# vseib/point-cloud-donkey

Hardware: AMD Instinct MI355X
Metric: objects/sec classified (ModelNet10-like, SHOT-352) (higher is better)
Workload: dtype f32; 1 GPU; configs[1]: ModelNet10-like test split, 16384 pts, 1024 uniform keypoints/object, SHOT-352 (Radius 0.4, LRF 0.3), exact kNN K=1 squared-L2, mean-shift bandwidth 0.6; points_per_object=16384, keypoints_per_object=1024, classes=10, codebook_words=102400, descriptor_dim=352, collective_world_size=1

## Files before the change

### include/ismhip.h

```cpp
#ifndef ISMHIP_H_
#define ISMHIP_H_

#include <stdint.h>

#ifdef __cplusplus
extern "C" {
#endif

#define ISMHIP_ABI_VERSION 4

#define ISMHIP_OK               0
#define ISMHIP_ERR_INVALID     -1
#define ISMHIP_ERR_HIP         -2
#define ISMHIP_ERR_NOMEM       -3
#define ISMHIP_ERR_UNSUPPORTED -4
#define ISMHIP_ERR_NODEVICE    -5

#define ISMHIP_METRIC_L2SQ 0
#define ISMHIP_METRIC_CHI2 1

#define ISMHIP_W_CLASS    1u
#define ISMHIP_W_VOTE     2u
#define ISMHIP_W_MATCHING 4u
#define ISMHIP_W_CODEWORD 8u

#define ISMHIP_KERNEL_GAUSSIAN 0
#define ISMHIP_KERNEL_UNIFORM  1
#define ISMHIP_SUPPRESS_AVERAGE  0
#define ISMHIP_SUPPRESS_SUPPRESS 1
#define ISMHIP_SUPPRESS_NONE     2
#define ISMHIP_MAXFILTER_NONE   0
#define ISMHIP_MAXFILTER_SIMPLE 1
#define ISMHIP_MAXFILTER_MERGE  2
#define ISMHIP_SOM_MEANSHIFT              0
#define ISMHIP_SOM_BANDWIDTH              1
#define ISMHIP_SOM_MODEL_RADIUS           2
#define ISMHIP_SOM_COMPLETE_VOTING_SPACE  3

#define ISMHIP_SHOT_DIM   352
#define ISMHIP_BSHOT_DIM  352
#define ISMHIP_CSHOT_DIM 1344
#define ISMHIP_FPFH_DIM    33
#define ISMHIP_SHORT_SHOT_MAX_DIM 256
#define ISMHIP_COSPAIR_LEVELS 7
#define ISMHIP_COSPAIR_BINS   9
#define ISMHIP_COSPAIR_DIM  378
#define ISMHIP_SPIN_IMAGE_WIDTH 8
#define ISMHIP_SPIN_IMAGE_DIM 153
#define ISMHIP_SHORT_CSHOT_MAX_DIM 1344

typedef struct ismhip_ctx      ismhip_ctx;
typedef struct ismhip_cloud    ismhip_cloud;
typedef struct ismhip_codebook ismhip_codebook;

int  ismhip_abi_version(void);
int  ismhip_ctx_create(int device, void* stream, ismhip_ctx** out);
int  ismhip_ctx_create_on_stream(int device, void* stream, ismhip_ctx** out);
int  ismhip_ctx_destroy(ismhip_ctx* ctx);
int  ismhip_sync(ismhip_ctx* ctx);
const char* ismhip_last_error(const ismhip_ctx* ctx);
int  ismhip_timers_enable(ismhip_ctx* ctx, int on);
int  ismhip_timers_reset(ismhip_ctx* ctx);
int  ismhip_timer_get(ismhip_ctx* ctx, const char* name, double* ms_out, int64_t* launches_out);

int  ismhip_cloud_create(ismhip_ctx* ctx, int n_obj, const uint32_t* pt_offsets_h,
                         const float* x, const float* y, const float* z,
                         const float* nx, const float* ny, const float* nz,
                         const uint32_t* rgba, float cell_size, ismhip_cloud** out);
int  ismhip_cloud_destroy(ismhip_ctx* ctx, ismhip_cloud* cloud);
int  ismhip_estimate_normals(ismhip_ctx* ctx, ismhip_cloud* cloud, float radius, float* nx_out, float* ny_out, float* nz_out);
int  ismhip_estimate_normals_pca(ismhip_ctx* ctx, ismhip_cloud* cloud, float radius, int orientation, float* nx_out, float* ny_out, float* nz_out);
typedef struct ismhip_point_arrays { float *x, *y, *z, *nx, *ny, *nz; uint32_t* rgba; } ismhip_point_arrays;
int  ismhip_filter_normals(ismhip_ctx* ctx, int n_obj, const uint32_t* pt_offsets_h, const ismhip_point_arrays* in,
                           const ismhip_point_arrays* out, uint32_t* pt_offsets_h_out);
#define ISMHIP_SOR_MAX_MEAN_K 64
int  ismhip_filter_statistical(ismhip_ctx* ctx, const ismhip_cloud* cloud, int mean_k, float stddev_mul, uint8_t* keep_out,
                               float* mean_dist_out, double* threshold_h_out);
int  ismhip_filter_radius(ismhip_ctx* ctx, const ismhip_cloud* cloud, float radius, int min_neighbors, uint8_t* keep_out, uint32_t* count_out);
int  ismhip_filter_passthrough_z(ismhip_ctx* ctx, uint32_t n_pts, const float* x, const float* y, const float* z, float z_min, float z_max,
                                 uint8_t* keep_out);
int  ismhip_compact_points(ismhip_ctx* ctx, int n_obj, const uint32_t* pt_offsets_h, const ismhip_point_arrays* in, const uint8_t* keep,
                           const ismhip_point_arrays* out, uint32_t* pt_offsets_h_out);
int  ismhip_cloud_centroids(ismhip_ctx* ctx, const ismhip_cloud* cloud, float* centroid_out);
int  ismhip_cloud_radii(ismhip_ctx* ctx, const ismhip_cloud* cloud, const float* centroid, float* radius_out);

int  ismhip_shot_lrf(ismhip_ctx* ctx, const ismhip_cloud* cloud, const uint32_t* kp_offsets_h,
                     const float* kpx, const float* kpy, const float* kpz,
                     float radius, float* lrf9_out);
int  ismhip_shotna_lrf(ismhip_ctx* ctx, const ismhip_cloud* cloud, const uint32_t* kp_offsets_h,
                       const float* kpx, const float* kpy, const float* kpz,
                       float radius, float* lrf9_out);

int  ismhip_shot352(ismhip_ctx* ctx, const ismhip_cloud* cloud, const uint32_t* kp_offsets_h,
                    const float* kpx, const float* kpy, const float* kpz,
                    const float* lrf9, float radius, float* desc_out, uint32_t* neighbour_count_out);
int  ismhip_bshot_binarize(ismhip_ctx* ctx, int n_rows, const float* src, float* dst);
int  ismhip_bshot352(ismhip_ctx* ctx, const ismhip_cloud* cloud, const uint32_t* kp_offsets_h,
                     const float* kpx, const float* kpy, const float* kpz,
                     const float* lrf9, float radius, float* desc_out, uint32_t* neighbour_count_out);
int  ismhip_cshot1344(ismhip_ctx* ctx, const ismhip_cloud* cloud, const uint32_t* kp_offsets_h,
                      const float* kpx, const float* kpy, const float* kpz, const uint32_t* kp_rgba,
                      const float* lrf9, float radius, float* desc_out, uint32_t* neighbour_count_out);
int  ismhip_fpfh33(ismhip_ctx* ctx, const ismhip_cloud* cloud, const uint32_t* kp_offsets_h,
                   const float* kpx, const float* kpy, const float* kpz,
                   float radius, float* desc_out, uint32_t* neighbour_count_out);
int  ismhip_short_shot(ismhip_ctx* ctx, const ismhip_cloud* cloud, const uint32_t* kp_offsets_h,
                       const float* kpx, const float* kpy, const float* kpz, const float* lrf9,
                       float radius, float min_radius, int log_radius, int r_bins, int e_bins, int a_bins,
                       float* desc_out, uint32_t* neighbour_count_out);
int  ismhip_short_cshot(ismhip_ctx* ctx, const ismhip_cloud* cloud, const uint32_t* kp_offsets_h,
                        const float* kpx, const float* kpy, const float* kpz, const uint32_t* kp_rgba, const float* lrf9,
                        float radius, float min_radius, int log_radius, int r_bins, int e_bins, int a_bins,
                        int rc_bins, int ec_bins, int ac_bins, int hist_size, float* desc_out, uint32_t* neighbour_count_out);
int  ismhip_cospair(ismhip_ctx* ctx, const ismhip_cloud* cloud, const uint32_t* kp_offsets_h,
                    const float* kpx, const float* kpy, const float* kpz, float radius, float* desc_out,
                    uint32_t* neighbour_count_out, uint32_t* level_count_out, uint32_t* snap_index_out);
int  ismhip_keypoint_normals(ismhip_ctx* ctx, const ismhip_cloud* cloud, const uint32_t* kp_offsets_h,
                             const float* kpx, const float* kpy, const float* kpz,
                             float* knx_out, float* kny_out, float* knz_out, int32_t* src_index_out);
int  ismhip_spin_image(ismhip_ctx* ctx, const ismhip_cloud* cloud, const uint32_t* kp_offsets_h,
                       const float* kpx, const float* kpy, const float* kpz, const float* ax, const float* ay, const float* az,
                       float radius, int image_width, float* desc_out, uint32_t* neighbour_count_out);
int  ismhip_center_dist(ismhip_ctx* ctx, const ismhip_cloud* cloud, const uint32_t* kp_offsets_h,
                        const float* kpx, const float* kpy, const float* kpz, float* out);

int  ismhip_global_short_shot(ismhip_ctx* ctx, const ismhip_cloud* cloud, int n_regions, const int32_t* region_obj, const float* region_center,
                              const float* region_radius, double min_radius, int log_radius, int r_bins, int e_bins, int a_bins,
                              uint32_t* n_sel_out, float* centroid_out, float* radius_out, float* lrf9_out, float* desc_out, uint32_t* count_out);
int  ismhip_global_shot352(ismhip_ctx* ctx, const ismhip_cloud* cloud, int n_regions, const int32_t* region_obj, const float* region_center,
                           const float* region_radius, uint32_t* n_sel_out, float* centroid_out, float* radius_out, float* lrf9_out, float* desc_out);

int  ismhip_voxel_keypoints(ismhip_ctx* ctx, int n_obj, const uint32_t* pt_offsets_h,
                            const float* x, const float* y, const float* z, const uint32_t* rgba, float leaf,
                            uint32_t capacity, float* kx, float* ky, float* kz, uint32_t* krgba,
                            uint32_t* kp_offsets_h_out);

int  ismhip_iss3d_saliency(ismhip_ctx* ctx, const ismhip_cloud* cloud, float salient_radius, double gamma21, double gamma32, int min_neighbors,
                           double* saliency_out, double* eig_out, uint32_t* count_out);
int  ismhip_iss3d_keypoints(ismhip_ctx* ctx, const ismhip_cloud* cloud, float salient_radius, float non_max_radius, double gamma21, double gamma32,
                            int min_neighbors, uint32_t capacity, float* kx, float* ky, float* kz, uint32_t* krgba, uint32_t* src_index_out,
                            uint32_t* kp_offsets_h_out);

int  ismhip_compact_features(ismhip_ctx* ctx, int n_obj, const uint32_t* kp_offsets_h, int dim,
                             const float* desc, const float* lrf9,
                             const float* kpx, const float* kpy, const float* kpz,
                             float* desc_out, float* lrf9_out,
                             float* kpx_out, float* kpy_out, float* kpz_out,
                             uint32_t* src_index_out, uint32_t* keep_offsets_h_out);

int  ismhip_compact_descriptor_rows(ismhip_ctx* ctx, int n_obj, const uint32_t* kp_offsets_h, int dim,
                                    const float* desc, const float* lrf9,
                                    const float* kpx, const float* kpy, const float* kpz,
                                    float* desc_out, float* lrf9_out,
                                    float* kpx_out, float* kpy_out, float* kpz_out,
                                    uint32_t* src_index_out, uint32_t* keep_offsets_h_out, int* all_kept_out);

int  ismhip_gather_columns(ismhip_ctx* ctx, int n_rows, int dim_in, const float* src, int n_cols, const int32_t* cols_h, float* dst);

int  ismhip_codebook_create(ismhip_ctx* ctx, int n_words, int dim, const float* words_h,
                            const float* word_weight_h,
                            const uint32_t* vote_offsets_h,
                            const float* vote_xyz_h,
                            const float* vote_weight_h,
                            const float* vote_class_weight_h,
                            const uint32_t* vote_class_h,
                            const uint32_t* vote_instance_h,
                            const float* vote_bbox_quat_h,
                            const float* vote_bbox_size_h,
                            int n_classes, const float* class_sigma_h,
                            ismhip_codebook** out);
int  ismhip_codebook_set_word_class(ismhip_ctx* ctx, ismhip_codebook* cb, const uint32_t* word_class_h);
int  ismhip_codebook_set_word_keypoint(ismhip_ctx* ctx, ismhip_codebook* cb, const float* word_keypoint_h);
int  ismhip_codebook_destroy(ismhip_ctx* ctx, ismhip_codebook* cb);
int  ismhip_codebook_max_votes_per_word(const ismhip_codebook* cb);
int  ismhip_codebook_stage1_dims(const ismhip_codebook* cb, float* energy_out);
int  ismhip_codebook_stage2_dims(const ismhip_codebook* cb, float* energy_out);

int  ismhip_codebook_make_binary(ismhip_ctx* ctx, ismhip_codebook* cb);
int  ismhip_codebook_has_binary(const ismhip_codebook* cb);

int  ismhip_knn(ismhip_ctx* ctx, const ismhip_codebook* cb, int metric, int nq, const float* q,
                int k, int32_t* idx_out, float* dist_out);
int  ismhip_knn_binary(ismhip_ctx* ctx, const ismhip_codebook* cb, int nq, const float* q, int k, int32_t* idx_out, float* dist_out);
#define ISMHIP_KNN_LARGE_K_MAX 1024
int  ismhip_knn_large_k(ismhip_ctx* ctx, const ismhip_codebook* cb, int metric, int nq, const float* q,
                        int k, int32_t* idx_out, float* dist_out);
int  ismhip_knn_ratio(ismhip_ctx* ctx, const ismhip_codebook* cb, int metric, int nq, const float* q,
                      float ratio_threshold, int32_t* idx_out, float* dist_out);

int  ismhip_knn_rule(ismhip_ctx* ctx, const ismhip_codebook* cb, int metric, int nq, const float* q,
                     float ratio_threshold, int32_t* idx_out, float* dist_out);

int  ismhip_knn_threshold(ismhip_ctx* ctx, const ismhip_codebook* cb, int metric, int nq, const float* q, float threshold,
                          int64_t capacity, uint32_t* act_offsets_out, int32_t* idx_out, float* dist_out, int64_t* n_act_h_out);

int  ismhip_cast_votes(ismhip_ctx* ctx, const ismhip_codebook* cb, uint32_t weight_flags,
                       int nq, const float* lrf9, const float* kpx, const float* kpy, const float* kpz,
                       int k, const int32_t* idx, const float* dist,
                       float* vote_pos_out,
                       float* vote_weight_out,
                       int32_t* vote_class_out,
                       int32_t* vote_instance_out,
                       int32_t* vote_codeword_out,
                       float* vote_bbox_quat_out,
                       float* vote_bbox_size_out );

int  ismhip_cast_votes_csr(ismhip_ctx* ctx, const ismhip_codebook* cb, uint32_t weight_flags,
                           int nq, const float* lrf9, const float* kpx, const float* kpy, const float* kpz,
                           const uint32_t* act_offsets, int64_t n_act, const int32_t* idx, const float* dist,
                           float* vote_pos_out, float* vote_weight_out, int32_t* vote_class_out, int32_t* vote_instance_out,
                           int32_t* vote_codeword_out, float* vote_bbox_quat_out, float* vote_bbox_size_out);

int  ismhip_vote_keypoints(ismhip_ctx* ctx, const ismhip_codebook* cb, int nq, const float* kpx, const float* kpy, const float* kpz,
                           int k, const int32_t* idx, float* vote_kp_out, float* vote_kp_train_out);
int  ismhip_vote_keypoints_csr(ismhip_ctx* ctx, const ismhip_codebook* cb, int nq, const float* kpx, const float* kpy, const float* kpz,
                               const uint32_t* act_offsets, int64_t n_act, const int32_t* idx, float* vote_kp_out, float* vote_kp_train_out);

int  ismhip_ransac_filter(ismhip_ctx* ctx, int n_clusters, const uint32_t* cluster_offsets_h, const float* src_xyz, const float* tgt_xyz,
                          const float* threshold_h, int max_iterations, unsigned long long seed,
                          uint8_t* inlier_out, int32_t* kept_out, int32_t* n_inliers_out, int32_t* best_hypothesis_out, int32_t* iterations_out,
                          float* transform_out);
int  ismhip_ransac_hypothesis(ismhip_ctx* ctx, int n_clusters, const uint32_t* cluster_offsets_h, const float* src_xyz, const float* tgt_xyz,
                              const float* threshold_h, unsigned long long seed, const int32_t* hypothesis_h,
                              uint8_t* inlier_out, int32_t* valid_out, int32_t* n_inliers_out, double* d2_out, double* transform_out);

typedef struct ismhip_maxima_params {
    int   n_classes;
    const float* class_bandwidth_h;
    float bandwidth;
    float threshold;
    int   max_iter;
    int   kernel;
    int   suppression;
    int   min_votes_threshold;
    float min_threshold;
    int   best_k;
    int   max_maxima;
    int   max_filter;
    const float* vote_bbox_quat;
    float* max_bbox_quat_out;
    int   single_object_max_type;
    const float* object_centroid;
    const float* object_radius;
} ismhip_maxima_params;

int  ismhip_find_maxima(ismhip_ctx* ctx, int n_obj, const uint32_t* slot_offsets_h,
                        const float* vote_pos, const float* vote_weight, const int32_t* vote_class,
                        const int32_t* vote_instance, const float* vote_bbox_size ,
                        const ismhip_maxima_params* params,
                        int32_t* n_maxima_out, float* max_pos_out, float* max_weight_out,
                        int32_t* max_class_out, int32_t* max_instance_out, float* max_instance_weight_out,
                        float* max_bbox_size_out , int32_t* max_n_votes_out,
                        float* class_score_out);

typedef struct ismhip_ransac_params {
    const float* vote_keypoint;
    const float* vote_keypoint_training;
    float inlier_threshold;
    const float* class_inlier_threshold_h;
    int   max_iterations;
    unsigned long long seed;
} ismhip_ransac_params;
int  ismhip_find_maxima_ransac(ismhip_ctx* ctx, int n_obj, const uint32_t* slot_offsets_h,
                               const float* vote_pos, const float* vote_weight, const int32_t* vote_class,
                               const int32_t* vote_instance, const float* vote_bbox_size ,
                               const ismhip_maxima_params* params,
                               int32_t* n_maxima_out, float* max_pos_out, float* max_weight_out,
                               int32_t* max_class_out, int32_t* max_instance_out, float* max_instance_weight_out,
                               float* max_bbox_size_out , int32_t* max_n_votes_out,
                               float* class_score_out, const ismhip_ransac_params* ransac, float* max_transform_out);

int  ismhip_train_activate(ismhip_ctx* ctx, int metric, int n, int dim, const float* desc, const float* lrf9,
                           const float* kpx, const float* kpy, const float* kpz,
                           const uint32_t* feat_class_h, const uint32_t* feat_model_h, const float* feat_center_h,
                           int n_codewords, const float* codewords ,
                           int k, int clean_up_single_vote, int n_classes,
                           int32_t* n_words_out, uint32_t* word_src_out, uint32_t* vote_offsets_out, uint32_t* vote_feature_out,
                           float* vote_xyz_out, float* vote_weight_out, float* vote_class_weight_out, float* class_sigma_out);

int  ismhip_train_activate_lists(ismhip_ctx* ctx, int metric, int n, int dim, const float* desc, const float* lrf9,
                                 const float* kpx, const float* kpy, const float* kpz,
                                 const uint32_t* feat_class_h, const uint32_t* feat_model_h, const float* feat_center_h,
                                 int n_codewords, const float* codewords ,
                                 const uint32_t* act_offsets, const int32_t* act_idx, int64_t n_act, int n_classes,
                                 int32_t* n_words_out, uint32_t* word_src_out, uint32_t* vote_offsets_out, uint32_t* vote_feature_out,
                                 float* vote_xyz_out, float* vote_weight_out, float* vote_class_weight_out, float* class_sigma_out);

#define ISMHIP_RANK_KNN_ACTIVATION 0
#define ISMHIP_RANK_INCREMENTAL    1
#define ISMHIP_RANK_STRANGENESS    2
#define ISMHIP_RANK_NAIVE_BAYES    3
int  ismhip_rank_scores(ismhip_ctx* ctx, int type, int n, int dim, const float* desc, int n_classes, const uint32_t* class_offsets_h,
                        int k_search, float dist_threshold, int increment_type, float* score_out);
int  ismhip_rank_select(ismhip_ctx* ctx, int n, int n_classes, const uint32_t* class_offsets_h, const float* score,
                        float factor, float extract_offset, uint8_t* keep_out, uint32_t* n_keep_h_out);

#define ISMHIP_CENTERS_RANDOM   0
#define ISMHIP_CENTERS_GONZALES 1
#define ISMHIP_CENTERS_KMEANSPP 2
int  ismhip_kmeans(ismhip_ctx* ctx, int metric, int n, int dim, const float* desc, int n_clusters, int max_iterations,
                   int centers_init, unsigned long long seed, float* centers_out, int32_t* assign_out, float* dist_out,
                   int32_t* n_clusters_out, int32_t* iterations_out );

typedef struct ismhip_hough_params {
    int   n_classes;
    float min_coord[3];
    float max_coord[3];
    float bin_size;
    const float* class_bin_h;
    int   use_interpolation;
    float rel_threshold;
    int   min_votes_threshold;
    float min_threshold;
    int   best_k;
    int   max_maxima;
    int   max_filter;
    const float* vote_bbox_quat;
    float* max_bbox_quat_out;
} ismhip_hough_params;
int  ismhip_hough3d_maxima(ismhip_ctx* ctx, int n_obj, const uint32_t* slot_offsets_h,
                           const float* vote_pos, const float* vote_weight, const int32_t* vote_class,
                           const int32_t* vote_instance, const float* vote_bbox_size ,
                           const ismhip_hough_params* params,
                           int32_t* n_maxima_out, float* max_pos_out, float* max_weight_out,
                           int32_t* max_class_out, int32_t* max_instance_out, float* max_instance_weight_out,
                           float* max_bbox_size_out , int32_t* max_n_votes_out,
                           float* class_score_out);

int  ismhip_hough3d_maxima_ransac(ismhip_ctx* ctx, int n_obj, const uint32_t* slot_offsets_h,
                                  const float* vote_pos, const float* vote_weight, const int32_t* vote_class,
                                  const int32_t* vote_instance, const float* vote_bbox_size ,
                                  const ismhip_hough_params* params,
                                  int32_t* n_maxima_out, float* max_pos_out, float* max_weight_out,
                                  int32_t* max_class_out, int32_t* max_instance_out, float* max_instance_weight_out,
                                  float* max_bbox_size_out , int32_t* max_n_votes_out,
                                  float* class_score_out, const ismhip_ransac_params* ransac, float* max_transform_out);

#ifdef __cplusplus
}
#endif
#endif
```

### point-cloud-donkey_amd/capi.py

```python
import ctypes as C
import os

import numpy as np

_HERE = os.path.dirname(os.path.abspath(__file__))
LIB_PATH = os.path.join(_HERE, "libismhip.so")

METRIC_L2SQ, METRIC_CHI2 = 0, 1
W_CLASS, W_VOTE, W_MATCHING, W_CODEWORD = 1, 2, 4, 8
KERNEL_GAUSSIAN, KERNEL_UNIFORM = 0, 1
SUPPRESS_AVERAGE, SUPPRESS_SUPPRESS, SUPPRESS_NONE = 0, 1, 2
MAXFILTER_NONE, MAXFILTER_SIMPLE, MAXFILTER_MERGE = 0, 1, 2
SOM_MEANSHIFT, SOM_BANDWIDTH, SOM_MODEL_RADIUS, SOM_COMPLETE_VOTING_SPACE = 0, 1, 2, 3
ERR_NODEVICE = -5

EXPORTS = [
    "ismhip_abi_version", "ismhip_ctx_create", "ismhip_ctx_create_on_stream", "ismhip_ctx_destroy", "ismhip_sync", "ismhip_last_error",
    "ismhip_timers_enable", "ismhip_timers_reset", "ismhip_timer_get",
    "ismhip_cloud_create", "ismhip_cloud_destroy", "ismhip_cloud_centroids", "ismhip_cloud_radii", "ismhip_estimate_normals", "ismhip_estimate_normals_pca",
    "ismhip_shot_lrf", "ismhip_shotna_lrf", "ismhip_shot352", "ismhip_cshot1344", "ismhip_fpfh33", "ismhip_center_dist",
    "ismhip_compact_features", "ismhip_compact_descriptor_rows", "ismhip_filter_normals", "ismhip_voxel_keypoints", "ismhip_gather_columns",
    "ismhip_codebook_create", "ismhip_codebook_set_word_class", "ismhip_codebook_destroy", "ismhip_codebook_max_votes_per_word", "ismhip_codebook_stage1_dims", "ismhip_codebook_stage2_dims",
    "ismhip_knn", "ismhip_knn_ratio", "ismhip_knn_rule", "ismhip_cast_votes", "ismhip_find_maxima", "ismhip_hough3d_maxima", "ismhip_train_activate", "ismhip_kmeans",
    "ismhip_knn_threshold", "ismhip_cast_votes_csr", "ismhip_train_activate_lists", "ismhip_knn_large_k",
    "ismhip_filter_statistical", "ismhip_filter_radius", "ismhip_filter_passthrough_z", "ismhip_compact_points",
    "ismhip_codebook_set_word_keypoint", "ismhip_vote_keypoints", "ismhip_vote_keypoints_csr", "ismhip_ransac_filter", "ismhip_ransac_hypothesis",
    "ismhip_find_maxima_ransac", "ismhip_hough3d_maxima_ransac", "ismhip_short_shot", "ismhip_short_cshot", "ismhip_cospair",
    "ismhip_bshot_binarize", "ismhip_bshot352", "ismhip_codebook_make_binary", "ismhip_codebook_has_binary", "ismhip_knn_binary",
    "ismhip_rank_scores", "ismhip_rank_select", "ismhip_global_short_shot", "ismhip_global_shot352",
    "ismhip_iss3d_saliency", "ismhip_iss3d_keypoints", "ismhip_keypoint_normals", "ismhip_spin_image",
]
RANSAC_MAX_ITERATIONS = 10000
RANSAC_SEED = 12345


class MaximaParams(C.Structure):
    _fields_ = [("n_classes", C.c_int), ("class_bandwidth_h", C.c_void_p), ("bandwidth", C.c_float),
                ("threshold", C.c_float), ("max_iter", C.c_int), ("kernel", C.c_int), ("suppression", C.c_int),
                ("min_votes_threshold", C.c_int), ("min_threshold", C.c_float), ("best_k", C.c_int),
                ("max_maxima", C.c_int), ("max_filter", C.c_int),
                ("vote_bbox_quat", C.c_void_p), ("max_bbox_quat_out", C.c_void_p), ("single_object_max_type", C.c_int),
                ("object_centroid", C.c_void_p), ("object_radius", C.c_void_p)]


class HoughParams(C.Structure):
    _fields_ = [("n_classes", C.c_int), ("min_coord", C.c_float * 3), ("max_coord", C.c_float * 3), ("bin_size", C.c_float),
                ("class_bin_h", C.c_void_p), ("use_interpolation", C.c_int), ("rel_threshold", C.c_float),
                ("min_votes_threshold", C.c_int), ("min_threshold", C.c_float), ("best_k", C.c_int), ("max_maxima", C.c_int), ("max_filter", C.c_int),
                ("vote_bbox_quat", C.c_void_p), ("max_bbox_quat_out", C.c_void_p)]


class RansacParams(C.Structure):
    _fields_ = [("vote_keypoint", C.c_void_p), ("vote_keypoint_training", C.c_void_p), ("inlier_threshold", C.c_float),
                ("class_inlier_threshold_h", C.c_void_p), ("max_iterations", C.c_int), ("seed", C.c_ulonglong)]


class IsmHipError(RuntimeError):
    pass


_lib = None


def lib():
    global _lib
    if _lib is None:
        if not os.path.exists(LIB_PATH):
            raise IsmHipError(f"{LIB_PATH} not built: run `python -c 'import __graft_entry__ as g; g.build()'` "
                              "(make -C point-cloud-donkey_amd/csrc)")
        import torch
        L = C.CDLL(LIB_PATH)
        L.ismhip_last_error.restype = C.c_char_p
        L.ismhip_last_error.argtypes = [C.c_void_p]
        for name in EXPORTS:
            fn = getattr(L, name)
            if name != "ismhip_last_error":
                fn.restype = C.c_int
        _lib = L
    return _lib


def _p(t):
    if t is None:
        return C.c_void_p(0)
    if isinstance(t, np.ndarray):
        assert t.flags["C_CONTIGUOUS"]
        return C.c_void_p(t.ctypes.data)
    assert t.is_contiguous()
    return C.c_void_p(t.data_ptr())


def _u32(a):
    return np.ascontiguousarray(np.asarray(a, dtype=np.uint32))


class Ctx:
    def __init__(self, device=0, stream="torch"):
        self._h = C.c_void_p()
        L = lib()
        if stream is None:
            rc = L.ismhip_ctx_create(C.c_int(device), C.c_void_p(0), C.byref(self._h))
        else:
            if stream == "torch":
                import torch
                if not torch.cuda.is_available():
                    raise IsmHipError("no gfx950 device visible: the hot path has no CPU fallback (ISMHIP_ERR_NODEVICE)")
                if not (0 <= device < torch.cuda.device_count()):
                    raise IsmHipError(f"device {device} out of range (ISMHIP_ERR_INVALID)")
                stream = torch.cuda.current_stream(device).cuda_stream
            rc = L.ismhip_ctx_create_on_stream(C.c_int(device), C.c_void_p(stream), C.byref(self._h))
        if rc != 0:
            raise IsmHipError(f"ismhip_ctx_create failed ({rc}); a gfx950 device is required, there is no CPU fallback")
        self.device = device

    def check(self, rc, what):
        if rc != 0:
            raise IsmHipError(f"{what} failed ({rc}): {lib().ismhip_last_error(self._h).decode()}")

    def sync(self):
        self.check(lib().ismhip_sync(self._h), "ismhip_sync")

    def timers_enable(self, on=True):
        self.check(lib().ismhip_timers_enable(self._h, C.c_int(1 if on else 0)), "timers_enable")

    def timers_reset(self):
        self.check(lib().ismhip_timers_reset(self._h), "timers_reset")

    def timer(self, name):
        ms, n = C.c_double(), C.c_int64()
        self.check(lib().ismhip_timer_get(self._h, name.encode(), C.byref(ms), C.byref(n)), "timer_get")
        return ms.value, n.value

    def close(self):
        if self._h:
            lib().ismhip_ctx_destroy(self._h)
            self._h = C.c_void_p()

    def __del__(self):
        try:
            self.close()
        except Exception:
            pass


class Cloud:

    def __init__(self, ctx, pt_offsets, x, y, z, nx, ny, nz, cell_size, rgba=None):
        self.ctx = ctx
        self.pt_offsets = _u32(pt_offsets)
        self.n_obj = len(self.pt_offsets) - 1
        self._keep = (x, y, z, nx, ny, nz, rgba)
        self._h = C.c_void_p()
        rc = lib().ismhip_cloud_create(ctx._h, C.c_int(self.n_obj), _p(self.pt_offsets), _p(x), _p(y), _p(z), _p(nx), _p(ny),
                                       _p(nz), _p(rgba), C.c_float(cell_size), C.byref(self._h))
        ctx.check(rc, "ismhip_cloud_create")

    def close(self):
        if self._h:
            lib().ismhip_cloud_destroy(self.ctx._h, self._h)
            self._h = C.c_void_p()

    def __del__(self):
        try:
            self.close()
        except Exception:
            pass


class Codebook:
    def __init__(self, ctx, words, vote_offsets, vote_xyz, vote_class, vote_instance, n_classes, class_sigma,
                 word_weight=None, vote_weight=None, vote_class_weight=None, vote_bbox_quat=None, vote_bbox_size=None):
        f32 = lambda a: None if a is None else np.ascontiguousarray(np.asarray(a, dtype=np.float32))
        self.ctx = ctx
        words = f32(words)
        self.n_words, self.dim = words.shape
        self.n_classes = int(n_classes)
        self._h = C.c_void_p()
        rc = lib().ismhip_codebook_create(ctx._h, C.c_int(self.n_words), C.c_int(self.dim), _p(words), _p(f32(word_weight)),
                                          _p(_u32(vote_offsets)), _p(f32(vote_xyz)), _p(f32(vote_weight)),
                                          _p(f32(vote_class_weight)), _p(_u32(vote_class)), _p(_u32(vote_instance)),
                                          _p(f32(vote_bbox_quat)), _p(f32(vote_bbox_size)), C.c_int(self.n_classes),
                                          _p(f32(class_sigma)), C.byref(self._h))
        ctx.check(rc, "ismhip_codebook_create")
        self.max_votes = lib().ismhip_codebook_max_votes_per_word(self._h)
        e = C.c_float(1.0)
        self.stage1_dims = int(lib().ismhip_codebook_stage1_dims(self._h, C.byref(e)))
        self.stage1_energy = float(e.value)
        self.stage2_dims = int(lib().ismhip_codebook_stage2_dims(self._h, C.byref(e)))
        self.stage2_energy = float(e.value)

    def set_word_class(self, word_class):
        self.ctx.check(lib().ismhip_codebook_set_word_class(self.ctx._h, self._h, _p(_u32(word_class))), "ismhip_codebook_set_word_class")

    def set_word_keypoint(self, word_keypoint):
        kp = np.ascontiguousarray(np.asarray(word_keypoint, dtype=np.float32))
        assert kp.shape == (self.n_words, 3)
        self.ctx.check(lib().ismhip_codebook_set_word_keypoint(self.ctx._h, self._h, _p(kp)), "ismhip_codebook_set_word_keypoint")

    def make_binary(self):
        self.ctx.check(lib().ismhip_codebook_make_binary(self.ctx._h, self._h), "ismhip_codebook_make_binary")

    @property
    def has_binary(self):
        return lib().ismhip_codebook_has_binary(self._h) == 1

    def close(self):
        if self._h:
            lib().ismhip_codebook_destroy(self.ctx._h, self._h)
            self._h = C.c_void_p()

    def __del__(self):
        try:
            self.close()
        except Exception:
            pass


def _torch():
    import torch
    return torch


def shot_lrf(ctx, cloud, kp_offsets, kpx, kpy, kpz, radius):
    torch = _torch()
    ko = _u32(kp_offsets)
    out = torch.empty((int(ko[-1]), 9), dtype=torch.float32, device=kpx.device)
    ctx.check(lib().ismhip_shot_lrf(ctx._h, cloud._h, _p(ko), _p(kpx), _p(kpy), _p(kpz), C.c_float(radius), _p(out)), "ismhip_shot_lrf")
    return out


def shotna_lrf(ctx, cloud, kp_offsets, kpx, kpy, kpz, radius):
    torch = _torch()
    ko = _u32(kp_offsets)
    out = torch.empty((int(ko[-1]), 9), dtype=torch.float32, device=kpx.device)
    ctx.check(lib().ismhip_shotna_lrf(ctx._h, cloud._h, _p(ko), _p(kpx), _p(kpy), _p(kpz), C.c_float(radius), _p(out)), "ismhip_shotna_lrf")
    return out


LRF_TYPES = {"SHOT": shot_lrf, "SHOTNA": shotna_lrf}


def shot352(ctx, cloud, kp_offsets, kpx, kpy, kpz, lrf, radius, want_counts=False):
    torch = _torch()
    ko = _u32(kp_offsets)
    n = int(ko[-1])
    out = torch.empty((n, 352), dtype=torch.float32, device=kpx.device)
    cnt = torch.empty((n,), dtype=torch.int32, device=kpx.device) if want_counts else None
    ctx.check(lib().ismhip_shot352(ctx._h, cloud._h, _p(ko), _p(kpx), _p(kpy), _p(kpz), _p(lrf), C.c_float(radius), _p(out), _p(cnt)),
              "ismhip_shot352")
    return (out, cnt) if want_counts else out


def bshot_binarize(ctx, src, out=None):
    torch = _torch()
    assert src.dim() == 2 and src.shape[1] == 352 and src.dtype == torch.float32
    if out is None:
        out = torch.empty_like(src)
    ctx.check(lib().ismhip_bshot_binarize(ctx._h, C.c_int(src.shape[0]), _p(src), _p(out)), "ismhip_bshot_binarize")
    return out


def bshot352(ctx, cloud, kp_offsets, kpx, kpy, kpz, lrf, radius, want_counts=False):
    torch = _torch()
    ko = _u32(kp_offsets)
    n = int(ko[-1])
    out = torch.empty((n, 352), dtype=torch.float32, device=kpx.device)
    cnt = torch.empty((n,), dtype=torch.int32, device=kpx.device) if want_counts else None
    ctx.check(lib().ismhip_bshot352(ctx._h, cloud._h, _p(ko), _p(kpx), _p(kpy), _p(kpz), _p(lrf), C.c_float(radius), _p(out), _p(cnt)),
              "ismhip_bshot352")
    return (out, cnt) if want_counts else out


def cshot1344(ctx, cloud, kp_offsets, kpx, kpy, kpz, kp_rgba, lrf, radius, want_counts=False):
    torch = _torch()
    ko = _u32(kp_offsets)
    n = int(ko[-1])
    out = torch.empty((n, 1344), dtype=torch.float32, device=kpx.device)
    cnt = torch.empty((n,), dtype=torch.int32, device=kpx.device) if want_counts else None
    ctx.check(lib().ismhip_cshot1344(ctx._h, cloud._h, _p(ko), _p(kpx), _p(kpy), _p(kpz), _p(kp_rgba), _p(lrf), C.c_float(radius),
                                     _p(out), _p(cnt)), "ismhip_cshot1344")
    return (out, cnt) if want_counts else out


def short_shot(ctx, cloud, kp_offsets, kpx, kpy, kpz, lrf, radius, bins=(2, 2, 8), min_radius=0.0, log_radius=False, want_counts=False):
    torch = _torch()
    ko = _u32(kp_offsets)
    n = int(ko[-1])
    r, e, a = (int(b) for b in bins)
    out = torch.empty((n, max(r * e * a, 0) if min(r, e, a) > 0 else 0), dtype=torch.float32, device=kpx.device)
    cnt = torch.empty((n,), dtype=torch.int32, device=kpx.device) if want_counts else None
    ctx.check(lib().ismhip_short_shot(ctx._h, cloud._h, _p(ko), _p(kpx), _p(kpy), _p(kpz), _p(lrf), C.c_float(radius), C.c_float(min_radius),
                                      C.c_int(1 if log_radius else 0), C.c_int(r), C.c_int(e), C.c_int(a), _p(out), _p(cnt)), "ismhip_short_shot")
    return (out, cnt) if want_counts else out


SHORT_SHOT_AUTO_BINS = {8: (1, 1, 8), 16: (2, 2, 4), 24: (2, 2, 6), 32: (2, 2, 8), 64: (2, 4, 8), 96: (3, 4, 8), 128: (4, 4, 8), 192: (6, 4, 8),
                        256: (8, 4, 8)}


def short_shot_grid(dims=32, bin_type="auto", bins=(2, 2, 8)):
    if bin_type == "manual":
        r, e, a = (int(b) for b in bins)
        return r * e * a, (r, e, a)
    if bin_type == "auto" and int(dims) in SHORT_SHOT_AUTO_BINS:
        return int(dims), SHORT_SHOT_AUTO_BINS[int(dims)]
    return 32, (2, 2, 8)


def short_shot_min_radius(radius, use_min_radius=False, min_radius_relative=0.0, log_radius=False):
    if use_min_radius:
        return float(np.float32(float(np.float32(radius)) * float(min_radius_relative)))
    return float(np.float32(float(np.float32(radius)) * float(np.float32(0.1)))) if log_radius else 0.0


def short_cshot(ctx, cloud, kp_offsets, kpx, kpy, kpz, kp_rgba, lrf, radius, bins=(2, 2, 8), color_bins=(2, 2, 8), hist_size=15, min_radius=0.0,
                log_radius=False, want_counts=False):
    torch = _torch()
    ko = _u32(kp_offsets)
    n = int(ko[-1])
    r, e, a = (int(b) for b in bins)
    rc, ec, ac = (int(b) for b in color_bins)
    h = int(hist_size)
    out = torch.empty((n, r * e * a + rc * ec * ac * h if min(r, e, a, rc, ec, ac, h) > 0 else 0), dtype=torch.float32, device=kpx.device)
    cnt = torch.empty((n,), dtype=torch.int32, device=kpx.device) if want_counts else None
    ctx.check(lib().ismhip_short_cshot(ctx._h, cloud._h, _p(ko), _p(kpx), _p(kpy), _p(kpz), _p(kp_rgba), _p(lrf), C.c_float(radius),
                                       C.c_float(min_radius), C.c_int(1 if log_radius else 0), C.c_int(r), C.c_int(e), C.c_int(a), C.c_int(rc),
                                       C.c_int(ec), C.c_int(ac), C.c_int(h), _p(out), _p(cnt)), "ismhip_short_cshot")
    return (out, cnt) if want_counts else out


SHORT_CSHOT_COLOR_BINS = {d: SHORT_SHOT_AUTO_BINS[d] for d in (8, 16, 24, 32, 64, 96, 128)}


def short_cshot_color_grid(dims=32):
    if int(dims) in SHORT_CSHOT_COLOR_BINS:
        return int(dims), SHORT_CSHOT_COLOR_BINS[int(dims)]
    return 32, (2, 2, 8)


COSPAIR_LEVELS, COSPAIR_BINS, COSPAIR_DIM = 7, 9, 378


def cospair(ctx, cloud, kp_offsets, kpx, kpy, kpz, radius, want_counts=False, want_levels=False, want_snap=False):
    torch = _torch()
    ko = _u32(kp_offsets)
    n = int(ko[-1])
    out = torch.empty((n, COSPAIR_DIM), dtype=torch.float32, device=kpx.device)
    cnt = torch.empty((n,), dtype=torch.int32, device=kpx.device) if want_counts else None
    lev = torch.empty((n, COSPAIR_LEVELS), dtype=torch.int32, device=kpx.device) if want_levels else None
    snap = torch.empty((n,), dtype=torch.int32, device=kpx.device) if want_snap else None
    ctx.check(lib().ismhip_cospair(ctx._h, cloud._h, _p(ko), _p(kpx), _p(kpy), _p(kpz), C.c_float(radius), _p(out), _p(cnt), _p(lev), _p(snap)),
              "ismhip_cospair")
    extra = [t for t in (cnt, lev, snap) if t is not None]
    return (out, *extra) if extra else out


SPIN_IMAGE_WIDTH = 8
SPIN_IMAGE_DIM = (SPIN_IMAGE_WIDTH + 1) * (2 * SPIN_IMAGE_WIDTH + 1)


def keypoint_normals(ctx, cloud, kp_offsets, kpx, kpy, kpz, want_index=False):
    torch = _torch()
    ko = _u32(kp_offsets)
    n = int(ko[-1])
    nx, ny, nz = (torch.empty((n,), dtype=torch.float32, device=kpx.device) for _ in range(3))
    src = torch.empty((n,), dtype=torch.int32, device=kpx.device) if want_index else None
    ctx.check(lib().ismhip_keypoint_normals(ctx._h, cloud._h, _p(ko), _p(kpx), _p(kpy), _p(kpz), _p(nx), _p(ny), _p(nz), _p(src)),
              "ismhip_keypoint_normals")
    return (nx, ny, nz, src) if want_index else (nx, ny, nz)


def spin_image(ctx, cloud, kp_offsets, kpx, kpy, kpz, ax, ay, az, radius, image_width=SPIN_IMAGE_WIDTH, want_counts=False):
    torch = _torch()
    ko = _u32(kp_offsets)
    n = int(ko[-1])
    w = int(image_width)
    out = torch.empty((n, (w + 1) * (2 * w + 1) if w >= 1 else 0), dtype=torch.float32, device=kpx.device)
    cnt = torch.empty((n,), dtype=torch.int32, device=kpx.device) if want_counts else None
    ctx.check(lib().ismhip_spin_image(ctx._h, cloud._h, _p(ko), _p(kpx), _p(kpy), _p(kpz), _p(ax), _p(ay), _p(az), C.c_float(radius), C.c_int(w),
                                      _p(out), _p(cnt)), "ismhip_spin_image")
    return (out, cnt) if want_counts else out


GLOBAL_SHORT_SHOT_AUTO_BINS = dict(SHORT_SHOT_AUTO_BINS)
GLOBAL_SHORT_SHOT_AUTO_BINS[64] = (4, 2, 8)


def global_short_shot_grid(dims=32, bin_type="auto", bins=(1, 1, 8)):
    if bin_type == "manual":
        r, e, a = (int(b) for b in bins)
        return r * e * a, (r, e, a)
    if bin_type == "auto" and int(dims) in GLOBAL_SHORT_SHOT_AUTO_BINS:
        return int(dims), GLOBAL_SHORT_SHOT_AUTO_BINS[int(dims)]
    return 32, (2, 2, 8)


def _regions(cloud, region_obj, region_center, region_radius, dev):
    torch = _torch()
    obj = torch.as_tensor(np.ascontiguousarray(np.asarray(region_obj, dtype=np.int32)), device=dev)
    n = int(obj.shape[0])
    cen = np.zeros((n, 3), np.float32) if region_center is None else np.ascontiguousarray(np.asarray(region_center, dtype=np.float32)).reshape(n, 3)
    rad = np.full((n,), -1.0, np.float32) if region_radius is None else np.ascontiguousarray(np.asarray(region_radius, dtype=np.float32)).reshape(n)
    return n, obj, torch.as_tensor(cen, device=dev), torch.as_tensor(rad, device=dev)


def _global_outputs(n, dim, dev):
    torch = _torch()
    return dict(n_sel=torch.empty((n,), dtype=torch.int32, device=dev), centroid=torch.empty((n, 3), dtype=torch.float32, device=dev),
                radius=torch.empty((n,), dtype=torch.float32, device=dev), lrf=torch.empty((n, 9), dtype=torch.float32, device=dev),
                desc=torch.empty((n, dim), dtype=torch.float32, device=dev))


def global_short_shot(ctx, cloud, dev, region_obj, region_center=None, region_radius=None, bins=(2, 2, 8), min_radius=0.1, log_radius=False,
                      want_counts=False):
    torch = _torch()
    n, obj, cen, rad = _regions(cloud, region_obj, region_center, region_radius, dev)
    r, e, a = (int(b) for b in bins)
    out = _global_outputs(n, r * e * a if min(r, e, a) > 0 else 0, dev)
    if want_counts:
        out["counts"] = torch.empty_like(out["desc"], dtype=torch.int32)
    ctx.check(lib().ismhip_global_short_shot(ctx._h, cloud._h, C.c_int(n), _p(obj), _p(cen), _p(rad), C.c_double(min_radius),
                                             C.c_int(1 if log_radius else 0), C.c_int(r), C.c_int(e), C.c_int(a), _p(out["n_sel"]),
                                             _p(out["centroid"]), _p(out["radius"]), _p(out["lrf"]), _p(out["desc"]), _p(out.get("counts"))),
              "ismhip_global_short_shot")
    return out


def global_shot352(ctx, cloud, dev, region_obj, region_center=None, region_radius=None):
    n, obj, cen, rad = _regions(cloud, region_obj, region_center, region_radius, dev)
    out = _global_outputs(n, 352, dev)
    ctx.check(lib().ismhip_global_shot352(ctx._h, cloud._h, C.c_int(n), _p(obj), _p(cen), _p(rad), _p(out["n_sel"]), _p(out["centroid"]),
                                          _p(out["radius"]), _p(out["lrf"]), _p(out["desc"])), "ismhip_global_shot352")
    return out


def fpfh33(ctx, cloud, kp_offsets, kpx, kpy, kpz, radius, want_counts=False):
    torch = _torch()
    ko = _u32(kp_offsets)
    n = int(ko[-1])
    out = torch.empty((n, 33), dtype=torch.float32, device=kpx.device)
    cnt = torch.empty((n,), dtype=torch.int32, device=kpx.device) if want_counts else None
    ctx.check(lib().ismhip_fpfh33(ctx._h, cloud._h, _p(ko), _p(kpx), _p(kpy), _p(kpz), C.c_float(radius), _p(out), _p(cnt)),
              "ismhip_fpfh33")
    return (out, cnt) if want_counts else out


def cloud_centroids(ctx, cloud, device):
    torch = _torch()
    out = torch.empty((cloud.n_obj, 3), dtype=torch.float32, device=device)
    ctx.check(lib().ismhip_cloud_centroids(ctx._h, cloud._h, _p(out)), "ismhip_cloud_centroids")
    return out


def cloud_radii(ctx, cloud, centroid):
    torch = _torch()
    out = torch.empty((cloud.n_obj,), dtype=torch.float32, device=centroid.device)
    ctx.check(lib().ismhip_cloud_radii(ctx._h, cloud._h, _p(centroid), _p(out)), "ismhip_cloud_radii")
    return out


def center_dist(ctx, cloud, kp_offsets, kpx, kpy, kpz):
    torch = _torch()
    ko = _u32(kp_offsets)
    out = torch.empty((int(ko[-1]),), dtype=torch.float32, device=kpx.device)
    ctx.check(lib().ismhip_center_dist(ctx._h, cloud._h, _p(ko), _p(kpx), _p(kpy), _p(kpz), _p(out)), "ismhip_center_dist")
    return out


def estimate_normals(ctx, cloud, radius, nx, ny, nz):
    ctx.check(lib().ismhip_estimate_normals(ctx._h, cloud._h, C.c_float(radius), _p(nx), _p(ny), _p(nz)), "ismhip_estimate_normals")
    cloud._keep = getattr(cloud, "_keep", ()) + (nx, ny, nz)
    return nx, ny, nz


def estimate_normals_pca(ctx, cloud, radius, orientation, nx, ny, nz):
    ctx.check(lib().ismhip_estimate_normals_pca(ctx._h, cloud._h, C.c_float(radius), C.c_int(orientation), _p(nx), _p(ny), _p(nz)), "ismhip_estimate_normals_pca")
    cloud._keep = getattr(cloud, "_keep", ()) + (nx, ny, nz)
    return nx, ny, nz


class _PointArrays(C.Structure):
    _fields_ = [(n, C.c_void_p) for n in ("x", "y", "z", "nx", "ny", "nz", "rgba")]


def _compact_point_arrays(ctx, symbol, pt_offsets, arrays, rgba, *mask):
    torch = _torch()
    po = _u32(pt_offsets)
    n_obj = len(po) - 1
    ins = list(arrays) + ([rgba] if rgba is not None else [])
    outs = [torch.empty_like(t) for t in ins]
    a_in = _PointArrays(*[t.data_ptr() for t in ins], *([None] if rgba is None else []))
    a_out = _PointArrays(*[t.data_ptr() for t in outs], *([None] if rgba is None else []))
    new = np.zeros(n_obj + 1, dtype=np.uint32)
# ... 431 lines not shown
```

### point-cloud-donkey_amd/csrc/common.h

```cpp
#pragma once
#include <hip/hip_runtime.h>
#include <stdint.h>
#include <map>
#include <set>
#include <string>
#include <vector>
#include "../../include/ismhip.h"

#define ISM_WAVE 64

#define ISM_GRID_MAXDIM 32
#define ISM_GRID_MAXCELLS (ISM_GRID_MAXDIM * ISM_GRID_MAXDIM * ISM_GRID_MAXDIM)
#define ISM_GRID_STRIDE (ISM_GRID_MAXCELLS + 1)

#define ISM_GRID_XFRAC 3
struct GridMeta {
    float minv[3];
    float cell[3];
    float inv_cell[3];
    int   dim[3];
    float centroid[3];
    uint32_t n_finite;
};

struct ismhip_cloud {
    int n_obj = 0;
    uint32_t n_pts = 0;
    uint32_t max_pts = 0;
    std::vector<uint32_t> pt_off_h;
    uint32_t* pt_off = nullptr;
    const float *x = nullptr, *y = nullptr, *z = nullptr, *nx = nullptr, *ny = nullptr, *nz = nullptr;
    const uint32_t* rgba = nullptr;
    float4* sp4 = nullptr;
    float4* sn4 = nullptr;
    float4* slab4 = nullptr;
    uint32_t* cell_of_pt = nullptr;
    uint32_t* rank_of_pt = nullptr;
    uint32_t* members = nullptr;
    GridMeta* meta = nullptr;
    uint32_t* cell_start = nullptr;
    float requested_cell = 0.f;
    uint32_t* kp_perm = nullptr;
    size_t kp_perm_cap = 0;
    const float* kp_perm_key = nullptr;
    std::vector<uint32_t> kp_perm_off;
    uint16_t* cospair_code = nullptr;
    size_t cospair_code_cap = 0;
    bool cospair_code_valid = false;
    size_t cap_pts = 0; int cap_obj = 0; bool cap_color = false;
};

struct PcaImage {
    int m = 0;
    float* R = nullptr;
    unsigned short* f16t = nullptr;
    float* cn_scaled = nullptr;
    float* osc = nullptr;
    float sq = 1.f, sc = 1.f;
    float cmax2 = 0.f;
    float inv_sig2 = 1.f;
    float d_rel = 0.f;
    float dq_abs = 0.f, dc_abs = 0.f;
    float resid2 = 0.f;
    float energy = 0.f;
};

struct ismhip_codebook {
    int n_words = 0, dim = 0, dim_pad = 0, n_votes = 0, max_votes = 0, n_classes = 0;
    float* words = nullptr;
    int n_words_pad = 0;
    float* word_norm = nullptr;
    unsigned short* words_bf16_hi = nullptr;
    unsigned short* words_bf16_lo = nullptr;
    unsigned short* words_f16 = nullptr;
    unsigned short* words_f16t = nullptr;
    int ld16 = 0;
    float f16_scale = 1.f;
    bool words_nonneg = false;
    float max_norm2 = 0.f;
    float* word_weight = nullptr;
    uint32_t* vote_off = nullptr;
    float* vote_xyz = nullptr;
    float* vote_weight = nullptr;
    float* vote_class_weight = nullptr;
    uint32_t* vote_class = nullptr;
    uint32_t* vote_instance = nullptr;
    float* vote_bbox_quat = nullptr;
    float* vote_bbox_size = nullptr;
    float* class_sigma = nullptr;
    uint32_t* word_class = nullptr;
    float* word_keypoint = nullptr;
    ismhip_codebook* chi_shadow = nullptr;
    uint32_t* shadow_perm = nullptr;
    PcaImage pca, pca2;
    int8_t* bin_words = nullptr;
    int32_t* bin_norm = nullptr;
    int bin_ld = 0, bin_shift = 0;
};

struct TimerAcc {
    std::vector<std::pair<hipEvent_t, hipEvent_t>> pending;
    double ms = 0.0;
    int64_t launches = 0;
};

struct ismhip_ctx {
    int device = 0;
    hipStream_t stream = nullptr;
    bool own_stream = false;
    std::string err;
    bool timers_on = false;
    std::map<std::string, TimerAcc> timers;
    std::vector<hipEvent_t> event_pool;
    struct Slot { void* p = nullptr; size_t bytes = 0; };
    std::map<int, Slot> scratch;
    float* lut_srgb = nullptr;
    float* lut_sxyz = nullptr;
    std::vector<ismhip_cloud*> cloud_pool;
    uint32_t* truncated_d = nullptr;
    unsigned long long* ransac_counters_d = nullptr;
    uint32_t knn_stats[2] = {0, 0};
    std::set<const void*> attr_done;
    uint32_t knn_stage2_queries = 0;
    uint32_t knn_stage2_list_entries = 0;
    uint32_t knn_stage2_ranged = 0;
    uint32_t knn_seed_launches = 0;
    bool knn_stage2_splits = true;
    bool knn_stage2_seed = true;
    bool knn_two_stage = true;
    bool knn_join = true;
    bool knn_qpanel2 = true;
    bool knn_half = false;
    int knn_splits = 0;
    int knn_t = 0;
    bool xcd_map = true;
    bool grid_fused = true;
    bool kp_order = true;
    float grid_xfrac = 0.f;
    int shot_var = 0;
    bool knn_hell_emit = true;
    bool knn_hellinger = true;
    int knn_t1 = 2;
    int knn_pre_step = 32;
    float knn_pre_gamma = 1.0f;
    bool knn_prepass = true;
    int knn_pca_m = -1;
    bool knn_stage2_t4 = false;
    bool codebook_light = false;
    int knn_pca_m2 = -1;
    uint32_t knn_pca_launches = 0;
    uint32_t knn_thr_overflow = 0;
    uint32_t knn_thr_mfma_launches = 0;
    bool knn_lk_fast = false;
    bool knn_lk_exact = false;
    float knn_lk_seed_scale = 1.0f;
    uint32_t knn_lk_stats[3] = {0, 0, 0};
    uint32_t knn_binary_launches = 0;
    uint32_t rank_launches = 0;
    bool iss3d_wave = false;
    int knn_mode = 0;
};

enum ScratchSlot {
    SCR_KP_OFF = 1, SCR_TIE_LIST, SCR_TIE_REC, SCR_TIE_KEYS, SCR_COUNTERS, SCR_KNN_CAND_IDX, SCR_KNN_CAND_VAL,
    SCR_QNORM, SCR_FPFH_FLAG, SCR_FPFH_LIST, SCR_FPFH_SPFH, SCR_FPFH_LOOKUP, SCR_SLOT_OFF, SCR_CLASS_BW,
    SCR_COMPACT_KEEP, SCR_COMPACT_POS, SCR_OBJ_COUNT, SCR_QPAD, SCR_LRF_COV, SCR_KNN_FLAGS, SCR_KNN_QSPLIT, SCR_MAX_REC, SCR_QNORM2, SCR_KNN_Q2, SCR_KNN_LIST2, SCR_TRAIN, SCR_TRAIN2, SCR_MAX_WORK, SCR_KMEANS, SCR_KNN_CLOCK, SCR_PCA, SCR_KNN_THR0, SCR_KNN_QSQRT, SCR_KNN_HELL_EMIT, SCR_KNN_THR, SCR_KNN_THR2, SCR_TRAIN_ACT, SCR_KNN_LK, SCR_KNN_LK2, SCR_KNN_LK3, SCR_PREFILTER, SCR_RANSAC, SCR_COSPAIR, SCR_KNNB_FLAG, SCR_KNNB_Q, SCR_KNNB_CAND, SCR_RANK, SCR_RANK_KNN, SCR_KNN_LISTS, SCR_KNN_QUEUE, SCR_ISS3D
};

int  ism_set_err(ismhip_ctx* ctx, int code, const std::string& msg);
void* ism_scratch(ismhip_ctx* ctx, int slot, size_t bytes);
int  ism_lds_cap(ismhip_ctx* ctx, const void* kern, size_t bytes);

uint32_t* ism_upload_offsets(ismhip_ctx* ctx, int slot, const uint32_t* off_h, int n);
struct RaggedOffsets { uint32_t max_run = 0, total = 0; uint32_t* dev = nullptr; };
enum { RAGGED_START0 = 1,
       RAGGED_EMPTY = 2 };
int ism_ragged_offsets(ismhip_ctx* ctx, const std::string& name, const uint32_t* off_h, int n, int slot, int flags, RaggedOffsets* r);
int ism_offsets_from_counts(ismhip_ctx* ctx, int n, const uint32_t* cnt_d, uint32_t* off_h_out, uint32_t* max_run_out);
const uint32_t* ism_kp_order(ismhip_ctx* ctx, const ismhip_cloud* cloud, const uint32_t* kp_offsets_h, const uint32_t* ko,
                             const float* kpx, const float* kpy, const float* kpz, uint32_t maxk);

int ism_compact_keypoints(ismhip_ctx* ctx, const std::string& who, const ismhip_cloud* cloud, const uint8_t* mask, uint32_t capacity,
                          float* kx, float* ky, float* kz, uint32_t* krgba, uint32_t* src_index_out, uint32_t* kp_offsets_h_out);

#define ISM_HIP(ctx, call)                                                                          \
    do {                                                                                            \
        hipError_t e__ = (call);                                                                    \
        if (e__ != hipSuccess)                                                                      \
            return ism_set_err((ctx), ISMHIP_ERR_HIP, std::string(#call) + ": " + hipGetErrorString(e__)); \
    } while (0)

#define ISM_CHECK_LAUNCH(ctx, name)                                                                 \
    do {                                                                                            \
        hipError_t e__ = hipGetLastError();                                                         \
        if (e__ != hipSuccess)                                                                      \
            return ism_set_err((ctx), ISMHIP_ERR_HIP, std::string("launch ") + name + ": " + hipGetErrorString(e__)); \
    } while (0)

struct TimerScope {
    ismhip_ctx* ctx; const char* name; hipEvent_t a = nullptr, b = nullptr;
    TimerScope(ismhip_ctx* c, const char* n);
    ~TimerScope();
};

#ifdef __HIPCC__
__device__ __forceinline__ int lane_id() { return threadIdx.x & 63; }

__device__ __forceinline__ float sqdist3(float ax, float ay, float az, float bx, float by, float bz) {
    float r = 0.f, d;
    d = ax - bx; r += d * d;
    d = ay - by; r += d * d;
    d = az - bz; r += d * d;
    return r;
}

template <int CTRL>
__device__ __forceinline__ int dpp_mov0(int v) { return __builtin_amdgcn_update_dpp(0, v, CTRL, 0xf, 0xf, false); }

__device__ __forceinline__ float wave_sum_f(float v) {
    v += __int_as_float(dpp_mov0<0xb1>(__float_as_int(v)));
    v += __int_as_float(dpp_mov0<0x4e>(__float_as_int(v)));
    v += __int_as_float(dpp_mov0<0x114>(__float_as_int(v)));
    v += __int_as_float(dpp_mov0<0x118>(__float_as_int(v)));
    v += __int_as_float(dpp_mov0<0x142>(__float_as_int(v)));
    v += __int_as_float(dpp_mov0<0x143>(__float_as_int(v)));
    return __int_as_float(__builtin_amdgcn_readlane(__float_as_int(v), 63));
}
__device__ __forceinline__ int wave_sum_i(int v) {
    v += dpp_mov0<0xb1>(v);
    v += dpp_mov0<0x4e>(v);
    v += dpp_mov0<0x114>(v);
    v += dpp_mov0<0x118>(v);
    v += dpp_mov0<0x142>(v);
    v += dpp_mov0<0x143>(v);
    return __builtin_amdgcn_readlane(v, 63);
}
template <int CTRL>
__device__ __forceinline__ int dpp_movi(int ident, int v) { return __builtin_amdgcn_update_dpp(ident, v, CTRL, 0xf, 0xf, false); }
__device__ __forceinline__ float wave_min_f(float v) {
    const int inf = 0x7f800000;
    v = fminf(v, __int_as_float(dpp_movi<0xb1>(inf, __float_as_int(v))));
    v = fminf(v, __int_as_float(dpp_movi<0x4e>(inf, __float_as_int(v))));
    v = fminf(v, __int_as_float(dpp_movi<0x114>(inf, __float_as_int(v))));
    v = fminf(v, __int_as_float(dpp_movi<0x118>(inf, __float_as_int(v))));
    v = fminf(v, __int_as_float(dpp_movi<0x142>(inf, __float_as_int(v))));
    v = fminf(v, __int_as_float(dpp_movi<0x143>(inf, __float_as_int(v))));
    return __int_as_float(__builtin_amdgcn_readlane(__float_as_int(v), 63));
}
template <int CTRL>
__device__ __forceinline__ unsigned long long dpp_min_u64(unsigned long long v) {
    const unsigned lo = (unsigned)dpp_movi<CTRL>(-1, (int)(unsigned)(v & 0xffffffffull)), hi = (unsigned)dpp_movi<CTRL>(-1, (int)(unsigned)(v >> 32));
    const unsigned long long o = ((unsigned long long)hi << 32) | lo;
    return o < v ? o : v;
}
__device__ __forceinline__ unsigned long long wave_min_u64(unsigned long long v) {
    v = dpp_min_u64<0xb1>(v); v = dpp_min_u64<0x4e>(v); v = dpp_min_u64<0x114>(v);
    v = dpp_min_u64<0x118>(v); v = dpp_min_u64<0x142>(v); v = dpp_min_u64<0x143>(v);
    const unsigned lo = (unsigned)__builtin_amdgcn_readlane((int)(unsigned)(v & 0xffffffffull), 63), hi = (unsigned)__builtin_amdgcn_readlane((int)(unsigned)(v >> 32), 63);
    return ((unsigned long long)hi << 32) | lo;
}
__device__ __forceinline__ float wave_max_f(float v) {
    const int ninf = (int)0xff800000;
    v = fmaxf(v, __int_as_float(dpp_movi<0xb1>(ninf, __float_as_int(v))));
    v = fmaxf(v, __int_as_float(dpp_movi<0x4e>(ninf, __float_as_int(v))));
    v = fmaxf(v, __int_as_float(dpp_movi<0x114>(ninf, __float_as_int(v))));
    v = fmaxf(v, __int_as_float(dpp_movi<0x118>(ninf, __float_as_int(v))));
    v = fmaxf(v, __int_as_float(dpp_movi<0x142>(ninf, __float_as_int(v))));
    v = fmaxf(v, __int_as_float(dpp_movi<0x143>(ninf, __float_as_int(v))));
    return __int_as_float(__builtin_amdgcn_readlane(__float_as_int(v), 63));
}
__device__ __forceinline__ uint32_t wave_max_u32(uint32_t v) {
    v = max(v, (uint32_t)dpp_mov0<0xb1>((int)v)); v = max(v, (uint32_t)dpp_mov0<0x4e>((int)v)); v = max(v, (uint32_t)dpp_mov0<0x114>((int)v));
    v = max(v, (uint32_t)dpp_mov0<0x118>((int)v)); v = max(v, (uint32_t)dpp_mov0<0x142>((int)v)); v = max(v, (uint32_t)dpp_mov0<0x143>((int)v));
    return (uint32_t)__builtin_amdgcn_readlane((int)v, 63);
}
template <int CTRL>
__device__ __forceinline__ unsigned long long dpp_mov0_u64(unsigned long long v) {
    const unsigned lo = (unsigned)dpp_mov0<CTRL>((int)(unsigned)(v & 0xffffffffull)), hi = (unsigned)dpp_mov0<CTRL>((int)(unsigned)(v >> 32));
    return ((unsigned long long)hi << 32) | lo;
}
__device__ __forceinline__ unsigned long long readlane63_u64(unsigned long long v) {
    const unsigned lo = (unsigned)__builtin_amdgcn_readlane((int)(unsigned)(v & 0xffffffffull), 63), hi = (unsigned)__builtin_amdgcn_readlane((int)(unsigned)(v >> 32), 63);
    return ((unsigned long long)hi << 32) | lo;
}
template <int CTRL>
__device__ __forceinline__ unsigned long long dpp_max_u64(unsigned long long v) { const unsigned long long o = dpp_mov0_u64<CTRL>(v); return o > v ? o : v; }
__device__ __forceinline__ unsigned long long wave_max_u64(unsigned long long v) {
    v = dpp_max_u64<0xb1>(v); v = dpp_max_u64<0x4e>(v); v = dpp_max_u64<0x114>(v);
    v = dpp_max_u64<0x118>(v); v = dpp_max_u64<0x142>(v); v = dpp_max_u64<0x143>(v);
    return readlane63_u64(v);
}
__device__ __forceinline__ unsigned long long wave_sum_u64(unsigned long long v) {
    v += dpp_mov0_u64<0xb1>(v); v += dpp_mov0_u64<0x4e>(v); v += dpp_mov0_u64<0x114>(v);
    v += dpp_mov0_u64<0x118>(v); v += dpp_mov0_u64<0x142>(v); v += dpp_mov0_u64<0x143>(v);
    return readlane63_u64(v);
}
__device__ __forceinline__ uint32_t wave_incl_scan_u32(uint32_t v) {
    int x = (int)v;
    x += dpp_mov0<0x111>(x); x += dpp_mov0<0x112>(x); x += dpp_mov0<0x114>(x); x += dpp_mov0<0x118>(x);
    x += __builtin_amdgcn_update_dpp(0, x, 0x142, 0xa, 0xf, false);
    x += __builtin_amdgcn_update_dpp(0, x, 0x143, 0xc, 0xf, false);
    return (uint32_t)x;
}
template <int NT>
struct BlockScan {
    uint32_t wave[NT / 64];
    uint32_t carry;
    __device__ __forceinline__ void init() {
        if (threadIdx.x == 0) carry = 0;
        __syncthreads();
    }
    __device__ __forceinline__ uint32_t step(uint32_t v) {
        const uint32_t incl = wave_incl_scan_u32(v);
        const int w = threadIdx.x >> 6;
        if (lane_id() == 63) wave[w] = incl;
        __syncthreads();
        uint32_t before = carry;
        for (int k = 0; k < w; ++k) before += wave[k];
        __syncthreads();
        if (threadIdx.x == NT - 1) carry = before + incl;
        __syncthreads();
        return before + incl - v;
    }
    __device__ __forceinline__ uint32_t total() const { return carry; }
};
template <int NT>
struct BlockRank {
    uint32_t wave[NT / 64];
    __device__ __forceinline__ uint32_t step(bool flag, uint32_t& total) {
        const unsigned long long b = __ballot(flag);
        const int w = threadIdx.x >> 6;
        if (lane_id() == 0) wave[w] = (uint32_t)__popcll(b);
        __syncthreads();
        uint32_t before = total, chunk = 0;
#pragma unroll
        for (int k = 0; k < NT / 64; ++k) { const uint32_t c = wave[k]; chunk += c; if (k < w) before += c; }
        __syncthreads();
        total += chunk;
        return before + (uint32_t)__popcll(b & ((1ull << lane_id()) - 1ull));
    }
};
template <int CTRL>
__device__ __forceinline__ double dpp_mov0_d(double v) {
    const long long b = __double_as_longlong(v);
    const int lo = dpp_mov0<CTRL>((int)(b & 0xffffffffll)), hi = dpp_mov0<CTRL>((int)(b >> 32));
    return __longlong_as_double(((long long)hi << 32) | (unsigned int)lo);
}
__device__ __forceinline__ double wave_sum_d(double v) {
    v += dpp_mov0_d<0xb1>(v);
    v += dpp_mov0_d<0x4e>(v);
    v += dpp_mov0_d<0x114>(v);
    v += dpp_mov0_d<0x118>(v);
    v += dpp_mov0_d<0x142>(v);
    v += dpp_mov0_d<0x143>(v);
    const long long b = __double_as_longlong(v);
    const int lo = __builtin_amdgcn_readlane((int)(b & 0xffffffffll), 63), hi = __builtin_amdgcn_readlane((int)(b >> 32), 63);
    return __longlong_as_double(((long long)hi << 32) | (unsigned int)lo);
}

template <int NW, class T, class F>
__device__ __forceinline__ T block_fold(T wave_total, T* red, F&& combine) {
    if (lane_id() == 0) red[threadIdx.x >> 6] = wave_total;
    __syncthreads();
    T r = red[0];
#pragma unroll
    for (int k = 1; k < NW; ++k) r = combine(r, red[k]);
    __syncthreads();
    return r;
}
template <int NW = 4, class T>
__device__ __forceinline__ T block_sum_i(T v, T* red) { return block_fold<NW>((T)wave_sum_i((int)v), red, [](T a, T b) { return (T)(a + b); }); }
template <int NW = 4>
__device__ __forceinline__ unsigned long long block_sum_u64(unsigned long long v, unsigned long long* red) {
    return block_fold<NW>(wave_sum_u64(v), red, [](unsigned long long a, unsigned long long b) { return a + b; });
}
template <int NW = 4>
__device__ __forceinline__ float block_min_f(float v, float* red) { return block_fold<NW>(wave_min_f(v), red, [](float a, float b) { return fminf(a, b); }); }
template <int NW = 4>
__device__ __forceinline__ float block_max_f(float v, float* red) { return block_fold<NW>(wave_max_f(v), red, [](float a, float b) { return fmaxf(a, b); }); }
template <int NW = 4>
__device__ __forceinline__ uint32_t block_max_u32(uint32_t v, uint32_t* red) { return block_fold<NW>(wave_max_u32(v), red, [](uint32_t a, uint32_t b) { return a > b ? a : b; }); }
template <int NW = 4>
__device__ __forceinline__ unsigned long long block_min_u64(unsigned long long v, unsigned long long* red) {
    return block_fold<NW>(wave_min_u64(v), red, [](unsigned long long a, unsigned long long b) { return b < a ? b : a; });
}
template <int NW = 4>
__device__ __forceinline__ unsigned long long block_max_u64(unsigned long long v, unsigned long long* red) {
    return block_fold<NW>(wave_max_u64(v), red, [](unsigned long long a, unsigned long long b) { return b > a ? b : a; });
}
template <int NW = 4>
__device__ __forceinline__ double block_sum_d_left(double v, double* red) { return block_fold<NW>(wave_sum_d(v), red, [](double a, double b) { return a + b; }); }
template <class T>
__device__ __forceinline__ T block_sum_pairwise(T wave_total, T* red) {
    if (lane_id() == 0) red[threadIdx.x >> 6] = wave_total;
    __syncthreads();
    const T r = (red[0] + red[1]) + (red[2] + red[3]);
    __syncthreads();
    return r;
}
__device__ __forceinline__ float block_sum_f_pairwise(float v, float* red) { return block_sum_pairwise(wave_sum_f(v), red); }
__device__ __forceinline__ double block_sum_d_pairwise(double v, double* red) { return block_sum_pairwise(wave_sum_d(v), red); }

__device__ __forceinline__ float shot_atan2(float y, float x) {
    const float ax = fabsf(x), ay = fabsf(y);
    const float mx = fmaxf(ax, ay), mn = fminf(ax, ay);
    const float a = mn * __builtin_amdgcn_rcpf(mx);
    const float z = a * a;
    float p = 0.0028662257f;
    p = __builtin_fmaf(p, z, -0.0161657367f); p = __builtin_fmaf(p, z, 0.0429096138f); p = __builtin_fmaf(p, z, -0.0752896400f);
    p = __builtin_fmaf(p, z, 0.1065626393f); p = __builtin_fmaf(p, z, -0.1420889944f); p = __builtin_fmaf(p, z, 0.1999355085f);
    p = __builtin_fmaf(p, z, -0.3333314528f); p = __builtin_fmaf(p, z, 1.0f);
    float r = a * p;
    if (ay > ax) r = 1.57079632679489661923f - r;
    if (x < 0.f) r = 3.14159265358979323846f - r;
    return y < 0.f ? -r : r;
}

__device__ __forceinline__ void rgb2lab(const float* lut_srgb, const float* lut_sxyz, uint32_t c4, float& L, float& A, float& B) {
    const float fr = lut_srgb[(c4 >> 16) & 0xff], fg = lut_srgb[(c4 >> 8) & 0xff], fb = lut_srgb[c4 & 0xff];
    const float X = fr * 0.412453f + fg * 0.357580f + fb * 0.180423f;
    const float Y = fr * 0.212671f + fg * 0.715160f + fb * 0.072169f;
    const float Z = fr * 0.019334f + fg * 0.119193f + fb * 0.950227f;
    float vx = X / 0.95047f, vy = Y, vz = Z / 1.08883f;
    int ix = (int)(vx * 4000), iy = (int)(vy * 4000), iz = (int)(vz * 4000);
    ix = ix < 0 ? 0 : (ix > 3999 ? 3999 : ix); iy = iy < 0 ? 0 : (iy > 3999 ? 3999 : iy); iz = iz < 0 ? 0 : (iz > 3999 ? 3999 : iz);
    vx = lut_sxyz[ix]; vy = lut_sxyz[iy]; vz = lut_sxyz[iz];
    L = 116.0f * vy - 16.0f; if (L > 100) L = 100.0f;
    A = 500.0f * (vx - vy); if (A > 120) A = 120.0f; else if (A < -120) A = -120.0f;
    B = 200.0f * (vy - vz); if (B > 120) B = 120.0f; else if (B < -120) B = -120.0f;
}
__device__ __forceinline__ void rgb2lab_norm(const float* lut_srgb, const float* lut_sxyz, uint32_t c4, float& L, float& A, float& B) {
    rgb2lab(lut_srgb, lut_sxyz, c4, L, A, B);
    L /= 100.0f; A /= 120.0f; B /= 120.0f;
}

__device__ __forceinline__ bool xcd_object_block(int nbx, int n_obj, int& o, int& bx) {
    if (n_obj < 8) { o = blockIdx.x / nbx; bx = blockIdx.x % nbx; return true; }
    const int slot = blockIdx.x >> 3;
    o = (slot / nbx) * 8 + (blockIdx.x & 7);
    bx = slot % nbx;
    return o < n_obj;
}
__device__ __forceinline__ uint32_t ordered_keypoint(const uint32_t* __restrict__ perm, uint32_t kp_begin, uint32_t slot) {
    return kp_begin + (perm ? perm[kp_begin + slot] : slot);
}
static inline unsigned xcd_object_grid(unsigned nbx, int n_obj) { return n_obj < 8 ? nbx * (unsigned)n_obj : 8u * nbx * (unsigned)((n_obj + 7) / 8); }

__device__ __forceinline__ int cell_coord(float v, float minv, float inv_cell, int dim) {
    int c = (int)floorf((v - minv) * inv_cell);
    return c < 0 ? 0 : (c >= dim ? dim - 1 : c);
}
// ... 140 lines not shown
```

### point-cloud-donkey_amd/csrc/ctx.hip

```cpp
#include "common.h"
#include <cmath>
#include <cstring>
#include <cstdlib>

extern "C" void ism_cloud_pool_release(ismhip_ctx* ctx);

int ism_set_err(ismhip_ctx* ctx, int code, const std::string& msg) {
    if (ctx) ctx->err = msg;
    return code;
}

int ism_lds_cap(ismhip_ctx* ctx, const void* kern, size_t bytes) {
    if (ctx->attr_done.count(kern)) return ISMHIP_OK;
    ISM_HIP(ctx, hipFuncSetAttribute(kern, hipFuncAttributeMaxDynamicSharedMemorySize, (int)bytes));
    ctx->attr_done.insert(kern);
    return ISMHIP_OK;
}

void* ism_scratch(ismhip_ctx* ctx, int slot, size_t bytes) {
    if (bytes == 0) bytes = 16;
    auto& s = ctx->scratch[slot];
    if (s.bytes >= bytes) return s.p;
    if (s.p) { (void)hipStreamSynchronize(ctx->stream); (void)hipFree(s.p); s.p = nullptr; s.bytes = 0; }
    size_t want = bytes + bytes / 4;
    void* p = nullptr;
    if (hipMalloc(&p, want) != hipSuccess) { ism_set_err(ctx, ISMHIP_ERR_NOMEM, "scratch hipMalloc failed"); return nullptr; }
    s.p = p; s.bytes = want;
    return p;
}

TimerScope::TimerScope(ismhip_ctx* c, const char* n) : ctx(c), name(n) {
    if (!ctx->timers_on) return;
    auto get = [&]() {
        hipEvent_t e = nullptr;
        if (!ctx->event_pool.empty()) { e = ctx->event_pool.back(); ctx->event_pool.pop_back(); }
        else (void)hipEventCreate(&e);
        return e;
    };
    a = get(); b = get();
    (void)hipEventRecord(a, ctx->stream);
}
TimerScope::~TimerScope() {
    if (!a) return;
    (void)hipEventRecord(b, ctx->stream);
    ctx->timers[name].pending.emplace_back(a, b);
}

extern "C" {

int ismhip_abi_version(void) { return ISMHIP_ABI_VERSION; }

static int ctx_create_impl(int device, void* stream, bool own, ismhip_ctx** out);

int ismhip_ctx_create(int device, void* stream, ismhip_ctx** out) { return ctx_create_impl(device, stream, stream == nullptr, out); }
int ismhip_ctx_create_on_stream(int device, void* stream, ismhip_ctx** out) { return ctx_create_impl(device, stream, false, out); }

static int ctx_create_impl(int device, void* stream, bool own, ismhip_ctx** out) {
    if (!out) return ISMHIP_ERR_INVALID;
    *out = nullptr;
    int n = 0;
    if (hipGetDeviceCount(&n) != hipSuccess || n <= 0) return ISMHIP_ERR_NODEVICE;
    if (device < 0 || device >= n) return ISMHIP_ERR_INVALID;
    if (hipSetDevice(device) != hipSuccess) return ISMHIP_ERR_HIP;
    hipDeviceProp_t prop;
    if (hipGetDeviceProperties(&prop, device) != hipSuccess) return ISMHIP_ERR_HIP;
    if (std::strncmp(prop.gcnArchName, "gfx950", 6) != 0) return ISMHIP_ERR_NODEVICE;
    ismhip_ctx* ctx = new ismhip_ctx();
    ctx->device = device;
    { const char* e = getenv("ISMHIP_KNN_MODE"); ctx->knn_mode = !e ? 0 : (!strcmp(e, "bf16x3") ? 1 : (!strcmp(e, "f32") ? 2 : 0)); }
    { const char* e = getenv("ISMHIP_XCD_MAP"); ctx->xcd_map = !(e && e[0] == '0'); }
    { const char* e = getenv("ISMHIP_GRID_FUSED"); ctx->grid_fused = !(e && e[0] == '0'); }
    { const char* e = getenv("ISMHIP_KP_ORDER"); ctx->kp_order = !(e && e[0] == '0'); }
    { const char* e = getenv("ISMHIP_GRID_XFRAC"); ctx->grid_xfrac = e ? (float)atof(e) : 0.f; }
    { const char* e = getenv("ISMHIP_SHOT_VAR"); ctx->shot_var = e ? atoi(e) : 0; }
    { const char* e = getenv("ISMHIP_KNN_TWOSTAGE"); ctx->knn_two_stage = !(e && e[0] == '0'); }
    { const char* e = getenv("ISMHIP_KNN_JOIN"); ctx->knn_join = !(e && e[0] == '0'); }
    { const char* e = getenv("ISMHIP_KNN_QPANEL2"); ctx->knn_qpanel2 = !(e && e[0] == '0'); }
    { const char* e = getenv("ISMHIP_KNN_HALF"); ctx->knn_half = e && e[0] == '1'; }
    { const char* e = getenv("ISMHIP_KNN_SPLITS"); ctx->knn_splits = e ? atoi(e) : 0; }
    { const char* e = getenv("ISMHIP_KNN_T"); ctx->knn_t = e ? atoi(e) : 0; }
    { const char* e = getenv("ISMHIP_KNN_HELL_EMIT"); ctx->knn_hell_emit = !(e && e[0] == '0'); }
    { const char* e = getenv("ISMHIP_KNN_HELLINGER"); ctx->knn_hellinger = !(e && e[0] == '0'); }
    { const char* e = getenv("ISMHIP_KNN_T1"); if (e) ctx->knn_t1 = atoi(e); }
    { const char* e = getenv("ISMHIP_KNN_STAGE2_T4"); if (e) ctx->knn_stage2_t4 = atoi(e) != 0; }
    { const char* e = getenv("ISMHIP_KNN_STAGE2_SPLITS"); ctx->knn_stage2_splits = !(e && e[0] == '0'); }
    { const char* e = getenv("ISMHIP_KNN_STAGE2_SEED"); ctx->knn_stage2_seed = !(e && e[0] == '0'); }
    { const char* e = getenv("ISMHIP_KNN_PRE_STEP"); if (e && atoi(e) > 0) ctx->knn_pre_step = atoi(e); }
    { const char* e = getenv("ISMHIP_KNN_PRE_GAMMA"); if (e) ctx->knn_pre_gamma = (float)atof(e); }
    { const char* e = getenv("ISMHIP_KNN_PREPASS"); ctx->knn_prepass = !(e && e[0] == '0'); }
    { const char* e = getenv("ISMHIP_KNN_PCA_M"); ctx->knn_pca_m = e ? atoi(e) : -1; }
    { const char* e = getenv("ISMHIP_KNN_LARGE_K_FAST"); ctx->knn_lk_fast = e && e[0] == '1'; }
    { const char* e = getenv("ISMHIP_KNN_LARGE_K_EXACT"); ctx->knn_lk_exact = e && e[0] == '1'; }
    { const char* e = getenv("ISMHIP_KNN_LARGE_K_SEED_SCALE"); if (e) ctx->knn_lk_seed_scale = (float)atof(e); }
    { const char* e = getenv("ISMHIP_ISS3D_MAP"); ctx->iss3d_wave = e && !strcmp(e, "wave"); }
    { const char* e = getenv("ISMHIP_KNN_PCA_M2"); ctx->knn_pca_m2 = e ? atoi(e) : -1; }
    if (!own) { ctx->stream = (hipStream_t)stream; ctx->own_stream = false; }
    else {
        if (hipStreamCreateWithFlags(&ctx->stream, hipStreamNonBlocking) != hipSuccess) { delete ctx; return ISMHIP_ERR_HIP; }
        ctx->own_stream = true;
    }
    std::vector<float> srgb(256), sxyz(4000);
    for (int i = 0; i < 256; i++) {
        float f = static_cast<float>(i) / 255.0f;
        srgb[i] = (f > 0.04045) ? powf((f + 0.055f) / 1.055f, 2.4f) : f / 12.92f;
    }
    for (int i = 0; i < 4000; i++) {
        float f = static_cast<float>(i) / 4000.0f;
        sxyz[i] = (f > 0.008856) ? static_cast<float>(powf(f, 0.3333f)) : static_cast<float>((7.787 * f) + (16.0 / 116.0));
    }
    if (hipMalloc((void**)&ctx->lut_srgb, 256 * 4) != hipSuccess || hipMalloc((void**)&ctx->lut_sxyz, 4000 * 4) != hipSuccess) {
        delete ctx; return ISMHIP_ERR_NOMEM;
    }
    (void)hipMemcpy(ctx->lut_srgb, srgb.data(), 256 * 4, hipMemcpyHostToDevice);
    (void)hipMemcpy(ctx->lut_sxyz, sxyz.data(), 4000 * 4, hipMemcpyHostToDevice);
    if (hipMalloc((void**)&ctx->truncated_d, 4) != hipSuccess) { delete ctx; return ISMHIP_ERR_NOMEM; }
    (void)hipMemset(ctx->truncated_d, 0, 4);
    (void)hipDeviceSynchronize();
    *out = ctx;
    return ISMHIP_OK;
}

int ismhip_ctx_destroy(ismhip_ctx* ctx) {
    if (!ctx) return ISMHIP_ERR_INVALID;
    (void)hipSetDevice(ctx->device);
    (void)hipStreamSynchronize(ctx->stream);
    ism_cloud_pool_release(ctx);
    for (auto& kv : ctx->scratch) if (kv.second.p) (void)hipFree(kv.second.p);
    for (auto& kv : ctx->timers) for (auto& pr : kv.second.pending) { (void)hipEventDestroy(pr.first); (void)hipEventDestroy(pr.second); }
    for (auto e : ctx->event_pool) (void)hipEventDestroy(e);
    if (ctx->lut_srgb) (void)hipFree(ctx->lut_srgb);
    if (ctx->lut_sxyz) (void)hipFree(ctx->lut_sxyz);
    if (ctx->truncated_d) (void)hipFree(ctx->truncated_d);
    if (ctx->ransac_counters_d) (void)hipFree(ctx->ransac_counters_d);
    if (ctx->own_stream) (void)hipStreamDestroy(ctx->stream);
    delete ctx;
    return ISMHIP_OK;
}

int ismhip_sync(ismhip_ctx* ctx) {
    if (!ctx) return ISMHIP_ERR_INVALID;
    if (ctx->truncated_d) {
        uint32_t n = 0;
        ISM_HIP(ctx, hipMemcpyAsync(&n, ctx->truncated_d, 4, hipMemcpyDeviceToHost, ctx->stream));
        ISM_HIP(ctx, hipStreamSynchronize(ctx->stream));
        if (n) {
            ISM_HIP(ctx, hipMemsetAsync(ctx->truncated_d, 0, 4, ctx->stream));
            ISM_HIP(ctx, hipStreamSynchronize(ctx->stream));
            return ism_set_err(ctx, ISMHIP_ERR_UNSUPPORTED, "find_maxima / hough3d_maxima: " + std::to_string(n) +
                               " (object, class) lists exceeded 128 maxima per class or 1024 per object since the last sync; the results of those objects are truncated");
        }
        return ISMHIP_OK;
    }
    ISM_HIP(ctx, hipStreamSynchronize(ctx->stream));
    return ISMHIP_OK;
}

const char* ismhip_last_error(const ismhip_ctx* ctx) { return ctx ? ctx->err.c_str() : "null ctx"; }

int ismhip_timers_enable(ismhip_ctx* ctx, int on) {
    if (!ctx) return ISMHIP_ERR_INVALID;
    ctx->timers_on = on != 0;
    return ISMHIP_OK;
}

static void resolve_timers(ismhip_ctx* ctx) {
    (void)hipStreamSynchronize(ctx->stream);
    for (auto& kv : ctx->timers) {
        for (auto& pr : kv.second.pending) {
            float ms = 0.f;
            if (hipEventElapsedTime(&ms, pr.first, pr.second) == hipSuccess) { kv.second.ms += ms; kv.second.launches++; }
            ctx->event_pool.push_back(pr.first); ctx->event_pool.push_back(pr.second);
        }
        kv.second.pending.clear();
    }
}

int ismhip_timers_reset(ismhip_ctx* ctx) {
    if (!ctx) return ISMHIP_ERR_INVALID;
    resolve_timers(ctx);
    for (auto& kv : ctx->timers) { kv.second.ms = 0; kv.second.launches = 0; }
    if (ctx->ransac_counters_d) { ISM_HIP(ctx, hipMemsetAsync(ctx->ransac_counters_d, 0, 4 * sizeof(unsigned long long), ctx->stream)); ISM_HIP(ctx, hipStreamSynchronize(ctx->stream)); }
    return ISMHIP_OK;
}

int ismhip_timer_get(ismhip_ctx* ctx, const char* name, double* ms_out, int64_t* launches_out) {
    if (!ctx || !name) return ISMHIP_ERR_INVALID;
    resolve_timers(ctx);
    if (std::strcmp(name, "knn_seed_launches") == 0) { if (ms_out) *ms_out = (double)ctx->knn_seed_launches; if (launches_out) *launches_out = 1; return ISMHIP_OK; }
    if (std::strcmp(name, "knn_binary_launches") == 0) { if (ms_out) *ms_out = (double)ctx->knn_binary_launches; if (launches_out) *launches_out = 1; return ISMHIP_OK; }
    if (std::strcmp(name, "rank_launches") == 0) { if (ms_out) *ms_out = (double)ctx->rank_launches; if (launches_out) *launches_out = 1; return ISMHIP_OK; }
    if (std::strcmp(name, "knn_pca_launches") == 0) { if (ms_out) *ms_out = (double)ctx->knn_pca_launches; if (launches_out) *launches_out = 1; return ISMHIP_OK; }
    if (std::strcmp(name, "knn_threshold_overflow_queries") == 0) { if (ms_out) *ms_out = (double)ctx->knn_thr_overflow; if (launches_out) *launches_out = 1; return ISMHIP_OK; }
    if (std::strcmp(name, "knn_threshold_mfma_launches") == 0) { if (ms_out) *ms_out = (double)ctx->knn_thr_mfma_launches; if (launches_out) *launches_out = 1; return ISMHIP_OK; }
    {
        static const char* const lk[3] = {"knn_large_k_certified_queries", "knn_large_k_retry_queries", "knn_large_k_exact_queries"};
        for (int i = 0; i < 3; ++i)
            if (std::strcmp(name, lk[i]) == 0) { if (ms_out) *ms_out = (double)ctx->knn_lk_stats[i]; if (launches_out) *launches_out = 1; return ISMHIP_OK; }
    }
    {
        static const char* const rs[4] = {"ransac_clusters", "ransac_clusters_kept", "ransac_hypotheses_needed", "ransac_hypotheses_evaluated"};
        for (int i = 0; i < 4; ++i)
            if (std::strcmp(name, rs[i]) == 0) {
                unsigned long long v[4] = {0, 0, 0, 0};
                if (ctx->ransac_counters_d) {
                    ISM_HIP(ctx, hipMemcpyAsync(v, ctx->ransac_counters_d, sizeof(v), hipMemcpyDeviceToHost, ctx->stream));
                    ISM_HIP(ctx, hipStreamSynchronize(ctx->stream));
                }
                if (ms_out) *ms_out = (double)v[i]; if (launches_out) *launches_out = 1; return ISMHIP_OK;
            }
    }
    if (std::strcmp(name, "knn_stage2_list_entries") == 0) { if (ms_out) *ms_out = (double)ctx->knn_stage2_list_entries; if (launches_out) *launches_out = 1; return ISMHIP_OK; }
    if (std::strcmp(name, "knn_stage2_ranged") == 0) { if (ms_out) *ms_out = (double)ctx->knn_stage2_ranged; if (launches_out) *launches_out = 1; return ISMHIP_OK; }
    if (std::strcmp(name, "knn_stage2_queries") == 0) { if (ms_out) *ms_out = (double)ctx->knn_stage2_queries; if (launches_out) *launches_out = 1; return ISMHIP_OK; }
    if (std::strcmp(name, "knn_flagged_queries") == 0 || std::strcmp(name, "knn_flagged_items") == 0) {
        if (ms_out) *ms_out = (double)ctx->knn_stats[name[12] == 'q' ? 0 : 1];
        if (launches_out) *launches_out = 1;
        return ISMHIP_OK;
    }
    auto it = ctx->timers.find(name);
    if (ms_out) *ms_out = it == ctx->timers.end() ? 0.0 : it->second.ms;
    if (launches_out) *launches_out = it == ctx->timers.end() ? 0 : it->second.launches;
    return ISMHIP_OK;
}

}
```

### point-cloud-donkey_amd/csrc/knn.hip

```cpp
#include "knn_internal.h"

namespace {

__device__ __forceinline__ u16 f32_to_bf16_rn(float x) {
    const unsigned u = __float_as_uint(x);
    return (u16)((u + 0x7FFFu + ((u >> 16) & 1u)) >> 16);
}

__global__ void k_split_bf16(const float* __restrict__ src, int n, int dim, int ld, int n_pad, int dim_pad,
                             u16* __restrict__ hi, u16* __restrict__ lo) {
    const size_t i = (size_t)blockIdx.x * blockDim.x + threadIdx.x;
    if (i >= (size_t)n_pad * dim_pad) return;
    const int row = (int)(i / dim_pad), col = (int)(i % dim_pad);
    float x = 0.f;
    if (row < n && col < dim) x = src[(size_t)row * ld + col];
    const u16 h = f32_to_bf16_rn(x);
    const float hf = __uint_as_float((unsigned)h << 16);
    hi[i] = h; lo[i] = f32_to_bf16_rn(x - hf);
}

__global__ void k_absmax(const float* __restrict__ src, int n, int dim, int ld, uint32_t* __restrict__ out_bits) {
    uint32_t m = 0u;
    const size_t tot = (size_t)n * dim;
    if (ld == dim) {
        const size_t n4 = tot >> 2;
        const uint4* s4 = (const uint4*)src;
        for (size_t i = (size_t)blockIdx.x * blockDim.x + threadIdx.x; i < n4; i += (size_t)gridDim.x * blockDim.x) {
            const uint4 v = s4[i];
            const uint32_t a = max(max(v.x & 0x7fffffffu, v.y & 0x7fffffffu), max(v.z & 0x7fffffffu, v.w & 0x7fffffffu));
            m = a > m ? a : m;
        }
        for (size_t i = 4 * n4 + (size_t)blockIdx.x * blockDim.x + threadIdx.x; i < tot; i += (size_t)gridDim.x * blockDim.x) {
            const uint32_t b = __float_as_uint(src[i]) & 0x7fffffffu; m = b > m ? b : m;
        }
    } else
    for (size_t i = (size_t)blockIdx.x * blockDim.x + threadIdx.x; i < tot; i += (size_t)gridDim.x * blockDim.x) {
        const int row = (int)(i / dim), col = (int)(i % dim);
        const uint32_t b = __float_as_uint(src[(size_t)row * ld + col]) & 0x7fffffffu;
        m = b > m ? b : m;
    }
    __shared__ uint32_t s_m[4];
    m = block_max_u32(m, s_m);
    if (threadIdx.x == 0 && m) atomicMax(out_bits, m);
}
__device__ __forceinline__ float f16_image_scalars(uint32_t* __restrict__ sc, float other_scale, size_t i) {
    const float s = f16_scale_for(sc[0]);
    if (i == 0) {
        ((float*)sc)[1] = -2.0f / (s * other_scale);
        ((float*)sc)[2] = (sc[0] >> 23) == 255u ? __builtin_inff() : F16_FLUSH / s;
    }
    return s;
}
__device__ __forceinline__ u16 f16_image_element(const float* __restrict__ src, int n, int dim, int ld, size_t row, int col, float s) {
    float x = 0.f;
    if (row < (size_t)n && col < dim) x = src[row * ld + col];
    const _Float16 hx = (_Float16)(x * s);
    return __builtin_bit_cast(u16, hx);
}
__global__ void k_to_f16(const float* __restrict__ src, int n, int dim, int ld, int n_pad, int dim_pad,
                         uint32_t* __restrict__ sc, float other_scale, u16* __restrict__ dst) {
    const size_t i = (size_t)blockIdx.x * blockDim.x + threadIdx.x;
    const float s = f16_image_scalars(sc, other_scale, i);
    if (i >= (size_t)n_pad * dim_pad) return;
    dst[i] = f16_image_element(src, n, dim, ld, i / dim_pad, (int)(i % dim_pad), s);
}
__global__ void k_to_f16_tiled(const float* __restrict__ src, int n, int dim, int ld, int n_tiles, int nk,
                               uint32_t* __restrict__ sc, float other_scale, u16* __restrict__ dst) {
    const size_t i = (size_t)blockIdx.x * blockDim.x + threadIdx.x;
    const float s = f16_image_scalars(sc, other_scale, i);
    if (i >= f16t_halves(n_tiles, nk)) return;
    const int e = (int)(i & 7), p = (int)((i >> 3) & 3), r = (int)((i / F16T_KB) % F16T_ROWS);
    const size_t blk = i / F16T_BLOCK;
    const int col = (int)(blk % nk) * F16T_KB + ((p ^ f16t_swizzle(r)) << 3) + e;
    dst[i] = f16_image_element(src, n, dim, ld, blk / nk * F16T_ROWS + r, col, s);
}

__global__ void k_scale_norms(const float* __restrict__ norm, int n, const float* __restrict__ out_scale, float* __restrict__ dst) {
    const int i = blockIdx.x * blockDim.x + threadIdx.x;
    if (i < n) dst[i] = norm[i] * (1.0f / out_scale[0]);
}
__global__ void k_pad_rows(const float* __restrict__ src, int n, int dim, float* __restrict__ dst, int dim_pad) {
    const size_t i = (size_t)blockIdx.x * blockDim.x + threadIdx.x;
    if (i >= (size_t)n * dim_pad) return;
    const int row = (int)(i / dim_pad), col = (int)(i % dim_pad);
    dst[i] = col < dim ? src[(size_t)row * dim + col] : 0.f;
}

__global__ void k_sqrt_rows(const float* __restrict__ src, int n, int dim, int ld, int dim_pad, float* __restrict__ dst, uint32_t* __restrict__ flag) {
    const size_t i = (size_t)blockIdx.x * blockDim.x + threadIdx.x;
    bool bad = false;
    if (i < (size_t)n * dim_pad) {
        const int row = (int)(i / dim_pad), col = (int)(i % dim_pad);
        float v = 0.f;
        if (col < dim) { v = src[(size_t)row * ld + col]; bad = !(v >= 0.f); }
        dst[i] = sqrtf(v);
    }
    if (__any(bad) && (threadIdx.x & 63) == 0) atomicOr(flag, 1u);
}

__global__ void k_ratio(int nq, float thr, const int32_t* __restrict__ idx2, const float* __restrict__ d2,
                        int32_t* __restrict__ idx_out, float* __restrict__ dist_out) {
    const int i = blockIdx.x * blockDim.x + threadIdx.x;
    if (i >= nq) return;
    int id = idx2[i * 2]; const float a = d2[i * 2], b = d2[i * 2 + 1];
    if (idx2[i * 2 + 1] >= 0 && a / b > thr) id = -1;
    idx_out[i] = id; dist_out[i] = a;
}

__global__ void k_rule(int nq, float thr, const int32_t* __restrict__ idx3, const float* __restrict__ d3, const uint32_t* __restrict__ word_class,
                       int32_t* __restrict__ idx_out, float* __restrict__ dist_out) {
    const int i = blockIdx.x * blockDim.x + threadIdx.x;
    if (i >= nq) return;
    const int i0 = idx3[i * 3], i1 = idx3[i * 3 + 1], i2 = idx3[i * 3 + 2];
    const float a = d3[i * 3], b = d3[i * 3 + 1], c = d3[i * 3 + 2];
    int id = -1; float dd = __builtin_nanf("");
    if (i2 < 0) {
        if (i0 >= 0) { id = i0; dd = a; }
    } else {
        const uint32_t c0 = word_class[i0], c1 = word_class[i1], c2 = word_class[i2];
        if (c0 == c1 && c0 == c2) { id = i0; dd = a; }
        else if (c0 == c1 && c0 != c2) { if (a / c < thr) { id = i0; dd = a; } }
        else if (c0 != c1 && c1 == c2) { if (a / b >= thr) { id = i1; dd = b; } }
        else if (c0 != c1 && c1 != c2) { if (a / b < thr) { id = i0; dd = a; } }
    }
    idx_out[i] = id; dist_out[i] = dd;
}

int knn_carve_scratch(KnnRun& r) {
    const KnnPlan& p = r.p; const size_t nq = (size_t)r.nq, q_items = nq * p.n_bound;
    r.n_cand = p.n_cand; r.n_bound = p.n_bound;
    r.cand_val = (float*)ism_scratch(r.ctx, SCR_KNN_CAND_VAL, nq * (p.n_cand + p.n_bound + (p.merged ? KNN_MERGE_KEEP + 1 : 0)) * sizeof(float));
    r.cand_idx = (int*)ism_scratch(r.ctx, SCR_KNN_CAND_IDX, nq * (p.n_cand + (p.merged ? KNN_MERGE_KEEP : 0)) * sizeof(int));
    r.counters = (uint32_t*)ism_scratch(r.ctx, SCR_KNN_FLAGS, knn_queue_bytes(nq, q_items, r.k));
    if (!r.cand_val || !r.cand_idx || !r.counters) return ISMHIP_ERR_NOMEM;
    r.cand_bound = r.cand_val + nq * p.n_cand; r.qsc = r.counters + KNN_CNT_QSC;
    ISM_HIP(r.ctx, hipMemsetAsync(r.counters, 0, KNN_CNT_WORDS * sizeof(uint32_t), r.ctx->stream));
    r.queue = r.rq->ranged ? *r.rq->ranged->queue : knn_queue_carve(r.counters, nq, q_items);
    return ISMHIP_OK;
}

int knn_query_images(KnnRun& r) {
    ismhip_ctx* ctx = r.ctx; const ismhip_codebook* cb = r.cb; const KnnPlan& p = r.p; const int nq = r.nq;
    if (p.mode != 0 && p.mode != 1) return ISMHIP_OK;
    const bool ring = p.cand == KNN_CAND_RING16;
    const int nq_pad = ring ? (nq + F16T_ROWS - 1) / F16T_ROWS * F16T_ROWS : (nq + p.BN - 1) / p.BN * p.BN;
    const size_t tot = ring ? f16t_halves(nq_pad / F16T_ROWS, p.ring_nk) : (size_t)nq_pad * cb->ld16;
    r.q_hi = (u16*)ism_scratch(ctx, SCR_KNN_QSPLIT, tot * 2 * sizeof(u16));
    if (!r.q_hi) return ISMHIP_ERR_NOMEM;
    r.q_lo = r.q_hi + tot;
    if (p.pca) {
        TimerScope tr(ctx, "knn_rotate");
        const int rc = ism_pca_rotate_queries(ctx, cb, r.PI, r.qq, nq, r.ldq, r.q_hi);
        if (rc != ISMHIP_OK) return rc;
        ++ctx->knn_pca_launches;
    } else if (p.mode == 0) {
        const float* cq = p.hell ? r.rq->hell_q : r.qq; const int cldq = p.hell ? cb->dim_pad : r.ldq;
        hipLaunchKernelGGL(k_absmax, dim3(512), dim3(256), 0, ctx->stream, cq, nq, cb->dim, cldq, r.qsc);
        ISM_CHECK_LAUNCH(ctx, "k_absmax");
        if (ring) hipLaunchKernelGGL(k_to_f16_tiled, dim3((unsigned)((tot + 255) / 256)), dim3(256), 0, ctx->stream, cq, nq, cb->dim, cldq, nq_pad / F16T_ROWS, p.ring_nk, r.qsc, r.xb->f16_scale, r.q_hi);
        else hipLaunchKernelGGL(k_to_f16, dim3((unsigned)((tot + 255) / 256)), dim3(256), 0, ctx->stream, cq, nq, cb->dim, cldq, nq_pad, cb->ld16, r.qsc, r.xb->f16_scale, r.q_hi);
        ISM_CHECK_LAUNCH(ctx, "k_to_f16");
    } else {
        hipLaunchKernelGGL(k_split_bf16, dim3((unsigned)((tot + 255) / 256)), dim3(256), 0, ctx->stream, r.qq, nq, cb->dim, r.ldq, nq_pad, cb->ld16, r.q_hi, r.q_lo);
        ISM_CHECK_LAUNCH(ctx, "k_split_bf16");
    }
    return ISMHIP_OK;
}

int knn_launch_candidates(KnnRun& r) {
    ismhip_ctx* ctx = r.ctx; const ismhip_codebook *cb = r.cb, *xb = r.xb; const KnnPlan& p = r.p; const PcaImage& PI = *r.PI; const int nq = r.nq;
    {
        TimerScope ts(ctx, r.rq->tname ? r.rq->tname : (r.metric == ISMHIP_METRIC_L2SQ ? "knn_l2_mfma" : "knn_chi2"));
        const unsigned grid = 8 * ((p.n_qt + 7) / 8) * p.n_splits;
        KnnCandArgs a{};
        a.n_tiles_m = cb->n_words_pad / p.BM; a.ld = cb->ld16; a.k_steps = p.pca ? PI.m / 16 : (cb->dim + 15) / 16;
        a.qh = r.q_hi; a.ql = r.q_lo; a.nq = nq; a.out_scale = (const float*)(r.qsc + 1);
        a.tiles_per_split = p.tiles_per_split; a.n_splits = p.n_splits;
        a.cand_val = r.cand_val; a.cand_idx = r.cand_idx; a.cand_stride = r.n_cand; a.cand_bound = r.cand_bound; a.bound_stride = r.n_bound;
        a.qrange = p.ranged ? r.rq->ranged->qrange : nullptr;
        int rc = ISMHIP_OK;
        if (p.cand == KNN_CAND_RING16) {
            rc = ism_lds_cap(ctx, p.kern, p.lds_cap);
            if (rc != ISMHIP_OK) return rc;
            a.wh = xb->words_f16t;
            if (p.pca) { a.wh = PI.f16t; a.out_scale = PI.osc; a.word_norm = PI.cn_scaled; }
            else {
                float* cn_scaled = (float*)ism_scratch(ctx, SCR_QNORM2, ((size_t)cb->n_words_pad + 256) * sizeof(float));
                if (!cn_scaled) return ISMHIP_ERR_NOMEM;
                hipLaunchKernelGGL(k_scale_norms, dim3((cb->n_words_pad + 255) / 256), dim3(256), 0, ctx->stream, xb->word_norm, cb->n_words_pad, a.out_scale, cn_scaled);
                ISM_CHECK_LAUNCH(ctx, "k_scale_norms");
                a.word_norm = cn_scaled;
            }
            unsigned int* clock = nullptr;
            if (p.join) {
                clock = (unsigned int*)ism_scratch(ctx, SCR_KNN_CLOCK, 8 * 64 * sizeof(unsigned int));
                if (!clock) return ISMHIP_ERR_NOMEM;
                ISM_HIP(ctx, hipMemsetAsync(clock, 0, 8 * 64 * sizeof(unsigned int), ctx->stream));
            }
            float* thr0 = nullptr;
            float relax = 0.f;
            if (p.prepass || p.seeded) {
                thr0 = (float*)ism_scratch(ctx, SCR_KNN_THR0, (size_t)((nq + 255) / 256 * 256) * sizeof(float));
                if (!thr0) return ISMHIP_ERR_NOMEM;
                if (p.pca) relax = -ctx->knn_pre_gamma * 2.0f * PI.resid2 * (PI.sq * PI.sc * 0.5f);
            }
            if (p.seeded && (rc = knn_seed_thresholds(r, a.out_scale, thr0)) != ISMHIP_OK) return rc;
            rc = knn_ring16_launch(ctx, r.T, p.kern, grid, p.threads, p.lds, a, clock, thr0, p.prepass ? ctx->knn_pre_step : 0, relax);
        } else if (p.cand == KNN_CAND_MFMA16) {
            rc = ism_lds_cap(ctx, p.kern, p.lds_cap);
            if (rc != ISMHIP_OK) return rc;
            a.wh = p.mode == 0 ? xb->words_f16 : xb->words_bf16_hi;
            a.wl = p.mode == 0 ? nullptr : xb->words_bf16_lo;
            a.word_norm = xb->word_norm;
            rc = knn_mfma16_launch(ctx, p.kern, grid, p.threads, p.lds, a, nullptr, nullptr, nullptr, 0);
        } else if (p.cand == KNN_CAND_F32) {
            rc = knn_l2_f32_launch(ctx, r.T, grid, cb, r.qq, nq, r.ldq, p.tiles_per_split, p.n_splits, r.cand_val, r.cand_idx, r.n_cand, r.cand_bound, r.n_bound);
        } else {
            rc = knn_chi2_launch(ctx, r.T, p.n_qt, cb, r.qq, nq, r.ldq, r.counters + KNN_CNT_NEGATIVE, p.tiles_per_split, p.n_splits, r.cand_val, r.cand_idx, r.n_cand, r.cand_bound, r.n_bound);
        }
        if (rc != ISMHIP_OK) return rc;
    }
    return ISMHIP_OK;
}

KnnSlotRows knn_fb_desc(const KnnPlan& p, const ismhip_codebook* cb) { return KnnSlotRows{p.fb_tiles_per_split, cb->n_words_pad / p.BM, p.BM, (int)p.fb_layout, p.n_splits}; }
}

KnnPlan knn_plan(const ismhip_ctx* ctx, const ismhip_codebook* cb, int metric, int nq, int k, int T, const KnnRequest& rq) {
    KnnPlan p{};
    p.hell = rq.hell_q != nullptr && metric == ISMHIP_METRIC_CHI2 && cb->chi_shadow;
    const ismhip_codebook* xb = p.hell ? cb->chi_shadow : cb;
    const bool l2 = p.hell || metric == ISMHIP_METRIC_L2SQ;
    const PcaImage& PI = rq.use_pca == 2 ? cb->pca2 : cb->pca;
    const bool short_dim = cb->dim <= 64 && ctx->knn_mode == 0 && !(rq.use_pca && PI.m > 0);
    p.mode = !l2 ? -1 : (p.hell ? 0 : (short_dim ? 2 : (ctx->knn_mode == 0 && cb->words_f16 ? 0 : (ctx->knn_mode <= 1 && cb->words_bf16_hi ? 1 : 2))));
    const bool use_lp = p.mode == 0 || p.mode == 1;
    p.big_tile = use_lp && nq >= 4096 && cb->n_words_pad >= 4096;
    const bool ring = p.big_tile && p.mode == 0 && xb->words_f16t && (cb->dim + 15) / 16 > 2;
    p.half = ring && (rq.half || ctx->knn_half);
    p.qpanel2 = ring && !p.half && ctx->knn_qpanel2 && rq.use_pca && PI.m > 0 && PI.m <= 160 && !rq.ranged;
    p.pca = rq.use_pca && ring && PI.m > 0;
    p.ring_nk = p.pca ? PI.m / 32 : ((cb->dim + 15) / 16 + 1) / 2;
    p.merged = rq.many_splits && l2 && use_lp && !p.big_tile;
    p.join = ring && ctx->knn_join;
    p.BM = !l2 ? CHI_B : (p.half ? 128 : (p.big_tile ? 256 : KNN_BM));
    p.BN = !l2 ? CHI_B : (p.big_tile ? 256 : KNN_BN);
    p.slots = ring && !p.half ? 8 : 4;
    p.n_qt = (nq + p.BN - 1) / p.BN;
    p.ranged = rq.ranged && l2 && use_lp;
    const int n_mt = (p.ranged ? rq.ranged->rows_max : cb->n_words_pad) / p.BM;
    if (l2) {
        const int max_s = (p.hell ? 64 * KNN_HELL_CPL : 64) / (p.slots * T);
        p.n_splits = std::max(1, std::min(std::min(max_s, n_mt), std::max(p.pca ? 2 : 3, (1024 + p.n_qt - 1) / p.n_qt)));
        if (p.big_tile && p.n_qt >= 512) p.n_splits = std::min(p.n_splits, std::max(1, n_mt / 32));
        if (p.hell) p.n_splits = std::max(1, std::min(std::min(max_s, 8), n_mt / 4));
        if (ctx->knn_splits > 0) p.n_splits = std::max(1, std::min(std::min(max_s, n_mt), ctx->knn_splits));
        if (p.merged) p.n_splits = std::max(1, std::min(n_mt, (1024 + 8 * ((p.n_qt + 7) / 8) - 1) / (8 * ((p.n_qt + 7) / 8))));
        p.cand_per_split = p.slots * T;
    } else {
        const int max_s = 64 / T;
        p.n_splits = std::max(1, std::min(std::min(max_s, n_mt), (2048 + p.n_qt - 1) / p.n_qt));
        if (k > T) p.n_splits = std::max(p.n_splits, std::min(std::min(max_s, n_mt), (2 * k + T - 1) / T));
        p.cand_per_split = T;
    }
    if (p.ranged) p.n_splits = std::max(1, std::min(p.n_splits, rq.ranged->rows_min / p.BM));
    p.tiles_per_split = (n_mt + p.n_splits - 1) / p.n_splits;
    if (!p.ranged) p.n_splits = (n_mt + p.tiles_per_split - 1) / p.tiles_per_split;
    p.n_cand = p.n_splits * p.cand_per_split;
    p.n_bound = l2 ? p.n_splits * p.slots : p.n_splits;
    p.prepass = rq.stage1 && ring && !p.half && ctx->knn_prepass && n_mt >= 128 && !(p.pca && PI.resid2 <= 0.f);
    p.seeded = rq.seed_dk && ring && !p.prepass;
    p.fb_tiles_per_split = p.merged ? n_mt : p.tiles_per_split;
    p.fb_layout = p.merged ? KNN_FB_ALL : (p.half ? KNN_FB_RING_HALF : (ring ? KNN_FB_RING : (p.big_tile ? KNN_FB_TILE256 : KNN_FB_TILE128)));
    p.threads = 256;
    if (!l2) p.cand = KNN_CAND_CHI2;
    else if (!use_lp) p.cand = KNN_CAND_F32;
    else if (ring) {
        p.cand = KNN_CAND_RING16;
        p.threads = p.half ? 256 : 512;
        if (p.half) { p.kern = knn_ring16_kernel(T, 1, 0, 0, p.ranged); p.lds = p.lds_cap = Ring16Lds<1, 0>::total(0); }
        else if (p.qpanel2) { p.kern = knn_ring16_kernel(T, 2, 2); p.lds = Ring16Lds<2, 2>::total(p.ring_nk); p.lds_cap = Ring16Lds<2, 2>::total(160 / 32); }
        else { p.kern = knn_ring16_kernel(T, 2, 0, 0, p.ranged); p.lds = p.lds_cap = Ring16Lds<2, 0>::total(0); }
    } else {
        p.cand = KNN_CAND_MFMA16;
        p.threads = p.big_tile ? 512 : 256;
        p.kern = knn_mfma16_kernel(T, p.mode, p.big_tile);
        p.lds = p.lds_cap = knn_mfma16_lds(p.BM, p.BN, p.mode == 1 ? 32 : 64, p.mode == 1 ? 3 : 1);
    }
    return p;
}

int run_knn(ismhip_ctx* ctx, const ismhip_codebook* cb, int metric, int nq, const float* q, int k, int T, int32_t* idx_out, float* dist_out, const KnnRequest& rq) {
    if (cb->dim_pad / 16 > KNN_FB_MAXJ) return ism_set_err(ctx, ISMHIP_ERR_UNSUPPORTED, "knn: descriptor longer than 1344 not built");
    KnnRun r{};
    r.ctx = ctx; r.cb = cb; r.rq = &rq; r.metric = metric; r.nq = nq; r.k = k; r.T = T;
    r.p = knn_plan(ctx, cb, metric, nq, k, T, rq);
    if (r.p.cand == KNN_CAND_MFMA16 && !r.p.kern) return ism_set_err(ctx, ISMHIP_ERR_UNSUPPORTED, "knn: f16 256x256 tile without the ring not built");
    if (r.p.cand == KNN_CAND_RING16 && !r.p.kern) return ism_set_err(ctx, ISMHIP_ERR_UNSUPPORTED, "knn: ranged ring instance not built for this T");
    r.xb = r.p.hell ? cb->chi_shadow : cb;
    r.PI = rq.use_pca == 2 ? &cb->pca2 : &cb->pca;
    r.qq = q; r.ldq = rq.q_ld ? rq.q_ld : cb->dim;
    if (cb->dim_pad != r.ldq) {
        float* qpad = (float*)ism_scratch(ctx, SCR_QPAD, (size_t)nq * cb->dim_pad * sizeof(float));
        if (!qpad) return ISMHIP_ERR_NOMEM;
        const size_t tot = (size_t)nq * cb->dim_pad;
        hipLaunchKernelGGL(k_pad_rows, dim3((unsigned)((tot + 255) / 256)), dim3(256), 0, ctx->stream, q, nq, cb->dim, qpad, cb->dim_pad);
        ISM_CHECK_LAUNCH(ctx, "k_pad_rows");
        r.qq = qpad; r.ldq = cb->dim_pad;
    }
    int rc = knn_carve_scratch(r);
    if (rc == ISMHIP_OK) rc = knn_query_images(r);
    if (rc == ISMHIP_OK) rc = knn_launch_candidates(r);
    if (rc == ISMHIP_OK) rc = knn_rerank_prove(r, idx_out, dist_out);
    if (rc != ISMHIP_OK) return rc;
    if (rq.stage1) { *rq.stage1 = KnnStage1{r.queue, r.p.n_splits, r.p.slots, r.p.tiles_per_split * r.p.BM}; return ISMHIP_OK; }
    if (rq.ranged) { rq.ranged->queue->desc[rq.ranged->chunk] = knn_fb_desc(r.p, cb); return ISMHIP_OK; }
    r.queue.desc[0] = knn_fb_desc(r.p, cb);
    rc = knn_scan_queue(ctx, cb, metric, k, r.qq, r.ldq, r.queue, nullptr, idx_out, dist_out);
    if (rc != ISMHIP_OK) return rc;
    if (ctx->timers_on) ISM_HIP(ctx, hipMemcpyAsync(ctx->knn_stats, r.counters, 8, hipMemcpyDeviceToHost, ctx->stream));
    return ISMHIP_OK;
}

int knn_sqrt_queries(ismhip_ctx* ctx, const ismhip_codebook* cb, int nq, const float* q, float* sq, bool& negative) {
    uint32_t* flag = (uint32_t*)(sq + (size_t)nq * cb->dim_pad);
    ISM_HIP(ctx, hipMemsetAsync(flag, 0, 4, ctx->stream));
    const size_t tot = (size_t)nq * cb->dim_pad;
    hipLaunchKernelGGL(k_sqrt_rows, dim3((unsigned)((tot + 255) / 256)), dim3(256), 0, ctx->stream, q, nq, cb->dim, cb->dim, cb->dim_pad, sq, flag);
    ISM_CHECK_LAUNCH(ctx, "k_sqrt_rows");
    uint32_t neg = 0;
    ISM_HIP(ctx, hipMemcpyAsync(&neg, flag, 4, hipMemcpyDeviceToHost, ctx->stream));
    ISM_HIP(ctx, hipStreamSynchronize(ctx->stream));
    negative = neg != 0;
    return ISMHIP_OK;
}

int knn_f16_emit_image(ismhip_ctx* ctx, const ismhip_codebook* cb, const ismhip_codebook* xb, const float* qv, int n, int ldv, int n_pad,
                       uint32_t* sc, u16* qimg) {
    hipLaunchKernelGGL(k_absmax, dim3(512), dim3(256), 0, ctx->stream, qv, n, cb->dim, ldv, sc);
    ISM_CHECK_LAUNCH(ctx, "k_absmax");
    const size_t tot = (size_t)n_pad * cb->ld16;
    hipLaunchKernelGGL(k_to_f16, dim3((unsigned)((tot + 255) / 256)), dim3(256), 0, ctx->stream, qv, n, cb->dim, ldv, n_pad, cb->ld16, sc, xb->f16_scale, qimg);
    ISM_CHECK_LAUNCH(ctx, "k_to_f16");
    return ISMHIP_OK;
}

int ism_codebook_split_bf16(ismhip_ctx* ctx, ismhip_codebook* cb, uint32_t absmax_bits) {
    cb->ld16 = (cb->dim + 63) / 64 * 64;
    const size_t tot = (size_t)cb->n_words_pad * cb->ld16;
    if (hipMalloc((void**)&cb->words_bf16_hi, tot * 3 * sizeof(u16) + 16) != hipSuccess) return ism_set_err(ctx, ISMHIP_ERR_NOMEM, "codebook bf16/f16 images");
    cb->words_bf16_lo = cb->words_bf16_hi + tot;
    cb->words_f16 = cb->words_bf16_lo + tot;
    uint32_t* sc = (uint32_t*)(cb->words_f16 + tot);
    hipLaunchKernelGGL(k_split_bf16, dim3((unsigned)((tot + 255) / 256)), dim3(256), 0, ctx->stream, cb->words, cb->n_words_pad, cb->dim_pad, cb->dim_pad,
                       cb->n_words_pad, cb->ld16, cb->words_bf16_hi, cb->words_bf16_lo);
    ISM_CHECK_LAUNCH(ctx, "k_split_bf16");
    cb->f16_scale = f16_scale_for(absmax_bits);
    ISM_HIP(ctx, hipMemcpyAsync(sc, &absmax_bits, 4, hipMemcpyHostToDevice, ctx->stream));
    hipLaunchKernelGGL(k_to_f16, dim3((unsigned)((tot + 255) / 256)), dim3(256), 0, ctx->stream, cb->words, cb->n_words_pad, cb->dim_pad, cb->dim_pad,
                       cb->n_words_pad, cb->ld16, sc, 1.0f, cb->words_f16);
    ISM_CHECK_LAUNCH(ctx, "k_to_f16");
    {
        const int nk = ((cb->dim + 15) / 16 + 1) / 2, n_tiles = cb->n_words_pad / F16T_ROWS;
        const size_t tt = f16t_halves(n_tiles, nk);
        if (hipMalloc((void**)&cb->words_f16t, tt * sizeof(u16)) != hipSuccess) return ism_set_err(ctx, ISMHIP_ERR_NOMEM, "codebook tiled f16 image");
        hipLaunchKernelGGL(k_to_f16_tiled, dim3((unsigned)((tt + 255) / 256)), dim3(256), 0, ctx->stream, cb->words, cb->n_words_pad, cb->dim_pad, cb->dim_pad,
                           n_tiles, nk, sc, 1.0f, cb->words_f16t);
        ISM_CHECK_LAUNCH(ctx, "k_to_f16_tiled");
    }
    ISM_HIP(ctx, hipStreamSynchronize(ctx->stream));
    return ISMHIP_OK;
}

extern "C" {

int ismhip_knn(ismhip_ctx* ctx, const ismhip_codebook* cb, int metric, int nq, const float* q, int k,
               int32_t* idx_out, float* dist_out) {
    if (!ctx || !cb || !q || !idx_out || !dist_out || nq < 0 || k <= 0 || (metric != ISMHIP_METRIC_L2SQ && metric != ISMHIP_METRIC_CHI2))
        return ism_set_err(ctx, ISMHIP_ERR_INVALID, "knn: bad argument");
    if (k > KNN_MAX_K) return ism_set_err(ctx, ISMHIP_ERR_UNSUPPORTED, "knn: k > 16 not built");
    if (nq == 0) return ISMHIP_OK;
    TimerScope ts(ctx, "knn");
    const bool wide = k > 2 || (metric == ISMHIP_METRIC_L2SQ && cb->words_bf16_hi && ctx->knn_mode <= 1 && !(cb->dim <= 64 && ctx->knn_mode == 0));
    if (metric == ISMHIP_METRIC_L2SQ && k <= 2 && ctx->knn_t == 0 && ctx->knn_mode == 0 && ctx->knn_two_stage && cb->words_f16t && nq >= 4096 &&
        cb->n_words_pad >= 4096 && (cb->dim > 64 || cb->pca.m > 0))
        return run_knn_two_stage(ctx, cb, nq, q, k, idx_out, dist_out);
    if (metric == ISMHIP_METRIC_CHI2 && cb->chi_shadow && ctx->knn_hellinger && knn_matrix_gate(ctx, cb, nq)) {
        bool taken = false;
        const int rc = run_knn_chi2_hellinger(ctx, cb, nq, q, k, idx_out, dist_out, taken);
        if (rc != ISMHIP_OK || taken) return rc;
    }
    const bool forced = ctx->knn_t >= 1 && ctx->knn_t <= 3 && k <= ctx->knn_t;
    return run_knn(ctx, cb, metric, nq, q, k, forced ? ctx->knn_t : (wide ? 4 : 2), idx_out, dist_out);
}

int ismhip_knn_ratio(ismhip_ctx* ctx, const ismhip_codebook* cb, int metric, int nq, const float* q,
                     float ratio_threshold, int32_t* idx_out, float* dist_out) {
    if (!ctx || !cb || !q || !idx_out || !dist_out || nq < 0) return ism_set_err(ctx, ISMHIP_ERR_INVALID, "knn_ratio: bad argument");
    if (nq == 0) return ISMHIP_OK;
    int32_t* idx2 = (int32_t*)ism_scratch(ctx, SCR_QNORM, (size_t)nq * 2 * (sizeof(int32_t) + sizeof(float)));
    if (!idx2) return ISMHIP_ERR_NOMEM;
    float* d2 = (float*)(idx2 + (size_t)nq * 2);
    int rc = ismhip_knn(ctx, cb, metric, nq, q, 2, idx2, d2);
    if (rc != ISMHIP_OK) return rc;
    hipLaunchKernelGGL(k_ratio, dim3((nq + 255) / 256), dim3(256), 0, ctx->stream, nq, ratio_threshold, idx2, d2, idx_out, dist_out);
    ISM_CHECK_LAUNCH(ctx, "k_ratio");
    return ISMHIP_OK;
}

int ismhip_knn_rule(ismhip_ctx* ctx, const ismhip_codebook* cb, int metric, int nq, const float* q,
                    float ratio_threshold, int32_t* idx_out, float* dist_out) {
    if (!ctx || !cb || !q || !idx_out || !dist_out || nq < 0) return ism_set_err(ctx, ISMHIP_ERR_INVALID, "knn_rule: bad argument");
    if (nq == 0) return ISMHIP_OK;
    int32_t* idx3 = (int32_t*)ism_scratch(ctx, SCR_QNORM, (size_t)nq * 3 * (sizeof(int32_t) + sizeof(float)));
    if (!idx3) return ISMHIP_ERR_NOMEM;
    float* d3 = (float*)(idx3 + (size_t)nq * 3);
    int rc = ismhip_knn(ctx, cb, metric, nq, q, 3, idx3, d3);
    if (rc != ISMHIP_OK) return rc;
    hipLaunchKernelGGL(k_rule, dim3((nq + 255) / 256), dim3(256), 0, ctx->stream, nq, ratio_threshold, idx3, d3, cb->word_class, idx_out, dist_out);
    ISM_CHECK_LAUNCH(ctx, "k_rule");
    return ISMHIP_OK;
}

}
```

### point-cloud-donkey_amd/csrc/knn_internal.h

```cpp
#pragma once
#include "common.h"

namespace {

typedef float f32x16 __attribute__((ext_vector_type(16)));
typedef float f32x4 __attribute__((ext_vector_type(4)));
typedef __bf16 bf16x8 __attribute__((ext_vector_type(8)));
typedef unsigned short u16;
typedef _Float16 f16x8 __attribute__((ext_vector_type(8)));
#include "functor.h"

#define KNN_BM 128
#define KNN_BN 128
#define CHI_B 64
#define KNN_MAX_K 16
#define KNN_FB_MAXJ 84
#define KNN_TERMS (16 * KNN_FB_MAXJ)

template <int T>
struct TopT {
    float v[T]; int i[T];
    __device__ __forceinline__ void init() {
#pragma unroll
        for (int t = 0; t < T; ++t) { v[t] = __builtin_inff(); i[t] = -1; }
    }
    __device__ __forceinline__ void push_flat(float x, int idx) {
        bool c[T];
#pragma unroll
        for (int t = 0; t < T; ++t) c[t] = x < v[t];
#pragma unroll
        for (int t = T - 1; t > 0; --t) {
            v[t] = c[t - 1] ? v[t - 1] : (c[t] ? x : v[t]);
            i[t] = c[t - 1] ? i[t - 1] : (c[t] ? idx : i[t]);
        }
        v[0] = c[0] ? x : v[0];
        i[0] = c[0] ? idx : i[0];
    }
    __device__ __forceinline__ void push(float x, int idx) {
        if (!(x < v[T - 1])) return;
        v[T - 1] = x; i[T - 1] = idx;
#pragma unroll
        for (int t = T - 1; t > 0; --t) {
            if (v[t] < v[t - 1]) {
                float tv = v[t]; v[t] = v[t - 1]; v[t - 1] = tv;
                int ti = i[t]; i[t] = i[t - 1]; i[t - 1] = ti;
            }
        }
    }
};

constexpr size_t knn_mfma16_lds(int BM, int BN, int KB, int NTERM) { return (size_t)2 * (BM + BN) * KB * sizeof(u16) * (NTERM == 3 ? 2 : 1) + BM * sizeof(float); }
#define RG_BN 256
#define RG_KB 32
template <int WR, int QP>
struct Ring16Lds {
    static constexpr int STAGES = WR == 2 ? 4 : 3, STAGE_HALVES = (QP ? WR * 128 : WR * 128 + RG_BN) * RG_KB;
    static constexpr size_t cn = (size_t)STAGES * STAGE_HALVES * sizeof(u16);
    static constexpr size_t thr = cn + 4 * 256 * sizeof(float);
    static constexpr size_t panel = thr + (WR == 2 ? 8 * 4 * 64 * sizeof(float) : 0);
    static constexpr size_t total(int ring_nk) { return panel + (QP ? (size_t)ring_nk * 256 * RG_KB * sizeof(u16) : 0); }
};

#define F16_FLUSH 6.103515625e-05f
__host__ __device__ inline float f16_scale_for(uint32_t bits) {
    const int e = (int)(bits >> 23);
    if (e == 0 || e == 255) return 1.0f;
    int k = 13 - (e - 127);
    k = k > 40 ? 40 : (k < -40 ? -40 : k);
    return __builtin_bit_cast(float, (uint32_t)(127 + k) << 23);
}
#define F16T_ROWS 256
#define F16T_KB 32
#define F16T_BLOCK (F16T_ROWS * F16T_KB)
__host__ __device__ inline size_t f16t_halves(size_t n_tiles, int nk) { return n_tiles * nk * F16T_BLOCK; }
__device__ __forceinline__ int f16t_swizzle(int r) { return (0x78 >> (2 * ((r >> 2) & 3))) & 3; }
__device__ __forceinline__ size_t f16t_row(size_t tile, int r, int nk, int kc) { return ((tile * nk + kc) * F16T_ROWS + r) * F16T_KB; }
__device__ __forceinline__ size_t f16t_stored(unsigned row, int nk, unsigned h) { return f16t_row(row / F16T_ROWS, row % F16T_ROWS, nk, h / F16T_KB) + h % F16T_KB; }

struct VerifyParams {
    float ku;
    float dot_rel;
    float cmax2;
    float dabs_c;
    const float* dabs_q;
    float sqrt_dim;
    float cn_acc;
};
__device__ __forceinline__ float knn_abs_err(const VerifyParams& vp, float qn2) {
    if (!vp.dabs_q) return 0.f;
    const float dq = vp.dabs_q[0], dc = vp.dabs_c;
    return 1.01f * (vp.sqrt_dim * (dq * sqrtf(vp.cmax2) + dc * sqrtf(qn2)) + vp.sqrt_dim * vp.sqrt_dim * dq * dc);
}
#define KNN_U 5.9604645e-08f
__device__ __forceinline__ float knn_eps_s_raw(const VerifyParams& vp, float qn2) {
    return 17.f * KNN_U * vp.cmax2 + (2.f * vp.dot_rel + 2.f * KNN_U) * sqrtf(qn2 * vp.cmax2) + 2.f * knn_abs_err(vp, qn2) + vp.cn_acc * vp.cmax2;
}
__device__ __forceinline__ float knn_eps_s(const VerifyParams& vp, float qn2) { return knn_eps_s_raw(vp, qn2) * 1.00001f; }
__device__ __forceinline__ float wave_norm2(const float* __restrict__ x, int dim, int lane) {
    float s = 0.f;
    for (int i = lane; i < dim; i += 64) { const float v = x[i]; s += v * v; }
    return wave_sum_f(s);
}

VerifyParams knn_verify_params(const ismhip_codebook* xb, int dim_pad, int mode, const uint32_t* qsc, bool cn_acc) {
    VerifyParams vp;
    vp.ku = 1.01f * (float)dim_pad * KNN_U;
    vp.dot_rel = mode == 0 ? (2.002f * 4.8828125e-04f + 1.01f * (float)dim_pad * 1.1920929e-07f)
               : mode == 1 ? (3.1f * 1.52587890625e-05f + 1.01f * 3.f * (float)dim_pad * 1.1920929e-07f) : vp.ku;
    vp.cmax2 = xb->max_norm2;
    vp.dabs_c = mode == 0 ? F16_FLUSH / xb->f16_scale : 0.f;
    vp.dabs_q = mode == 0 ? (const float*)(qsc + 2) : nullptr;
    vp.sqrt_dim = sqrtf((float)dim_pad);
    vp.cn_acc = mode == 0 && cn_acc ? 1.01f * (float)(dim_pad + 1) * 1.1920929e-07f : 0.f;
    return vp;
}

__device__ __forceinline__ float thr_tau_of(float thr, float qn2, int dim, const VerifyParams& vp) {
    const float eps_s = knn_eps_s(vp, qn2);
    float t = thr * (1.f + 2.f * vp.ku) - qn2 * (1.f - 16.f * KNN_U) + eps_s + 8.f * KNN_U * (qn2 + vp.cmax2 + thr)
            + (float)(dim / 64 + 8) * KNN_U * qn2;
    if (!(fabsf(t) < __builtin_inff())) t = __builtin_inff();
    return t;
}

__device__ __forceinline__ bool knn_l2_slot_proven(float dk, float bnd, float qn2, const VerifyParams& vp) {
    const float eps_s = knn_eps_s_raw(vp, qn2);
    const float rhs = qn2 * (1.f - 16.f * KNN_U) + bnd - eps_s;
    return dk < rhs - vp.ku * fabsf(rhs) - 1e-37f;
}
struct PcaLb { float qn2h, eps_s, dlt, inv_sig2; };
__device__ __forceinline__ float pca_lb_of(const PcaLb& b, float s) {
    float L = b.qn2h * (1.f - 16.f * KNN_U) + s - b.eps_s;
    L -= 4.f * KNN_U * (b.qn2h + fabsf(s));
    if (!(L > 0.f)) return 0.f;
    const float t = sqrtf(L) * (1.f - 4.f * KNN_U) - b.dlt;
    if (!(t > 0.f)) return 0.f;
    return t * t * b.inv_sig2 * (1.f - 8.f * KNN_U);
}
__device__ __forceinline__ bool pca_slot_proven(float dk, float bnd, const PcaLb& b, float ku) { return dk < pca_lb_of(b, bnd) * (1.f - ku) - 1e-37f; }

#define CHI_FAST_CH 6
__device__ __forceinline__ void chi2_fast_load_q(const float* __restrict__ qp, int n4, int lane, f32x4* qv) {
#pragma unroll
    for (int j = 0; j < CHI_FAST_CH; ++j) { const int g = lane + 64 * j; qv[j] = g < n4 ? *(const f32x4*)(qp + 4 * g) : f32x4{0.f, 0.f, 0.f, 0.f}; }
}
__device__ __forceinline__ float chi2_fast(const f32x4* qv, const float* __restrict__ wp, int n4, int lane) {
    f32x4 wv[CHI_FAST_CH];
#pragma unroll
    for (int j = 0; j < CHI_FAST_CH; ++j) { const int g = lane + 64 * j; wv[j] = g < n4 ? *(const f32x4*)(wp + 4 * g) : f32x4{0.f, 0.f, 0.f, 0.f}; }
    float part = 0.f;
#pragma unroll
    for (int j = 0; j < CHI_FAST_CH; ++j)
#pragma unroll
        for (int e = 0; e < 4; ++e) { const float sm = qv[j][e] + wv[j][e], df = qv[j][e] - wv[j][e]; part += sm > 0.f ? df * df / sm : 0.f; }
    return wave_sum_f(part);
}
#define KNN_MERGE_KEEP 16
#define KNN_HELL_CPL 4
enum KnnCounter {
    KNN_CNT_QUERIES = 0, KNN_CNT_ITEMS = 1,
    KNN_CNT_QSC = 4,
    KNN_CNT_NEGATIVE = 12,
    KNN_CNT_WORDS = 16
};

bool knn_matrix_gate(const ismhip_ctx* ctx, const ismhip_codebook* cb, int nq) {
    return ctx->knn_mode == 0 && ctx->knn_t == 0 && nq >= 256 && cb->n_words >= 1024 && cb->dim % 4 == 0;
}

}

enum KnnFbLayout { KNN_FB_TILE128 = 64, KNN_FB_TILE256 = 128, KNN_FB_RING = -1, KNN_FB_ALL = -2, KNN_FB_RING_HALF = -3 };
struct KnnSlotRows { int tiles_per_split, n_tiles, tile_rows, wr_rows, n_splits; };
struct KnnQueue { uint32_t *count, *qrec, *items; unsigned long long* item_out; size_t q_items; KnnSlotRows desc[2]; };
struct KnnStage1 { KnnQueue queue; int n_splits, slots, rows_per_split; };
struct KnnRanged { const int* qrange; const uint32_t* live; KnnQueue* queue; int q_base, chunk, rows_min, rows_max; const float* known_dk; };
struct KnnRequest {
    KnnStage1* stage1 = nullptr;
    const char* tname = nullptr;
    bool many_splits = false;
    int use_pca = 0;
    const float* hell_q = nullptr;
    bool half = false;
    const float* seed_dk = nullptr;
    const KnnRanged* ranged = nullptr;
    int q_ld = 0;
};
enum KnnCand { KNN_CAND_F32, KNN_CAND_CHI2, KNN_CAND_MFMA16, KNN_CAND_RING16 };
struct KnnPlan {
    bool hell;
    int mode;
    KnnCand cand;
    const void* kern;
    int BM, BN, threads;
    bool big_tile, half, qpanel2, pca, merged, prepass, seeded, join, ranged;
    int slots, ring_nk;
    int n_qt, n_splits, tiles_per_split, cand_per_split, n_cand, n_bound;
    int fb_tiles_per_split; KnnFbLayout fb_layout;
    size_t lds, lds_cap;
};
struct KnnRun {
    ismhip_ctx* ctx; const ismhip_codebook *cb, *xb; const PcaImage* PI; const KnnRequest* rq; KnnPlan p;
    int metric, nq, k, T;
    const float* qq; int ldq;
    u16 *q_hi, *q_lo;
    float *cand_val, *cand_bound; int* cand_idx; int n_cand, n_bound;
    uint32_t *counters, *qsc;
    KnnQueue queue;
};

KnnPlan knn_plan(const ismhip_ctx* ctx, const ismhip_codebook* cb, int metric, int nq, int k, int T, const KnnRequest& rq);
int run_knn(ismhip_ctx* ctx, const ismhip_codebook* cb, int metric, int nq, const float* q, int k, int T, int32_t* idx_out, float* dist_out, const KnnRequest& rq = KnnRequest());
int knn_sqrt_queries(ismhip_ctx* ctx, const ismhip_codebook* cb, int nq, const float* q, float* sq, bool& negative);
int knn_f16_emit_image(ismhip_ctx* ctx, const ismhip_codebook* cb, const ismhip_codebook* xb, const float* qv, int n, int ldv, int n_pad,
                       uint32_t* sc, u16* qimg);
int ism_pca_rotate_queries(ismhip_ctx* ctx, const ismhip_codebook* cb, const PcaImage* P, const float* q, int nq, int ldq, unsigned short* dst);
int knn_seed_thresholds(KnnRun& r, const float* out_scale, float* thr0);
int knn_rerank_prove(KnnRun& r, int32_t* idx_out, float* dist_out);
size_t knn_queue_bytes(size_t n_queries, size_t q_items, int k);
KnnQueue knn_queue_carve(void* mem, size_t n_queries, size_t q_items);
int knn_scan_queue(ismhip_ctx* ctx, const ismhip_codebook* cb, int metric, int k, const float* q, int ldq, const KnnQueue& Q, const int* qrange, int32_t* idx_out, float* dist_out);
int run_knn_two_stage(ismhip_ctx* ctx, const ismhip_codebook* cb, int nq, const float* q, int k, int32_t* idx_out, float* dist_out);
int run_knn_chi2_hellinger(ismhip_ctx* ctx, const ismhip_codebook* cb, int nq, const float* q, int k, int32_t* idx_out, float* dist_out, bool& taken);

struct KnnCandArgs {
    const u16 *wh, *wl; const float* word_norm; int n_tiles_m, ld, k_steps;
    const u16 *qh, *ql; int nq; const float* out_scale; int tiles_per_split, n_splits;
    float* cand_val; int* cand_idx; int cand_stride; float* cand_bound; int bound_stride;
    const int* qrange;
};
__host__ __device__ inline void knn_range_split(int lo, int hi, int split, int n_splits, int& mt0, int& mt1) {
    const long long len = hi - lo;
    mt0 = lo + (int)(len * split / n_splits); mt1 = lo + (int)(len * (split + 1) / n_splits);
}
const void* knn_ring16_kernel(int T, int WR, int QP, int PRE = 0, int RNG = 0);
int knn_ring16_launch(ismhip_ctx* ctx, int T, const void* kern, unsigned grid, int threads, size_t lds, KnnCandArgs a,
                      unsigned int* stream_clock, float* thr0, int pre_step, float pre_relax);
const void* knn_mfma16_kernel(int T, int mode, bool big_tile);
int knn_mfma16_launch(ismhip_ctx* ctx, const void* kern, unsigned grid, int threads, size_t lds, KnnCandArgs a,
                      const float* emit_tau, uint32_t* emit_cnt, uint32_t* emit_list, int emit_cap);
int knn_mfma16_emit(ismhip_ctx* ctx, const ismhip_codebook* cb, const ismhip_codebook* xb, int n, int n_pad, const uint32_t* sc, const u16* qimg,
                    const float* tau, uint32_t* emit_cnt, uint32_t* rows, int cap);

int knn_l2_f32_launch(ismhip_ctx* ctx, int T, unsigned grid, const ismhip_codebook* cb, const float* q, int nq, int ldq, int tiles_per_split, int n_splits,
                      float* cand_val, int* cand_idx, int n_cand, float* cand_bound, int n_bound);
int knn_chi2_launch(ismhip_ctx* ctx, int T, int n_qt, const ismhip_codebook* cb, const float* q, int nq, int ldq, uint32_t* q_negative, int tiles_per_split, int n_splits,
                    float* cand_val, int* cand_idx, int n_cand, float* cand_bound, int n_bound);
```

### point-cloud-donkey_amd/csrc/knn_rerank.hip

```cpp
#include "knn_internal.h"

namespace {

__device__ __forceinline__ unsigned knn_sortable(float f) { const unsigned u = __float_as_uint(f); return (u & 0x80000000u) ? ~u : (u | 0x80000000u); }
__global__ __launch_bounds__(256) void k_knn_merge_splits(int nq, const float* __restrict__ cand_val, const int* __restrict__ cand_idx, int n_cand,
                                                          const float* __restrict__ cand_bound, int n_bound,
                                                          float* __restrict__ out_val, int* __restrict__ out_idx, float* __restrict__ out_bound) {
    const int qi = blockIdx.x * 4 + (threadIdx.x >> 6);
    if (qi >= nq) return;
    const int lane = lane_id();
    const float* v = cand_val + (size_t)qi * n_cand; const int* id = cand_idx + (size_t)qi * n_cand;
    unsigned long long prev = 0ull;
    bool first = true;
    float dropped = __builtin_inff();
    for (int r = 0; r <= KNN_MERGE_KEEP; ++r) {
        unsigned long long best = ~0ull;
        for (int i = lane; i < n_cand; i += 64) {
            if (id[i] < 0) continue;
            const unsigned long long key = ((unsigned long long)knn_sortable(v[i]) << 32) | (unsigned)i;
            if ((first || key > prev) && key < best) best = key;
        }
        best = wave_min_u64(best);
        if (r < KNN_MERGE_KEEP) {
            if (lane == 0) {
                const bool have = best != ~0ull;
                const int i = have ? (int)(best & 0xffffffffull) : 0;
                out_val[(size_t)qi * KNN_MERGE_KEEP + r] = have ? v[i] : __builtin_inff();
                out_idx[(size_t)qi * KNN_MERGE_KEEP + r] = have ? id[i] : -1;
            }
        } else if (best != ~0ull) dropped = v[(int)(best & 0xffffffffull)];
        if (best == ~0ull) { for (int rr = r + 1; rr < KNN_MERGE_KEEP; ++rr) if (lane == 0) { out_val[(size_t)qi * KNN_MERGE_KEEP + rr] = __builtin_inff(); out_idx[(size_t)qi * KNN_MERGE_KEEP + rr] = -1; } break; }
        prev = best; first = false;
    }
    float b = dropped;
    for (int i = lane; i < n_bound; i += 64) { const float x = cand_bound[(size_t)qi * n_bound + i]; if (x < b || x != x) b = x; }
#pragma unroll
    for (int o = 32; o > 0; o >>= 1) { const float x = __shfl_xor(b, o, 64); if (x < b || x != x) b = x; }
    if (lane == 0) out_bound[qi] = b;
}

__device__ __forceinline__ int knn_load_cand(const int* __restrict__ cand_idx, const float* __restrict__ cand_val, int qi, int cand_stride,
                                             int j, int n_cand, int n_words, float& av) {
    int id = -1; av = __builtin_inff();
    if (j < n_cand) { id = cand_idx[(size_t)qi * cand_stride + j]; av = cand_val[(size_t)qi * cand_stride + j]; }
    if (!(id >= 0 && id < n_words)) { id = -1; av = __builtin_inff(); }
    return id;
}
template <int CPL>
__device__ __forceinline__ bool knn_select_write(unsigned long long* key, int qi, int k, int lane, int32_t* __restrict__ idx_out, float* __restrict__ dist_out, float& dk) {
    bool have_k = true;
    dk = 0.f;
    for (int j = 0; j < k; ++j) {
        unsigned long long lm = key[0];
#pragma unroll
        for (int c = 1; c < CPL; ++c) lm = key[c] < lm ? key[c] : lm;
        const unsigned long long mn = wave_min_u64(lm);
        if (lane == 0) {
            if (mn == ~0ull) { idx_out[(size_t)qi * k + j] = -1; dist_out[(size_t)qi * k + j] = __builtin_nanf(""); }
            else { idx_out[(size_t)qi * k + j] = (int)(mn & 0xffffffffull); dist_out[(size_t)qi * k + j] = __uint_as_float((unsigned)(mn >> 32)); }
        }
        if (mn == ~0ull) have_k = false; else dk = __uint_as_float((unsigned)(mn >> 32));
#pragma unroll
        for (int c = 0; c < CPL; ++c) if (key[c] == mn) key[c] = ~0ull;
    }
    return have_k;
}
struct KnnQueueTag { const uint32_t* live; int q_base, slot_tag; const float* known_dk; };
__device__ __forceinline__ bool knn_is_padding(const KnnQueueTag& tg, int qi) { return tg.live && tg.live[qi] == ~0u; }
__device__ __forceinline__ bool knn_proof_dk(const KnnQueueTag& tg, int qi, bool have_k, float& dk) {
    if (tg.known_dk) { const float U = tg.known_dk[qi]; if (U == U) { dk = have_k ? fminf(dk, U) : U; return true; } }
    return have_k;
}
__device__ __forceinline__ void knn_queue_unproven(bool viol, int qi, int lane, uint32_t* __restrict__ flag_count, uint32_t* __restrict__ qrec, uint32_t* __restrict__ items, const KnnQueueTag& tg) {
    const unsigned long long vmask = __ballot(viol);
    if (vmask != 0ull) {
        const int nv = __popcll(vmask);
        uint32_t ibase = 0;
        if (lane == 0) {
            const uint32_t qs = atomicAdd(&flag_count[KNN_CNT_QUERIES], 1u);
            ibase = atomicAdd(&flag_count[KNN_CNT_ITEMS], (uint32_t)nv);
            qrec[3 * (size_t)qs] = (uint32_t)(qi + tg.q_base); qrec[3 * (size_t)qs + 1] = ibase; qrec[3 * (size_t)qs + 2] = (uint32_t)nv;
        }
        ibase = __shfl(ibase, 0, 64);
        if (viol) {
            const uint32_t it = ibase + __popcll(vmask & ((1ull << lane) - 1ull));
            items[2 * (size_t)it] = (uint32_t)(qi + tg.q_base); items[2 * (size_t)it + 1] = (uint32_t)(lane | tg.slot_tag);
        }
    }
}

__global__ __launch_bounds__(256) void k_knn_rerank(const float* __restrict__ words, int dim, int dim_pad, int n_words,
                                                    const float* __restrict__ q, int nq, int ldq, int metric,
                                                    const int* __restrict__ cand_idx, const float* __restrict__ cand_val, int cand_stride, int n_cand,
                                                    const float* __restrict__ cand_bound, int n_bound, VerifyParams vp,
                                                    int k, int32_t* __restrict__ idx_out, float* __restrict__ dist_out,
                                                    uint32_t* __restrict__ flag_count, uint32_t* __restrict__ qrec, uint32_t* __restrict__ items, KnnQueueTag tg) {
    const int qi = blockIdx.x * 4 + (threadIdx.x >> 6);
    if (qi >= nq || knn_is_padding(tg, qi)) return;
    const int lane = lane_id();
    const float* qp = q + (size_t)qi * ldq;
    const float qn2 = wave_norm2(qp, dim, lane);
    float av;
    const int id = knn_load_cand(cand_idx, cand_val, qi, cand_stride, lane, n_cand, n_words, av);
    float kth = av;
    {
        float cur = av;
        for (int j = 0; j < k; ++j) {
            const float mn = wave_min_f(cur);
            kth = mn;
            const unsigned long long eq = __ballot(cur == mn);
            if (eq && lane == __ffsll((long long)eq) - 1) cur = __builtin_inff();
        }
    }
    float slack;
    if (metric == ISMHIP_METRIC_CHI2) slack = 4.f * (((float)dim_pad + 8.f) * KNN_U + vp.ku) * fabsf(kth);
    else slack = 2.f * knn_eps_s_raw(vp, qn2) + 4.f * vp.ku * (qn2 + fabsf(kth) + vp.cmax2);
    unsigned long long key = ~0ull;
    {
        __shared__ __attribute__((aligned(16))) float s_terms[4][KNN_TERMS];
        float* sT = s_terms[threadIdx.x >> 6];
        unsigned long long need = __ballot(id >= 0 && !(av > kth + slack));
        while (need) {
            const int src = __ffsll((long long)need) - 1; need &= need - 1;
            const int cid = __shfl(id, src, 64);
            const float d = wave_functor(metric, qp, words + (size_t)cid * dim_pad, dim, lane, sT);
            if (lane == src) key = ((unsigned long long)__float_as_uint(d) << 32) | (unsigned)id;
        }
    }
    float bnd = __builtin_inff();
    if (lane < n_bound) bnd = cand_bound[(size_t)qi * n_bound + lane];
    float dk;
    const bool have_k = knn_proof_dk(tg, qi, knn_select_write<1>(&key, qi, k, lane, idx_out, dist_out, dk), dk);
    bool viol = false;
    const float eps_chk = metric == ISMHIP_METRIC_CHI2 ? qn2 + vp.cmax2 : knn_eps_s_raw(vp, qn2) + qn2;
    if (lane < n_bound && (bnd != __builtin_inff() || !(eps_chk < __builtin_inff()))) {
        if (!have_k) viol = true;
        else if (metric == ISMHIP_METRIC_CHI2) {
            const float lo = bnd * (1.f - ((float)dim_pad + 8.f) * KNN_U) * (1.f - vp.ku);
            viol = !(dk < lo);
        } else viol = !knn_l2_slot_proven(dk, bnd, qn2, vp);
    }
    knn_queue_unproven(viol, qi, lane, flag_count, qrec, items, tg);
}

struct PcaVerify {
    const u16* qimg; int nk;
    float inv_sq2;
    float inv_sig2, d_rel, dq_abs, dc;
    float eps_c2, dot2, cmax2;
    float ku;
};
__device__ __forceinline__ PcaLb pca_lb_query(const PcaVerify& pv, int qi, float qn2, int lane) {
    float qn2h = 0.f;
    for (int i = lane; i < pv.nk * F16T_KB; i += 64) {
        const float v = (float)__builtin_bit_cast(_Float16, pv.qimg[f16t_stored(qi, pv.nk, i)]);
        qn2h += v * v;
    }
    PcaLb b;
    b.qn2h = wave_sum_f(qn2h) * pv.inv_sq2;
    b.dlt = pv.d_rel * (sqrtf(qn2) * 1.00001f) + pv.dq_abs + pv.dc;
    b.eps_s = (pv.eps_c2 + pv.dot2 * sqrtf(b.qn2h * pv.cmax2)) * 1.00001f;
    b.inv_sig2 = pv.inv_sig2;
    return b;
}
__global__ __launch_bounds__(256) void k_knn_rerank_pca(const float* __restrict__ words, int dim, int dim_pad, int n_words,
                                                        const float* __restrict__ q, int nq, int ldq,
                                                        const int* __restrict__ cand_idx, const float* __restrict__ cand_val, int cand_stride, int n_cand,
                                                        const float* __restrict__ cand_bound, int n_bound, PcaVerify pv,
                                                        int k, int32_t* __restrict__ idx_out, float* __restrict__ dist_out,
                                                        uint32_t* __restrict__ flag_count, uint32_t* __restrict__ qrec, uint32_t* __restrict__ items, KnnQueueTag tg) {
    const int qi = blockIdx.x * 4 + (threadIdx.x >> 6);
    if (qi >= nq || knn_is_padding(tg, qi)) return;
    const int lane = lane_id();
    const float* qp = q + (size_t)qi * ldq;
    const PcaLb lbq = pca_lb_query(pv, qi, wave_norm2(qp, dim, lane), lane);
    float av;
    const int id = knn_load_cand(cand_idx, cand_val, qi, cand_stride, lane, n_cand, n_words, av);
    const float lb = id >= 0 ? pca_lb_of(lbq, av) : __builtin_inff();
    bool done = id < 0;
    unsigned long long key = ~0ull;
    {
        __shared__ __attribute__((aligned(16))) float s_terms[4][KNN_TERMS];
        float* sT = s_terms[threadIdx.x >> 6];
        float kth = __builtin_inff(); int n_eval = 0;
        for (;;) {
            const float cur = done ? __builtin_inff() : lb;
            const float mn = wave_min_f(cur);
            if (!(mn < __builtin_inff())) break;
            if (n_eval >= k && mn * (1.f - pv.ku) > kth) break;
            const unsigned long long eq = __ballot(!done && cur == mn);
            const int src = __ffsll((long long)eq) - 1;
            const int cid = __shfl(id, src, 64);
            const float d = wave_functor(ISMHIP_METRIC_L2SQ, qp, words + (size_t)cid * dim_pad, dim, lane, sT);
            if (lane == src) { key = ((unsigned long long)__float_as_uint(d) << 32) | (unsigned)id; done = true; }
            if (++n_eval >= k) {
                unsigned long long kk = key, m_ = ~0ull;
                for (int j = 0; j < k; ++j) { m_ = wave_min_u64(kk); if (kk == m_) kk = ~0ull; }
                kth = __uint_as_float((unsigned)(m_ >> 32));
            }
        }
    }
    float bnd = __builtin_inff();
    if (lane < n_bound) bnd = cand_bound[(size_t)qi * n_bound + lane];
    float dk;
    const bool have_k = knn_proof_dk(tg, qi, knn_select_write<1>(&key, qi, k, lane, idx_out, dist_out, dk), dk);
    bool viol = false;
    if (lane < n_bound && (bnd != __builtin_inff() || !(lbq.eps_s + lbq.qn2h + lbq.dlt < __builtin_inff()))) {
        if (!have_k) viol = true;
        else viol = !pca_slot_proven(dk, bnd, lbq, pv.ku);
    }
    knn_queue_unproven(viol, qi, lane, flag_count, qrec, items, tg);
}

__global__ __launch_bounds__(256) void k_knn_seed_thr(const float* __restrict__ q, int nq, int ldq, int dim, const float* __restrict__ seed_dk,
                                                      bool pca, PcaVerify pv, VerifyParams vp, const float* __restrict__ out_scale, float* __restrict__ thr,
                                                      const uint32_t* __restrict__ live ) {
    const int qi = blockIdx.x * 4 + (threadIdx.x >> 6);
    if (qi >= nq) return;
    if (live && live[qi] == ~0u) { if (lane_id() == 0) thr[qi] = __builtin_inff(); return; }
    const int lane = lane_id();
    const float qn2 = wave_norm2(q + (size_t)qi * ldq, dim, lane);
    PcaLb lbq{};
    if (pca) lbq = pca_lb_query(pv, qi, qn2, lane);
    if (lane != 0) return;
    const float U = seed_dk[qi], osc = out_scale[0];
    float t0 = -__builtin_inff();
    if (U >= 0.f && U < __builtin_inff()) {
        float s, step;
        if (pca) {
            const float t = sqrtf((U + 1e-37f) / (lbq.inv_sig2 * (1.f - 8.f * KNN_U) * (1.f - pv.ku))) * (1.f + 4.f * KNN_U);
            const float rl = (t + lbq.dlt) / (1.f - 4.f * KNN_U);
            s = rl * rl * (1.f + 8.f * KNN_U) + lbq.eps_s - lbq.qn2h * (1.f - 16.f * KNN_U);
            step = 4.f * KNN_U * (lbq.qn2h + fabsf(s) + lbq.eps_s);
        } else {
            s = thr_tau_of(U, qn2, dim, vp);
            step = 4.f * KNN_U * (qn2 + fabsf(s) + vp.cmax2);
        }
        s += step;
        for (int it = 0; it < 24 && s < __builtin_inff(); ++it, s += step, step *= 2.f) {
            const float a = s / osc;
            if (pca ? pca_slot_proven(U, osc * a, lbq, pv.ku) : knn_l2_slot_proven(U, osc * a, qn2, vp)) { t0 = a; break; }
        }
    }
    thr[qi] = t0;
}

__global__ __launch_bounds__(256) void k_knn_rerank_hell(const float* __restrict__ words, int dim, int dim_pad, int n_words,
                                                         const float* __restrict__ q, int nq, int ldq, const float* __restrict__ sq ,
                                                         const uint32_t* __restrict__ perm ,
                                                         const int* __restrict__ cand_idx, const float* __restrict__ cand_val, int cand_stride, int n_cand,
                                                         const float* __restrict__ cand_bound, int n_bound, VerifyParams vp,
                                                         int k, int32_t* __restrict__ idx_out, float* __restrict__ dist_out,
                                                         uint32_t* __restrict__ flag_count, uint32_t* __restrict__ qrec, uint32_t* __restrict__ items, KnnQueueTag tg) {
    const int qi = blockIdx.x * 4 + (threadIdx.x >> 6);
    if (qi >= nq || knn_is_padding(tg, qi)) return;
    const int lane = lane_id();
    const float* qp = q + (size_t)qi * ldq;
    const float qn2 = wave_norm2(sq + (size_t)qi * dim_pad, dim, lane);
    const float eps_s = knn_eps_s(vp, qn2);
    auto lb_of = [&](float s) -> float {
        float L = qn2 * (1.f - 16.f * KNN_U) + s - eps_s;
        L -= 4.f * KNN_U * (qn2 + fabsf(s));
        return L > 0.f ? L : 0.f;
    };
    int id[KNN_HELL_CPL]; float lb[KNN_HELL_CPL], fd[KNN_HELL_CPL]; unsigned long long key[KNN_HELL_CPL];
#pragma unroll
    for (int c = 0; c < KNN_HELL_CPL; ++c) {
        float av;
        const int x = knn_load_cand(cand_idx, cand_val, qi, cand_stride, lane + 64 * c, n_cand, n_words, av);
        id[c] = -1; lb[c] = __builtin_inff(); fd[c] = __builtin_inff(); key[c] = ~0ull;
        if (x >= 0) { id[c] = (int)perm[x]; lb[c] = lb_of(av); }
    }
    const float mg = 4.f * vp.ku;
    float kth_fast = __builtin_inff();
    {
        const int n4 = (ldq >= dim_pad ? dim_pad : dim) >> 2;
        f32x4 qv[CHI_FAST_CH];
        chi2_fast_load_q(qp, n4, lane, qv);
        int n_eval = 0;
        for (;;) {
            float cur = lb[0];
#pragma unroll
            for (int c = 1; c < KNN_HELL_CPL; ++c) cur = fminf(cur, lb[c]);
            const float mn = wave_min_f(cur);
            if (!(mn < __builtin_inff())) break;
            if (n_eval >= k && mn * (1.f - vp.ku) > kth_fast * (1.f + mg)) break;
            const unsigned long long eq = __ballot(cur == mn);
            const int src = __ffsll((long long)eq) - 1;
            int mine = -1, cs = 0;
#pragma unroll
            for (int c = KNN_HELL_CPL - 1; c >= 0; --c) if (lb[c] == mn) { mine = id[c]; cs = c; }
            const int cid = __shfl(mine, src, 64);
            float d = chi2_fast(qv, words + (size_t)cid * dim_pad, n4, lane);
            if (d != d) d = 0.f;
            if (lane == src) {
#pragma unroll
                for (int c = 0; c < KNN_HELL_CPL; ++c) if (c == cs) { fd[c] = d; lb[c] = __builtin_inff(); }
            }
            if (++n_eval >= k) {
                float ff[KNN_HELL_CPL], m_ = __builtin_inff();
#pragma unroll
                for (int c = 0; c < KNN_HELL_CPL; ++c) ff[c] = fd[c];
                for (int j = 0; j < k; ++j) {
                    float lm = ff[0];
#pragma unroll
                    for (int c = 1; c < KNN_HELL_CPL; ++c) lm = fminf(lm, ff[c]);
                    m_ = wave_min_f(lm);
                    const unsigned long long e2 = __ballot(lm == m_);
                    if (lane == __ffsll((long long)e2) - 1) {
                        bool gone = false;
#pragma unroll
                        for (int c = 0; c < KNN_HELL_CPL; ++c) if (!gone && ff[c] == m_) { ff[c] = __builtin_inff(); gone = true; }
                    }
                }
                kth_fast = m_;
            }
        }
    }
    {
        __shared__ __attribute__((aligned(16))) float s_terms[4][KNN_TERMS];
        float* sT = s_terms[threadIdx.x >> 6];
        const float win = kth_fast * (1.f + 3.f * mg);
        for (;;) {
            int mine = -1, cs = 0;
#pragma unroll
            for (int c = KNN_HELL_CPL - 1; c >= 0; --c) if (fd[c] <= win && key[c] == ~0ull && id[c] >= 0) { mine = id[c]; cs = c; }
            const unsigned long long pend = __ballot(mine >= 0);
            if (pend == 0ull) break;
            const int src = __ffsll((long long)pend) - 1;
            const int cid = __shfl(mine, src, 64);
            const float d = wave_functor(ISMHIP_METRIC_CHI2, qp, words + (size_t)cid * dim_pad, dim, lane, sT);
            if (lane == src) {
#pragma unroll
                for (int c = 0; c < KNN_HELL_CPL; ++c) if (c == cs) { key[c] = ((unsigned long long)__float_as_uint(d) << 32) | (unsigned)id[c]; fd[c] = __builtin_inff(); }
            }
        }
    }
    float bnd = __builtin_inff();
    if (lane < n_bound) bnd = cand_bound[(size_t)qi * n_bound + lane];
    float dk;
    const bool have_k = knn_select_write<KNN_HELL_CPL>(key, qi, k, lane, idx_out, dist_out, dk);
    bool viol = false;
    if (lane < n_bound && (bnd != __builtin_inff() || !(eps_s + qn2 < __builtin_inff()))) {
        if (!have_k) viol = true;
        else viol = !(dk < lb_of(bnd) * (1.f - vp.ku) - 1e-37f);
    }
    knn_queue_unproven(viol, qi, lane, flag_count, qrec, items, tg);
}

PcaVerify knn_pca_verify(const KnnRun& r, const VerifyParams& vp) {
    const PcaImage& PI = *r.PI;
    PcaVerify pv;
    const float acc_rel = 1.01f * (float)PI.m * 1.1920929e-07f;
    pv.qimg = r.q_hi; pv.nk = r.p.ring_nk; pv.inv_sq2 = 1.0f / (PI.sq * PI.sq);
    pv.inv_sig2 = PI.inv_sig2; pv.d_rel = PI.d_rel; pv.dq_abs = PI.dq_abs;
    pv.dc = (PI.d_rel * sqrtf(r.cb->max_norm2) + PI.dc_abs) * 1.00001f;
    pv.cmax2 = PI.cmax2;
    const float fq = F16_FLUSH / PI.sq, fc = F16_FLUSH / PI.sc, sm = sqrtf((float)PI.m);
    pv.eps_c2 = (17.f * KNN_U + 1.01f * (float)(PI.m + 1) * 1.1920929e-07f) * PI.cmax2 + 2.02f * (sm * fq * sqrtf(PI.cmax2) + sm * sm * fq * fc);
    pv.dot2 = 2.f * acc_rel + 2.f * KNN_U + 2.02f * sm * fc / sqrtf(PI.cmax2);
    pv.ku = vp.ku;
    return pv;
}

KnnQueueTag knn_queue_tag(const KnnRanged* g) { return g ? KnnQueueTag{g->live, g->q_base, g->chunk << 8, g->known_dk} : KnnQueueTag{nullptr, 0, 0, nullptr}; }

}

int knn_seed_thresholds(KnnRun& r, const float* out_scale, float* thr0) {
    ismhip_ctx* ctx = r.ctx; const ismhip_codebook* cb = r.cb; const KnnPlan& p = r.p;
    const VerifyParams vp = knn_verify_params(r.xb, cb->dim_pad, p.mode, r.qsc, true);
    hipLaunchKernelGGL(k_knn_seed_thr, dim3((r.nq + 3) / 4), dim3(256), 0, ctx->stream, r.qq, r.nq, r.ldq, cb->dim, r.rq->seed_dk,
                       p.pca, p.pca ? knn_pca_verify(r, vp) : PcaVerify{}, vp, out_scale, thr0, knn_queue_tag(r.rq->ranged).live);
    ISM_CHECK_LAUNCH(ctx, "k_knn_seed_thr");
    ++ctx->knn_seed_launches;
    return ISMHIP_OK;
}

int knn_rerank_prove(KnnRun& r, int32_t* idx_out, float* dist_out) {
    ismhip_ctx* ctx = r.ctx; const ismhip_codebook* cb = r.cb; const KnnPlan& p = r.p; const KnnQueue& Q = r.queue;
    const VerifyParams vp = knn_verify_params(r.xb, cb->dim_pad, p.mode, r.qsc, true);
    const dim3 grid((r.nq + 3) / 4), block(256);
    const KnnQueueTag tg = knn_queue_tag(r.rq->ranged);
    if (p.merged) {
        float* m_val = r.cand_bound + (size_t)r.nq * r.n_bound; float* m_bound = m_val + (size_t)r.nq * KNN_MERGE_KEEP;
        int* m_idx = r.cand_idx + (size_t)r.nq * r.n_cand;
        hipLaunchKernelGGL(k_knn_merge_splits, grid, block, 0, ctx->stream, r.nq, r.cand_val, r.cand_idx, r.n_cand, r.cand_bound, r.n_bound, m_val, m_idx, m_bound);
        ISM_CHECK_LAUNCH(ctx, "k_knn_merge_splits");
        r.cand_val = m_val; r.cand_idx = m_idx; r.cand_bound = m_bound; r.n_cand = KNN_MERGE_KEEP; r.n_bound = 1;
    }
    TimerScope trr(ctx, "knn_rerank");
    if (p.pca) {
        const PcaVerify pv = knn_pca_verify(r, vp);
        hipLaunchKernelGGL(k_knn_rerank_pca, grid, block, 0, ctx->stream, cb->words, cb->dim, cb->dim_pad, cb->n_words,
                           r.qq, r.nq, r.ldq, r.cand_idx, r.cand_val, r.n_cand, r.n_cand, r.cand_bound, r.n_bound, pv, r.k, idx_out, dist_out, Q.count, Q.qrec, Q.items, tg);
    } else if (p.hell) {
        hipLaunchKernelGGL(k_knn_rerank_hell, grid, block, 0, ctx->stream, cb->words, cb->dim, cb->dim_pad, cb->n_words,
                           r.qq, r.nq, r.ldq, r.rq->hell_q, r.xb->shadow_perm, r.cand_idx, r.cand_val, r.n_cand, r.n_cand, r.cand_bound, r.n_bound, vp, r.k, idx_out, dist_out, Q.count, Q.qrec, Q.items, tg);
    } else
    hipLaunchKernelGGL(k_knn_rerank, grid, block, 0, ctx->stream, cb->words, cb->dim, cb->dim_pad, cb->n_words,
                       r.qq, r.nq, r.ldq, r.metric, r.cand_idx, r.cand_val, r.n_cand, r.n_cand, r.cand_bound, r.n_bound, vp, r.k, idx_out, dist_out, Q.count, Q.qrec, Q.items, tg);
    ISM_CHECK_LAUNCH(ctx, "k_knn_rerank");
    return ISMHIP_OK;
}
```

### point-cloud-donkey_amd/csrc/pca.hip

```cpp
#include "knn_internal.h"
#include <cmath>
#include <algorithm>
#include <numeric>

namespace {

#define SM_ROWS 64
__global__ __launch_bounds__(256) void k_second_moment(const float* __restrict__ w, int n_rows, int ld, int rows_per_chunk, int nb, float* __restrict__ part) {
    __shared__ float sA[SM_ROWS][33], sB[SM_ROWS][33];
    int bi = 0, rem = blockIdx.x;
    while (rem >= nb - bi) { rem -= nb - bi; ++bi; }
    const int bj = bi + rem;
    const int tx = threadIdx.x & 15, ty = threadIdx.x >> 4;
    const int r_beg = blockIdx.y * rows_per_chunk, r_end = min(n_rows, r_beg + rows_per_chunk);
    float a00 = 0.f, a01 = 0.f, a10 = 0.f, a11 = 0.f;
    for (int r0 = r_beg; r0 < r_end; r0 += SM_ROWS) {
        __syncthreads();
        for (int e = threadIdx.x; e < SM_ROWS * 32; e += 256) {
            const int rr = e >> 5, c = e & 31, r = r0 + rr;
            sA[rr][c] = r < r_end ? w[(size_t)r * ld + bi * 32 + c] : 0.f;
            sB[rr][c] = r < r_end ? w[(size_t)r * ld + bj * 32 + c] : 0.f;
        }
        __syncthreads();
#pragma unroll 8
        for (int rr = 0; rr < SM_ROWS; ++rr) {
            const float x0 = sA[rr][2 * ty], x1 = sA[rr][2 * ty + 1], y0 = sB[rr][2 * tx], y1 = sB[rr][2 * tx + 1];
            a00 = fmaf(x0, y0, a00); a01 = fmaf(x0, y1, a01); a10 = fmaf(x1, y0, a10); a11 = fmaf(x1, y1, a11);
        }
    }
    const int dimp = nb * 32;
    float* o = part + (size_t)blockIdx.y * dimp * dimp;
    o[(size_t)(bi * 32 + 2 * ty) * dimp + bj * 32 + 2 * tx] = a00;     o[(size_t)(bi * 32 + 2 * ty) * dimp + bj * 32 + 2 * tx + 1] = a01;
    o[(size_t)(bi * 32 + 2 * ty + 1) * dimp + bj * 32 + 2 * tx] = a10; o[(size_t)(bi * 32 + 2 * ty + 1) * dimp + bj * 32 + 2 * tx + 1] = a11;
}

#define ROT_LD 36
template <int NT>
__global__ __launch_bounds__(256, 2) void k_rotate_f16t(const float* __restrict__ x, int n, int ldx, int kdim,
                                                         const float* __restrict__ rmat, int m, float scale, u16* __restrict__ dst) {
    extern __shared__ __attribute__((aligned(16))) float rot_smem[];
    float* sX = rot_smem;
    float* sR = rot_smem + 128 * ROT_LD;
    const int tid = threadIdx.x, lane = tid & 63, wv = tid >> 6;
    const int r32 = lane & 31, h = lane >> 5;
    const int nct = m >> 5;
    const size_t row0 = (size_t)blockIdx.x * 128;
    f32x16 acc[NT];
#pragma unroll
    for (int t = 0; t < NT; ++t)
#pragma unroll
        for (int e = 0; e < 16; ++e) acc[t][e] = 0.f;
    const int srow = tid >> 3, scol = (tid & 7) * 4;
    for (int k0 = 0; k0 < kdim; k0 += 32) {
        __syncthreads();
#pragma unroll
        for (int i = 0; i < 4; ++i) {
            size_t r = row0 + srow + 32 * i; r = r < (size_t)n ? r : (size_t)n - 1;
            *(f32x4*)(sX + (srow + 32 * i) * ROT_LD + scol) = *(const f32x4*)(x + r * ldx + k0 + scol);
        }
#pragma unroll
        for (int i = 0; i < NT; ++i)
            if (i < nct) *(f32x4*)(sR + (srow + 32 * i) * ROT_LD + scol) = *(const f32x4*)(rmat + (size_t)(srow + 32 * i) * kdim + k0 + scol);
        __syncthreads();
        f32x4 fb[4];
        const float* pb = sX + (wv * 32 + r32) * ROT_LD + h * 16;
#pragma unroll
        for (int v = 0; v < 4; ++v) fb[v] = *(const f32x4*)(pb + 4 * v);
#pragma unroll
        for (int t = 0; t < NT; ++t) {
            if (t >= nct) continue;
            f32x4 fa[4];
            const float* pa = sR + (t * 32 + r32) * ROT_LD + h * 16;
#pragma unroll
            for (int v = 0; v < 4; ++v) fa[v] = *(const f32x4*)(pa + 4 * v);
#pragma unroll
            for (int v = 0; v < 4; ++v)
#pragma unroll
                for (int e = 0; e < 4; ++e) acc[t] = __builtin_amdgcn_mfma_f32_32x32x2f32(fa[v][e], fb[v][e], acc[t], 0, 0, 0);
        }
    }
    const size_t row = row0 + wv * 32 + r32;
    const size_t n_img = ((size_t)n + F16T_ROWS - 1) / F16T_ROWS * F16T_ROWS;
    if (row >= n_img) return;
    const bool live = row < (size_t)n;
    const size_t tile = row / F16T_ROWS; const int r = (int)(row % F16T_ROWS);
    const int fsw = f16t_swizzle(r);
#pragma unroll
    for (int t = 0; t < NT; ++t) {
        if (t >= nct) continue;
        u16* base = dst + f16t_row(tile, r, nct, t) + 4 * h;
#pragma unroll
        for (int j = 0; j < 4; ++j) {
            union { _Float16 hf[4]; uint2 u; } pk;
#pragma unroll
            for (int e = 0; e < 4; ++e) pk.hf[e] = live ? (_Float16)(acc[t][4 * j + e] * scale) : (_Float16)0.f;
            *(uint2*)(base + ((j ^ fsw) << 3)) = pk.u;
        }
    }
}

__global__ __launch_bounds__(256) void k_f16t_norms(const u16* __restrict__ img, int n_rows_pad, int n_rows, int nk, float cn_factor,
                                                    float* __restrict__ sumsq, float* __restrict__ cn) {
    const int row = blockIdx.x * 4 + (threadIdx.x >> 6);
    if (row >= n_rows_pad) return;
    const int lane = lane_id();
    float s = 0.f;
    for (int i = lane; i < nk * F16T_KB; i += 64) {
        const float v = (float)__builtin_bit_cast(_Float16, img[f16t_stored(row, nk, i)]);
        s += v * v;
    }
    s = wave_sum_f(s);
    if (lane == 0) {
        if (sumsq) sumsq[row] = s;
        cn[row] = row < n_rows ? -s * cn_factor : -__builtin_inff();
    }
}

void jacobi_eig(int n, std::vector<double>& A, std::vector<double>& V, std::vector<double>& w) {
    V.assign((size_t)n * n, 0.0);
    for (int i = 0; i < n; ++i) V[(size_t)i * n + i] = 1.0;
    for (int sweep = 0; sweep < 30; ++sweep) {
        double off = 0, diag = 0;
        for (int i = 0; i < n; ++i) { diag += A[(size_t)i * n + i] * A[(size_t)i * n + i]; for (int j = i + 1; j < n; ++j) off += A[(size_t)i * n + j] * A[(size_t)i * n + j]; }
        if (!(off > 1e-18 * diag)) break;
        for (int p = 0; p < n - 1; ++p) for (int q = p + 1; q < n; ++q) {
            const double apq = A[(size_t)p * n + q];
            if (std::fabs(apq) < 1e-300) continue;
            const double theta = (A[(size_t)q * n + q] - A[(size_t)p * n + p]) / (2.0 * apq);
            const double t = (theta >= 0 ? 1.0 : -1.0) / (std::fabs(theta) + std::sqrt(theta * theta + 1.0));
            const double c = 1.0 / std::sqrt(t * t + 1.0), s = t * c;
            double* Ap = &A[(size_t)p * n]; double* Aq = &A[(size_t)q * n];
            for (int k = 0; k < n; ++k) { const double x = Ap[k], y = Aq[k]; Ap[k] = c * x - s * y; Aq[k] = s * x + c * y; }
            for (int k = 0; k < n; ++k) { double* r = &A[(size_t)k * n]; const double x = r[p], y = r[q]; r[p] = c * x - s * y; r[q] = s * x + c * y; }
            double* Vp = &V[(size_t)p * n]; double* Vq = &V[(size_t)q * n];
            for (int k = 0; k < n; ++k) { const double x = Vp[k], y = Vq[k]; Vp[k] = c * x - s * y; Vq[k] = s * x + c * y; }
        }
    }
    w.resize(n);
    for (int i = 0; i < n; ++i) w[i] = A[(size_t)i * n + i];
}

int launch_rotate(ismhip_ctx* ctx, const float* x, int n, int ldx, int kdim, const float* rmat, int m, float scale, u16* dst) {
    const int nct = m / 32;
    const void* kern = nct <= 4 ? (const void*)k_rotate_f16t<4> : nct <= 6 ? (const void*)k_rotate_f16t<6> : (const void*)k_rotate_f16t<8>;
    const int nt = nct <= 4 ? 4 : nct <= 6 ? 6 : 8;
    const size_t lds = (size_t)(128 + nt * 32) * ROT_LD * sizeof(float);
    { const int rc = ism_lds_cap(ctx, kern, lds); if (rc != ISMHIP_OK) return rc; }
    const unsigned blocks = (unsigned)((((size_t)n + 255) / 256 * 256) / 128);
    void* args[] = {&x, &n, &ldx, &kdim, &rmat, &m, &scale, &dst};
    ISM_HIP(ctx, hipLaunchKernel(kern, dim3(blocks), dim3(256), args, lds, ctx->stream));
    ISM_CHECK_LAUNCH(ctx, "k_rotate_f16t");
    return ISMHIP_OK;
}

}

int ism_pca_rotate_queries(ismhip_ctx* ctx, const ismhip_codebook* cb, const PcaImage* P, const float* q, int nq, int ldq, unsigned short* dst) {
    return launch_rotate(ctx, q, nq, ldq, cb->dim_pad, P->R, P->m, P->sq, dst);
}

static int build_image(ismhip_ctx* ctx, ismhip_codebook* cb, PcaImage& P, const std::vector<float>& R, int m, double energy, double trace) {
    const int dp = cb->dim_pad;
    P.m = 0;
    double e2 = 0, fro2 = 0;
    for (int i = 0; i < m; ++i) for (int j = i; j < m; ++j) {
        double g = 0; for (int c = 0; c < dp; ++c) g += (double)R[(size_t)i * dp + c] * (double)R[(size_t)j * dp + c];
        if (i == j) { fro2 += g; if (g != 0.0) { g -= 1.0; e2 += g * g; } } else e2 += 2.0 * g * g;
    }
    const double sig2 = 1.0 + std::sqrt(e2), sig = std::sqrt(sig2), fro = std::sqrt(fro2);
    if (!(sig2 < 1.01)) return ISMHIP_OK;
    const double cmax = std::sqrt((double)cb->max_norm2);
    P.sc = f16_scale_for(__builtin_bit_cast(uint32_t, (float)(1.001 * sig * cmax)));
    P.sq = f16_scale_for(__builtin_bit_cast(uint32_t, (float)(2.002 * sig * cmax)));
    const double gamma = 1.01 * dp * 1.1920929e-07;
    P.d_rel = (float)(1.001 * (gamma * fro + 4.8828125e-04 * (sig + gamma * fro)));
    P.dq_abs = (float)(1.001 * std::sqrt((double)m) * (double)F16_FLUSH / P.sq);
    P.dc_abs = (float)(1.001 * std::sqrt((double)m) * (double)F16_FLUSH / P.sc);
    P.inv_sig2 = (float)((1.0 / sig2) * (1.0 - 1e-6));
    P.energy = (float)energy;
    P.resid2 = (float)((1.0 - energy) * trace / (double)cb->n_words);
    const int nk = m / F16T_KB, n_tiles = cb->n_words_pad / F16T_ROWS;
    if (hipMalloc((void**)&P.R, R.size() * sizeof(float)) != hipSuccess) return ism_set_err(ctx, ISMHIP_ERR_NOMEM, "codebook rotation matrix");
    ISM_HIP(ctx, hipMemcpy(P.R, R.data(), R.size() * sizeof(float), hipMemcpyHostToDevice));
    if (hipMalloc((void**)&P.f16t, f16t_halves(n_tiles, nk) * sizeof(u16)) != hipSuccess) return ism_set_err(ctx, ISMHIP_ERR_NOMEM, "codebook rotated f16 image");
    if (hipMalloc((void**)&P.cn_scaled, ((size_t)cb->n_words_pad + 256) * sizeof(float) + 16) != hipSuccess) return ism_set_err(ctx, ISMHIP_ERR_NOMEM, "codebook rotated norms");
    P.osc = P.cn_scaled + cb->n_words_pad + 256;
    P.m = m;
    int rc = launch_rotate(ctx, cb->words, cb->n_words_pad, dp, dp, P.R, m, P.sc, P.f16t);
    if (rc != ISMHIP_OK) { P.m = 0; return rc; }
    float* sumsq_d = (float*)ism_scratch(ctx, SCR_PCA, (size_t)cb->n_words_pad * sizeof(float));
    if (!sumsq_d) { P.m = 0; return ISMHIP_ERR_NOMEM; }
    ISM_HIP(ctx, hipMemsetAsync(P.cn_scaled, 0, ((size_t)cb->n_words_pad + 256) * sizeof(float), ctx->stream));
    const float cn_factor = P.sq / (2.0f * P.sc);
    hipLaunchKernelGGL(k_f16t_norms, dim3((cb->n_words_pad + 3) / 4), dim3(256), 0, ctx->stream, P.f16t, cb->n_words_pad, cb->n_words, nk, cn_factor, sumsq_d, P.cn_scaled);
    ISM_CHECK_LAUNCH(ctx, "k_f16t_norms");
    std::vector<float> ss(cb->n_words);
    ISM_HIP(ctx, hipMemcpyAsync(ss.data(), sumsq_d, (size_t)cb->n_words * sizeof(float), hipMemcpyDeviceToHost, ctx->stream));
    const float osc = -2.0f / (P.sq * P.sc);
    ISM_HIP(ctx, hipMemcpyAsync(P.osc, &osc, sizeof(float), hipMemcpyHostToDevice, ctx->stream));
    ISM_HIP(ctx, hipStreamSynchronize(ctx->stream));
    float mx = 0.f;
    for (float v : ss) mx = v > mx || v != v ? v : mx;
    P.cmax2 = mx / (P.sc * P.sc) * 1.00001f;
    if (!(P.cmax2 < 1e30f)) P.m = 0;
    return ISMHIP_OK;
}

int ism_codebook_build_pca(ismhip_ctx* ctx, ismhip_codebook* cb) {
    cb->pca.m = 0; cb->pca2.m = 0;
    const int dp = cb->dim_pad;
    if (ctx->knn_pca_m == 0 || !cb->words_f16t || dp < 64 || cb->n_words_pad < 4096 || (dp > 512 && ctx->knn_pca_m < 0)) return ISMHIP_OK;
    if (!(cb->max_norm2 > 0.f) || !(cb->max_norm2 < 1e30f)) return ISMHIP_OK;
    const bool identity = dp <= 64;
    std::vector<float> R;
    std::vector<double> w_sorted, V_sorted;
    int m = 0; double energy = 1.0, trace = 0.0;
    if (identity) {
        m = dp;
        R.assign((size_t)m * dp, 0.f);
        for (int j = 0; j < cb->dim; ++j) R[(size_t)j * dp + j] = 1.f;
        std::vector<float> nh(cb->n_words);
        ISM_HIP(ctx, hipMemcpy(nh.data(), cb->word_norm, (size_t)cb->n_words * 4, hipMemcpyDeviceToHost));
        for (float v : nh) trace += v;
    } else {
    const int nb = dp / 32, n_pairs = nb * (nb + 1) / 2;
    const int n_chunks = std::max(1, std::min(64, cb->n_words / 1024));
    const int rows_per_chunk = (cb->n_words + n_chunks - 1) / n_chunks;
    const size_t pbytes = (size_t)n_chunks * dp * dp * sizeof(float);
    float* part_d = (float*)ism_scratch(ctx, SCR_PCA, pbytes);
    if (!part_d) return ISMHIP_ERR_NOMEM;
    ISM_HIP(ctx, hipMemsetAsync(part_d, 0, pbytes, ctx->stream));
    hipLaunchKernelGGL(k_second_moment, dim3(n_pairs, n_chunks), dim3(256), 0, ctx->stream, cb->words, cb->n_words, dp, rows_per_chunk, nb, part_d);
    ISM_CHECK_LAUNCH(ctx, "k_second_moment");
    std::vector<float> part((size_t)n_chunks * dp * dp);
    ISM_HIP(ctx, hipMemcpyAsync(part.data(), part_d, pbytes, hipMemcpyDeviceToHost, ctx->stream));
    ISM_HIP(ctx, hipStreamSynchronize(ctx->stream));
    std::vector<double> S((size_t)dp * dp, 0.0), V, w;
    for (int c = 0; c < n_chunks; ++c)
        for (int i = 0; i < dp; ++i)
            for (int j = i / 32 * 32; j < dp; ++j) S[(size_t)i * dp + j] += (double)part[((size_t)c * dp + i) * dp + j];
    for (int i = 0; i < dp; ++i) for (int j = i + 1; j < dp; ++j) { const double v = i / 32 == j / 32 ? 0.5 * (S[(size_t)i * dp + j] + S[(size_t)j * dp + i]) : S[(size_t)i * dp + j]; S[(size_t)i * dp + j] = v; S[(size_t)j * dp + i] = v; }
    for (int i = 0; i < dp; ++i) trace += S[(size_t)i * dp + i];
    if (!(trace > 0) || !std::isfinite(trace)) return ISMHIP_OK;
    jacobi_eig(dp, S, V, w);
    std::vector<int> order(dp); std::iota(order.begin(), order.end(), 0);
    std::stable_sort(order.begin(), order.end(), [&](int a, int b) { return w[a] > w[b]; });
    w_sorted.resize(dp); V_sorted.resize((size_t)dp * dp);
    for (int j = 0; j < dp; ++j) { w_sorted[j] = w[order[j]]; std::copy(V.begin() + (size_t)order[j] * dp, V.begin() + (size_t)(order[j] + 1) * dp, V_sorted.begin() + (size_t)j * dp); }
    const int m_cap = std::min(256, dp);
    double cum = 0; energy = 0;
    if (ctx->knn_pca_m > 0) {
        m = std::max(64, std::min(m_cap, (ctx->knn_pca_m + 31) / 32 * 32));
        for (int i = 0; i < m; ++i) energy += w[order[i]];
        energy /= trace;
    } else {
        for (int i = 0; i < dp && !m; ++i) { cum += w[order[i]]; if ((i + 1) % 32 == 0 && i + 1 >= 64 && cum >= 0.97 * trace) { m = i + 1; energy = cum / trace; } }
        if (m == 0 || m > m_cap || m + 64 > dp) return ISMHIP_OK;
    }
    R.assign((size_t)m * dp, 0.f);
    for (int j = 0; j < m; ++j) for (int c = 0; c < dp; ++c) R[(size_t)j * dp + c] = c < cb->dim ? (float)V[(size_t)order[j] * dp + c] : 0.f;
    }
    int rc = build_image(ctx, cb, cb->pca, R, m, energy, trace);
    if (rc != ISMHIP_OK || cb->pca.m == 0 || identity || ctx->knn_pca_m2 == 0) return rc;
    int m2 = 0; double cum2 = 0, energy2 = 0;
    if (ctx->knn_pca_m2 > 0) m2 = std::max(m + 32, std::min(std::min(256, dp), (ctx->knn_pca_m2 + 31) / 32 * 32));
    for (int i = 0; i < dp; ++i) {
        cum2 += w_sorted[i];
        if (m2 == 0 && (i + 1) % 32 == 0 && i + 1 >= m + 64 && cum2 >= 0.997 * trace) m2 = i + 1;
        if (m2 && i + 1 == m2) energy2 = cum2 / trace;
    }
    if (m2 == 0 || m2 > std::min(256, dp) || (m2 + 64 > dp && ctx->knn_pca_m2 < 0)) return ISMHIP_OK;
    std::vector<float> R2((size_t)m2 * dp, 0.f);
    for (int j = 0; j < m2; ++j) for (int c2 = 0; c2 < dp; ++c2) R2[(size_t)j * dp + c2] = c2 < cb->dim ? (float)V_sorted[(size_t)j * dp + c2] : 0.f;
    return build_image(ctx, cb, cb->pca2, R2, m2, energy2, trace);
}

void ism_codebook_free_pca(ismhip_codebook* cb) {
    for (PcaImage* P : {&cb->pca, &cb->pca2}) {
        if (P->R) (void)hipFree(P->R);
        if (P->f16t) (void)hipFree(P->f16t);
        if (P->cn_scaled) (void)hipFree(P->cn_scaled);
        *P = PcaImage();
    }
}
```

Measured before the change: 20220 objects/s.

## Rotate kNN queries with split-f16 MFMA and fuse query norm computation

Adds a query PCA-rotation kernel that splits both the rotation matrix and the queries into hi/lo f16 parts and uses three f16 MFMAs per tile, replacing the prior f32 rotation path by default. The same kernel emits the f32 query norm and the f16 image norm, so the verify and seed kernels no longer recompute them with per-query wave reductions. Rounding-error bounds for the split product are derived on the host so the lower-bound pruning stays exact. The change also adds a probe API for testing, and an environment flag restores the old f32 rotation.

```diff
diff --git a/include/ismhip.h b/include/ismhip.h
--- a/include/ismhip.h
+++ b/include/ismhip.h
@@ -175,6 +175,8 @@
 int  ismhip_codebook_max_votes_per_word(const ismhip_codebook* cb);
 int  ismhip_codebook_stage1_dims(const ismhip_codebook* cb, float* energy_out);
 int  ismhip_codebook_stage2_dims(const ismhip_codebook* cb, float* energy_out);
+int  ismhip_codebook_rotate_probe(ismhip_ctx* ctx, const ismhip_codebook* cb, int stage, int nq, const float* q, uint16_t* image_out,
+                                  float* qn2_out, float* qn2h_out, float* r_out_h, float* consts_out_h);
 
 int  ismhip_codebook_make_binary(ismhip_ctx* ctx, ismhip_codebook* cb);
 int  ismhip_codebook_has_binary(const ismhip_codebook* cb);
diff --git a/point-cloud-donkey_amd/capi.py b/point-cloud-donkey_amd/capi.py
--- a/point-cloud-donkey_amd/capi.py
+++ b/point-cloud-donkey_amd/capi.py
@@ -20,7 +20,7 @@
     "ismhip_cloud_create", "ismhip_cloud_destroy", "ismhip_cloud_centroids", "ismhip_cloud_radii", "ismhip_estimate_normals", "ismhip_estimate_normals_pca",
     "ismhip_shot_lrf", "ismhip_shotna_lrf", "ismhip_shot352", "ismhip_cshot1344", "ismhip_fpfh33", "ismhip_center_dist",
     "ismhip_compact_features", "ismhip_compact_descriptor_rows", "ismhip_filter_normals", "ismhip_voxel_keypoints", "ismhip_gather_columns",
-    "ismhip_codebook_create", "ismhip_codebook_set_word_class", "ismhip_codebook_destroy", "ismhip_codebook_max_votes_per_word", "ismhip_codebook_stage1_dims", "ismhip_codebook_stage2_dims",
+    "ismhip_codebook_create", "ismhip_codebook_set_word_class", "ismhip_codebook_destroy", "ismhip_codebook_max_votes_per_word", "ismhip_codebook_stage1_dims", "ismhip_codebook_stage2_dims", "ismhip_codebook_rotate_probe",
     "ismhip_knn", "ismhip_knn_ratio", "ismhip_knn_rule", "ismhip_cast_votes", "ismhip_find_maxima", "ismhip_hough3d_maxima", "ismhip_train_activate", "ismhip_kmeans",
     "ismhip_knn_threshold", "ismhip_cast_votes_csr", "ismhip_train_activate_lists", "ismhip_knn_large_k",
     "ismhip_filter_statistical", "ismhip_filter_radius", "ismhip_filter_passthrough_z", "ismhip_compact_points",
@@ -189,6 +189,25 @@
         self.stage2_dims = int(lib().ismhip_codebook_stage2_dims(self._h, C.byref(e)))
         self.stage2_energy = float(e.value)
 
+    def rotate_probe(self, q, stage=1):
+        torch = _torch()
+        consts = np.zeros(3, np.float32)
+        m = lib().ismhip_codebook_rotate_probe(self.ctx._h, self._h, C.c_int(stage), C.c_int(0), None, None, None, None, None, _p(consts))
+        if m < 0:
+            self.ctx.check(m, "ismhip_codebook_rotate_probe")
+        if m == 0:
+            return None
+        nq = int(q.shape[0])
+        dim_pad = (self.dim + 31) // 32 * 32
+        R = np.zeros((m, dim_pad), np.float32)
+        img = torch.empty((nq, m), dtype=torch.float16, device=q.device)
+        qn2 = torch.empty(nq, dtype=torch.float32, device=q.device)
+        qn2h = torch.empty(nq, dtype=torch.float32, device=q.device)
+        rc = lib().ismhip_codebook_rotate_probe(self.ctx._h, self._h, C.c_int(stage), C.c_int(nq), _p(q), _p(img), _p(qn2), _p(qn2h), _p(R), _p(consts))
+        if rc < 0:
+            self.ctx.check(rc, "ismhip_codebook_rotate_probe")
+        return img.cpu().numpy(), qn2.cpu().numpy(), qn2h.cpu().numpy(), R, float(consts[0]), float(consts[1]), float(consts[2])
+
     def set_word_class(self, word_class):
         self.ctx.check(lib().ismhip_codebook_set_word_class(self.ctx._h, self._h, _p(_u32(word_class))), "ismhip_codebook_set_word_class")
 
diff --git a/point-cloud-donkey_amd/csrc/common.h b/point-cloud-donkey_amd/csrc/common.h
--- a/point-cloud-donkey_amd/csrc/common.h
+++ b/point-cloud-donkey_amd/csrc/common.h
@@ -61,6 +61,9 @@
     float inv_sig2 = 1.f;
     float d_rel = 0.f;
     float dq_abs = 0.f, dc_abs = 0.f;
+    unsigned short* R16 = nullptr;
+    int r16_shift = 0;
+    float dq_rel16 = 0.f, dq_abs16 = 0.f;
     float resid2 = 0.f;
     float energy = 0.f;
 };
@@ -147,6 +150,7 @@
     int knn_pca_m = -1;
     bool knn_stage2_t4 = false;
     bool codebook_light = false;
+    bool knn_rotate_f32 = false;
     int knn_pca_m2 = -1;
     uint32_t knn_pca_launches = 0;
     uint32_t knn_thr_overflow = 0;
diff --git a/point-cloud-donkey_amd/csrc/ctx.hip b/point-cloud-donkey_amd/csrc/ctx.hip
--- a/point-cloud-donkey_amd/csrc/ctx.hip
+++ b/point-cloud-donkey_amd/csrc/ctx.hip
@@ -94,6 +94,7 @@
     { const char* e = getenv("ISMHIP_KNN_LARGE_K_SEED_SCALE"); if (e) ctx->knn_lk_seed_scale = (float)atof(e); }
     { const char* e = getenv("ISMHIP_ISS3D_MAP"); ctx->iss3d_wave = e && !strcmp(e, "wave"); }
     { const char* e = getenv("ISMHIP_KNN_PCA_M2"); ctx->knn_pca_m2 = e ? atoi(e) : -1; }
+    { const char* e = getenv("ISMHIP_KNN_ROTATE_F32"); ctx->knn_rotate_f32 = e && e[0] == '1'; }
     if (!own) { ctx->stream = (hipStream_t)stream; ctx->own_stream = false; }
     else {
         if (hipStreamCreateWithFlags(&ctx->stream, hipStreamNonBlocking) != hipSuccess) { delete ctx; return ISMHIP_ERR_HIP; }
diff --git a/point-cloud-donkey_amd/csrc/knn.hip b/point-cloud-donkey_amd/csrc/knn.hip
--- a/point-cloud-donkey_amd/csrc/knn.hip
+++ b/point-cloud-donkey_amd/csrc/knn.hip
@@ -150,8 +150,10 @@
     r.q_lo = r.q_hi + tot;
     if (p.pca) {
         TimerScope tr(ctx, "knn_rotate");
-        const int rc = ism_pca_rotate_queries(ctx, cb, r.PI, r.qq, nq, r.ldq, r.q_hi);
+        float* norms = (float*)r.q_lo;
+        const int rc = ism_pca_rotate_queries(ctx, cb, r.PI, r.qq, nq, r.ldq, r.q_hi, norms, norms + nq_pad);
         if (rc != ISMHIP_OK) return rc;
+        if (ism_pca_split_queries(ctx, r.PI)) { r.qn2 = norms; r.qn2h = norms + nq_pad; }
         ++ctx->knn_pca_launches;
     } else if (p.mode == 0) {
         const float* cq = p.hell ? r.rq->hell_q : r.qq; const int cldq = p.hell ? cb->dim_pad : r.ldq;
diff --git a/point-cloud-donkey_amd/csrc/knn_internal.h b/point-cloud-donkey_amd/csrc/knn_internal.h
--- a/point-cloud-donkey_amd/csrc/knn_internal.h
+++ b/point-cloud-donkey_amd/csrc/knn_internal.h
@@ -204,6 +204,7 @@
     int metric, nq, k, T;
     const float* qq; int ldq;
     u16 *q_hi, *q_lo;
+    const float *qn2, *qn2h;
     float *cand_val, *cand_bound; int* cand_idx; int n_cand, n_bound;
     uint32_t *counters, *qsc;
     KnnQueue queue;
@@ -214,7 +215,8 @@
 int knn_sqrt_queries(ismhip_ctx* ctx, const ismhip_codebook* cb, int nq, const float* q, float* sq, bool& negative);
 int knn_f16_emit_image(ismhip_ctx* ctx, const ismhip_codebook* cb, const ismhip_codebook* xb, const float* qv, int n, int ldv, int n_pad,
                        uint32_t* sc, u16* qimg);
-int ism_pca_rotate_queries(ismhip_ctx* ctx, const ismhip_codebook* cb, const PcaImage* P, const float* q, int nq, int ldq, unsigned short* dst);
+int ism_pca_rotate_queries(ismhip_ctx* ctx, const ismhip_codebook* cb, const PcaImage* P, const float* q, int nq, int ldq, unsigned short* dst, float* qn2, float* qn2h);
+bool ism_pca_split_queries(const ismhip_ctx* ctx, const PcaImage* P);
 int knn_seed_thresholds(KnnRun& r, const float* out_scale, float* thr0);
 int knn_rerank_prove(KnnRun& r, int32_t* idx_out, float* dist_out);
 size_t knn_queue_bytes(size_t n_queries, size_t q_items, int k);
diff --git a/point-cloud-donkey_amd/csrc/knn_rerank.hip b/point-cloud-donkey_amd/csrc/knn_rerank.hip
--- a/point-cloud-donkey_amd/csrc/knn_rerank.hip
+++ b/point-cloud-donkey_amd/csrc/knn_rerank.hip
@@ -145,19 +145,26 @@
 
 struct PcaVerify {
     const u16* qimg; int nk;
+    const float *qn2, *qn2h;
     float inv_sq2;
     float inv_sig2, d_rel, dq_abs, dc;
     float eps_c2, dot2, cmax2;
     float ku;
 };
-__device__ __forceinline__ PcaLb pca_lb_query(const PcaVerify& pv, int qi, float qn2, int lane) {
-    float qn2h = 0.f;
-    for (int i = lane; i < pv.nk * F16T_KB; i += 64) {
-        const float v = (float)__builtin_bit_cast(_Float16, pv.qimg[f16t_stored(qi, pv.nk, i)]);
-        qn2h += v * v;
+__device__ __forceinline__ PcaLb pca_lb_query(const PcaVerify& pv, int qi, const float* __restrict__ qp, int dim, int lane) {
+    float qn2, qn2h;
+    if (pv.qn2) { qn2 = pv.qn2[qi]; qn2h = pv.qn2h[qi]; }
+    else {
+        qn2 = wave_norm2(qp, dim, lane);
+        float s = 0.f;
+        for (int i = lane; i < pv.nk * F16T_KB; i += 64) {
+            const float v = (float)__builtin_bit_cast(_Float16, pv.qimg[f16t_stored(qi, pv.nk, i)]);
+            s += v * v;
+        }
+        qn2h = wave_sum_f(s);
     }
     PcaLb b;
-    b.qn2h = wave_sum_f(qn2h) * pv.inv_sq2;
+    b.qn2h = qn2h * pv.inv_sq2;
     b.dlt = pv.d_rel * (sqrtf(qn2) * 1.00001f) + pv.dq_abs + pv.dc;
     b.eps_s = (pv.eps_c2 + pv.dot2 * sqrtf(b.qn2h * pv.cmax2)) * 1.00001f;
     b.inv_sig2 = pv.inv_sig2;
@@ -173,7 +180,7 @@
     if (qi >= nq || knn_is_padding(tg, qi)) return;
     const int lane = lane_id();
     const float* qp = q + (size_t)qi * ldq;
-    const PcaLb lbq = pca_lb_query(pv, qi, wave_norm2(qp, dim, lane), lane);
+    const PcaLb lbq = pca_lb_query(pv, qi, qp, dim, lane);
     float av;
     const int id = knn_load_cand(cand_idx, cand_val, qi, cand_stride, lane, n_cand, n_words, av);
     const float lb = id >= 0 ? pca_lb_of(lbq, av) : __builtin_inff();
@@ -219,9 +226,10 @@
     if (qi >= nq) return;
     if (live && live[qi] == ~0u) { if (lane_id() == 0) thr[qi] = __builtin_inff(); return; }
     const int lane = lane_id();
-    const float qn2 = wave_norm2(q + (size_t)qi * ldq, dim, lane);
+    float qn2 = 0.f;
     PcaLb lbq{};
-    if (pca) lbq = pca_lb_query(pv, qi, qn2, lane);
+    if (pca) lbq = pca_lb_query(pv, qi, q + (size_t)qi * ldq, dim, lane);
+    else qn2 = wave_norm2(q + (size_t)qi * ldq, dim, lane);
     if (lane != 0) return;
     const float U = seed_dk[qi], osc = out_scale[0];
     float t0 = -__builtin_inff();
@@ -353,7 +361,9 @@
     PcaVerify pv;
     const float acc_rel = 1.01f * (float)PI.m * 1.1920929e-07f;
     pv.qimg = r.q_hi; pv.nk = r.p.ring_nk; pv.inv_sq2 = 1.0f / (PI.sq * PI.sq);
-    pv.inv_sig2 = PI.inv_sig2; pv.d_rel = PI.d_rel; pv.dq_abs = PI.dq_abs;
+    pv.qn2 = r.qn2; pv.qn2h = r.qn2h;
+    const bool split = r.qn2 != nullptr;
+    pv.inv_sig2 = PI.inv_sig2; pv.d_rel = split ? PI.dq_rel16 : PI.d_rel; pv.dq_abs = split ? PI.dq_abs16 : PI.dq_abs;
     pv.dc = (PI.d_rel * sqrtf(r.cb->max_norm2) + PI.dc_abs) * 1.00001f;
     pv.cmax2 = PI.cmax2;
     const float fq = F16_FLUSH / PI.sq, fc = F16_FLUSH / PI.sc, sm = sqrtf((float)PI.m);
diff --git a/point-cloud-donkey_amd/csrc/pca.hip b/point-cloud-donkey_amd/csrc/pca.hip
--- a/point-cloud-donkey_amd/csrc/pca.hip
+++ b/point-cloud-donkey_amd/csrc/pca.hip
@@ -96,6 +96,125 @@
             for (int e = 0; e < 4; ++e) pk.hf[e] = live ? (_Float16)(acc[t][4 * j + e] * scale) : (_Float16)0.f;
             *(uint2*)(base + ((j ^ fsw) << 3)) = pk.u;
         }
+    }
+}
+
+typedef unsigned int u32x4 __attribute__((ext_vector_type(4)));
+template <int NT>
+__global__ __launch_bounds__(256, 2) void k_rotate_split16(const float* __restrict__ x, int n, int ldx, int kdim, const u16* __restrict__ r16, int m,
+                                                            float sx, float out_mul, u16* __restrict__ dst, float* __restrict__ qn2_out, float* __restrict__ qn2h_out) {
+    extern __shared__ __attribute__((aligned(16))) float rot_smem[];
+    const int tid = threadIdx.x, lane = tid & 63, wv = tid >> 6;
+    const int c16 = lane & 15, g = lane >> 4;
+    const int nct = m >> 5;
+    const size_t row0 = (size_t)blockIdx.x * 128;
+    const u32x4* rsrc = (const u32x4*)r16;
+    u32x4* sR = (u32x4*)rot_smem;
+    const float* xrow[2];
+#pragma unroll
+    for (int nt = 0; nt < 2; ++nt) {
+        size_t r = row0 + wv * 32 + nt * 16 + c16; r = r < (size_t)n ? r : (size_t)n - 1;
+        xrow[nt] = x + r * ldx + 4 * g;
+    }
+    f32x4 acc[2 * NT][2];
+#pragma unroll
+    for (int t = 0; t < 2 * NT; ++t)
+#pragma unroll
+        for (int nt = 0; nt < 2; ++nt) acc[t][nt] = f32x4{0.f, 0.f, 0.f, 0.f};
+    u32x4 rs[NT];
+    f32x4 xn[2][2];
+#pragma unroll
+    for (int i = 0; i < NT; ++i) if (i < nct) rs[i] = rsrc[tid + 256 * i];
+#pragma unroll
+    for (int nt = 0; nt < 2; ++nt) { xn[nt][0] = *(const f32x4*)(xrow[nt]); xn[nt][1] = *(const f32x4*)(xrow[nt] + 16); }
+#pragma unroll
+    for (int i = 0; i < NT; ++i) if (i < nct) sR[tid + 256 * i] = rs[i];
+    float qs[2] = {0.f, 0.f};
+    bool bad[2] = {false, false}, isnan_[2] = {false, false};
+    const int nkc = kdim >> 5;
+    for (int kc = 0; kc < nkc; ++kc) {
+        const u32x4* sRb = sR + (kc & 1) * (NT * 256);
+        f32x4 xr[2][2];
+#pragma unroll
+        for (int nt = 0; nt < 2; ++nt) { xr[nt][0] = xn[nt][0]; xr[nt][1] = xn[nt][1]; }
+        __syncthreads();
+        if (kc + 1 < nkc) {
+#pragma unroll
+            for (int i = 0; i < NT; ++i) if (i < nct) rs[i] = rsrc[(size_t)(kc + 1) * nct * 256 + tid + 256 * i];
+#pragma unroll
+            for (int nt = 0; nt < 2; ++nt) { xn[nt][0] = *(const f32x4*)(xrow[nt] + (kc + 1) * 32); xn[nt][1] = *(const f32x4*)(xrow[nt] + (kc + 1) * 32 + 16); }
+        }
+        f16x8 bh[2], bl[2];
+#pragma unroll
+        for (int nt = 0; nt < 2; ++nt) {
+            float part = 0.f;
+#pragma unroll
+            for (int j = 0; j < 8; ++j) {
+                const float xv = xr[nt][j >> 2][j & 3];
+                part += xv * xv;
+                float v = xv * sx;
+                const bool ok = fabsf(v) <= 65504.f;
+                bad[nt] |= !ok; isnan_[nt] |= v != v;
+                v = ok ? v : 0.f;
+                const _Float16 hi = (_Float16)v;
+                bh[nt][j] = hi; bl[nt][j] = (_Float16)(v - (float)hi);
+            }
+            qs[nt] += part;
+        }
+#pragma unroll
+        for (int t = 0; t < 2 * NT; ++t) {
+            if (t >= 2 * nct) continue;
+            const f16x8 ah = __builtin_bit_cast(f16x8, sRb[(2 * t) * 64 + lane]), al = __builtin_bit_cast(f16x8, sRb[(2 * t + 1) * 64 + lane]);
+#pragma unroll
+            for (int nt = 0; nt < 2; ++nt) {
+                acc[t][nt] = __builtin_amdgcn_mfma_f32_16x16x32_f16(al, bh[nt], acc[t][nt], 0, 0, 0);
+                acc[t][nt] = __builtin_amdgcn_mfma_f32_16x16x32_f16(ah, bl[nt], acc[t][nt], 0, 0, 0);
+                acc[t][nt] = __builtin_amdgcn_mfma_f32_16x16x32_f16(ah, bh[nt], acc[t][nt], 0, 0, 0);
+            }
+        }
+        if (kc + 1 < nkc) {
+            u32x4* sRn = sR + ((kc + 1) & 1) * (NT * 256);
+#pragma unroll
+            for (int i = 0; i < NT; ++i) if (i < nct) sRn[tid + 256 * i] = rs[i];
+        }
+    }
+    const size_t n_img = ((size_t)n + F16T_ROWS - 1) / F16T_ROWS * F16T_ROWS;
+#pragma unroll
+    for (int nt = 0; nt < 2; ++nt) {
+        float q2 = qs[nt]; int fl = (bad[nt] ? 1 : 0) | (isnan_[nt] ? 2 : 0);
+        q2 += __shfl_xor(q2, 16, 64); q2 += __shfl_xor(q2, 32, 64);
+        fl |= __shfl_xor(fl, 16, 64); fl |= __shfl_xor(fl, 32, 64);
+        const size_t row = row0 + wv * 32 + nt * 16 + c16;
+        const bool in_img = row < n_img, live = row < (size_t)n;
+        const size_t tile = row / F16T_ROWS; const int r = (int)(row % F16T_ROWS);
+        const int fsw = f16t_swizzle(r);
+        float sq4[16];
+#pragma unroll
+        for (int t = 0; t < 16; ++t) sq4[t] = 0.f;
+#pragma unroll
+        for (int t = 0; t < 2 * NT; ++t) {
+            if (t >= 2 * nct) continue;
+            union { _Float16 hf[4]; uint2 u; } pk;
+            float hs[4];
+#pragma unroll
+            for (int e = 0; e < 4; ++e) {
+                _Float16 hv = (_Float16)(acc[t][nt][e] * out_mul);
+                if (fl & 1) hv = (_Float16)__builtin_inff();
+                if (fl & 2) hv = (_Float16)__builtin_nanf("");
+                if (!live) hv = (_Float16)0.f;
+                pk.hf[e] = hv; hs[e] = (float)hv;
+            }
+            sq4[t] = (hs[0] * hs[0] + hs[1] * hs[1]) + (hs[2] * hs[2] + hs[3] * hs[3]);
+            const int seg = ((t & 1) << 1) | (g >> 1);
+            if (in_img) *(uint2*)(dst + f16t_row(tile, r, nct, t >> 1) + ((seg ^ fsw) << 3) + 4 * (g & 1)) = pk.u;
+        }
+#pragma unroll
+        for (int w = 8; w >= 1; w >>= 1)
+#pragma unroll
+            for (int t = 0; t < w; ++t) sq4[t] += sq4[t + w];
+        float h2 = sq4[0];
+        h2 += __shfl_xor(h2, 16, 64); h2 += __shfl_xor(h2, 32, 64);
+        if (in_img && g == 0) { qn2_out[row] = live ? q2 : 0.f; qn2h_out[row] = h2; }
     }
 }
 
@@ -153,10 +272,126 @@
     return ISMHIP_OK;
 }
 
-}
-
-int ism_pca_rotate_queries(ismhip_ctx* ctx, const ismhip_codebook* cb, const PcaImage* P, const float* q, int nq, int ldq, unsigned short* dst) {
-    return launch_rotate(ctx, q, nq, ldq, cb->dim_pad, P->R, P->m, P->sq, dst);
+int launch_rotate_split(ismhip_ctx* ctx, const float* x, int n, int ldx, int kdim, const PcaImage& P, u16* dst, float* qn2, float* qn2h) {
+    int m = P.m; const int nct = m / 32;
+    const void* kern = nct <= 4 ? (const void*)k_rotate_split16<4> : nct <= 6 ? (const void*)k_rotate_split16<6> : (const void*)k_rotate_split16<8>;
+    const int nt = nct <= 4 ? 4 : nct <= 6 ? 6 : 8;
+    const size_t lds = (size_t)2 * nt * 256 * 16;
+    { const int rc = ism_lds_cap(ctx, kern, lds); if (rc != ISMHIP_OK) return rc; }
+    const unsigned blocks = (unsigned)((((size_t)n + 255) / 256 * 256) / 128);
+    const u16* r16 = P.R16; float sx = P.sq, out_mul = std::ldexp(1.0f, -P.r16_shift);
+    void* args[] = {&x, &n, &ldx, &kdim, &r16, &m, &sx, &out_mul, &dst, &qn2, &qn2h};
+    ISM_HIP(ctx, hipLaunchKernel(kern, dim3(blocks), dim3(256), args, lds, ctx->stream));
+    ISM_CHECK_LAUNCH(ctx, "k_rotate_split16");
+    return ISMHIP_OK;
+}
+
+u16 f16_bits_ftz(float v) {
+    const uint32_t b = __builtin_bit_cast(uint32_t, v), sign = (b >> 16) & 0x8000u, man = b & 0x7fffffu;
+    const int e = (int)((b >> 23) & 0xffu) - 127;
+    if (e < -14) return (u16)sign;
+    uint32_t h = ((uint32_t)(e + 15) << 10) | (man >> 13);
+    const uint32_t rem = man & 0x1fffu;
+    if (rem > 0x1000u || (rem == 0x1000u && (h & 1u))) ++h;
+    return (u16)(sign | h);
+}
+float f16_bits_value(u16 h) {
+    if ((h & 0x7fffu) == 0) return 0.f;
+    const float v = std::ldexp((float)(0x400 | (h & 0x3ff)), ((h >> 10) & 0x1f) - 25);
+    return (h & 0x8000u) ? -v : v;
+}
+
+int split_r16(ismhip_ctx* ctx, PcaImage& P, const std::vector<float>& R, int m, int dp, double sig) {
+    float amax = 0.f;
+    for (float v : R) amax = std::max(amax, std::fabs(v));
+    int shift = 15;
+    while (shift > -40 && std::ldexp((double)amax, shift) > 32768.0) --shift;
+    const int mt_n = m / 16, kc_n = dp / 32;
+    std::vector<u16> frag((size_t)kc_n * mt_n * 2 * 64 * 8);
+    double e2 = 0, fh2 = 0, fl2 = 0;
+    for (int kc = 0; kc < kc_n; ++kc) for (int mt = 0; mt < mt_n; ++mt) for (int lane = 0; lane < 64; ++lane) for (int j = 0; j < 8; ++j) {
+        const int row = 16 * mt + (lane & 15), col = 32 * kc + 16 * (j >> 2) + 4 * (lane >> 4) + (j & 3);
+        const float rs = std::ldexp(R[(size_t)row * dp + col], shift);
+        const u16 hb = f16_bits_ftz(rs); const float hi = f16_bits_value(hb);
+        const u16 lb = f16_bits_ftz(rs - hi); const float lo = f16_bits_value(lb);
+        const size_t at = ((((size_t)kc * mt_n + mt) * 2) * 64 + lane) * 8 + j;
+        frag[at] = hb; frag[at + 64 * 8] = lb;
+        const double e = std::ldexp((double)rs - (double)hi - (double)lo, -shift);
+        e2 += e * e; fh2 += std::ldexp((double)hi, -shift) * std::ldexp((double)hi, -shift); fl2 += std::ldexp((double)lo, -shift) * std::ldexp((double)lo, -shift);
+    }
+    const double eR = std::sqrt(e2), fh = std::sqrt(fh2), fl = std::sqrt(fl2), sD = std::sqrt((double)dp);
+    const double gamma3 = 1.01 * 3.0 * dp * 1.1920929e-07;
+    const double u22 = 2.384185791015625e-07, u11 = 4.8828125e-04;
+    const double rel = eR + (sig + eR) * u22 + fl * 1.001 * u11 + gamma3 * (fh + fl) * 1.002;
+    const double abs_s = (sig + eR) * sD * (double)F16_FLUSH + fl * sD * 5.9604645e-08 + gamma3 * (fh + fl) * sD * 2.0 * (double)F16_FLUSH;
+    P.dq_rel16 = (float)(1.001 * (rel + u11 * (sig + rel)));
+    P.dq_abs16 = (float)(1.001 * ((1.0 + u11) * abs_s + std::sqrt((double)m) * (double)F16_FLUSH) / P.sq);
+    P.r16_shift = shift;
+    if (hipMalloc((void**)&P.R16, frag.size() * sizeof(u16)) != hipSuccess) return ism_set_err(ctx, ISMHIP_ERR_NOMEM, "codebook split rotation matrix");
+    ISM_HIP(ctx, hipMemcpy(P.R16, frag.data(), frag.size() * sizeof(u16), hipMemcpyHostToDevice));
+    return ISMHIP_OK;
+}
+
+__global__ void k_f16t_detile(const u16* __restrict__ img, int n, int m, u16* __restrict__ dense) {
+    const size_t i = (size_t)blockIdx.x * blockDim.x + threadIdx.x;
+    if (i >= (size_t)n * m) return;
+    const unsigned row = (unsigned)(i / m); const int c = (int)(i % m), r = (int)(row % F16T_ROWS);
+    dense[i] = img[f16t_row(row / F16T_ROWS, r, m / F16T_KB, c / F16T_KB) + ((((c % F16T_KB) >> 3) ^ f16t_swizzle(r)) << 3) + (c & 7)];
+}
+__global__ void k_probe_pad_rows(const float* __restrict__ src, int n, int dim, float* __restrict__ dst, int dim_pad) {
+    const size_t i = (size_t)blockIdx.x * blockDim.x + threadIdx.x;
+    if (i >= (size_t)n * dim_pad) return;
+    const int row = (int)(i / dim_pad), col = (int)(i % dim_pad);
+    dst[i] = col < dim ? src[(size_t)row * dim + col] : 0.f;
+}
+
+}
+
+int ism_pca_rotate_queries(ismhip_ctx* ctx, const ismhip_codebook* cb, const PcaImage* P, const float* q, int nq, int ldq, unsigned short* dst, float* qn2, float* qn2h) {
+    if (ctx->knn_rotate_f32 || !P->R16) return launch_rotate(ctx, q, nq, ldq, cb->dim_pad, P->R, P->m, P->sq, dst);
+    return launch_rotate_split(ctx, q, nq, ldq, cb->dim_pad, *P, dst, qn2, qn2h);
+}
+bool ism_pca_split_queries(const ismhip_ctx* ctx, const PcaImage* P) { return !ctx->knn_rotate_f32 && P->R16; }
+
+namespace {
+__global__ __launch_bounds__(256) void k_probe_row_norms(const float* __restrict__ x, int n, int ld, int dim, float* __restrict__ out) {
+    const int row = blockIdx.x * 4 + (threadIdx.x >> 6);
+    if (row >= n) return;
+    const float s = wave_norm2(x + (size_t)row * ld, dim, lane_id());
+    if (lane_id() == 0) out[row] = s;
+}
+}
+
+extern "C" int ismhip_codebook_rotate_probe(ismhip_ctx* ctx, const ismhip_codebook* cb, int stage, int nq, const float* q, uint16_t* image_out,
+                                            float* qn2_out, float* qn2h_out, float* r_out_h, float* consts_out_h) {
+    if (!ctx || !cb || (stage != 1 && stage != 2) || nq < 0) return ism_set_err(ctx, ISMHIP_ERR_INVALID, "codebook_rotate_probe: bad argument");
+    const PcaImage& P = stage == 2 ? cb->pca2 : cb->pca;
+    if (P.m == 0) return 0;
+    const int dp = cb->dim_pad, m = P.m;
+    const bool split = ism_pca_split_queries(ctx, &P);
+    if (consts_out_h) { consts_out_h[0] = P.sq; consts_out_h[1] = split ? P.dq_rel16 : P.d_rel; consts_out_h[2] = split ? P.dq_abs16 : P.dq_abs; }
+    if (r_out_h) ISM_HIP(ctx, hipMemcpy(r_out_h, P.R, (size_t)m * dp * sizeof(float), hipMemcpyDeviceToHost));
+    if (nq == 0 || !q || !image_out || !qn2_out || !qn2h_out) return m;
+    const size_t nq_pad = ((size_t)nq + F16T_ROWS - 1) / F16T_ROWS * F16T_ROWS;
+    const size_t b_q = nq_pad * dp * sizeof(float), b_img = nq_pad * m * sizeof(u16), b_n = nq_pad * sizeof(float);
+    char* buf = (char*)ism_scratch(ctx, SCR_PCA, b_q + b_img + 3 * b_n);
+    if (!buf) return ISMHIP_ERR_NOMEM;
+    float* qpad = (float*)buf; u16* img = (u16*)(buf + b_q); float* n2 = (float*)(buf + b_q + b_img); float* n2h = n2 + nq_pad; float* dummy = n2h + nq_pad;
+    hipLaunchKernelGGL(k_probe_pad_rows, dim3((unsigned)(((size_t)nq * dp + 255) / 256)), dim3(256), 0, ctx->stream, q, nq, cb->dim, qpad, dp);
+    ISM_CHECK_LAUNCH(ctx, "k_probe_pad_rows");
+    int rc = ism_pca_rotate_queries(ctx, cb, &P, qpad, nq, dp, img, n2, n2h);
+    if (rc != ISMHIP_OK) return rc;
+    if (!split) {
+        hipLaunchKernelGGL(k_probe_row_norms, dim3((nq + 3) / 4), dim3(256), 0, ctx->stream, (const float*)qpad, nq, dp, cb->dim, n2);
+        hipLaunchKernelGGL(k_f16t_norms, dim3((unsigned)((nq_pad + 3) / 4)), dim3(256), 0, ctx->stream, (const u16*)img, (int)nq_pad, nq, m / F16T_KB, 0.f, n2h, dummy);
+        ISM_CHECK_LAUNCH(ctx, "k_f16t_norms");
+    }
+    hipLaunchKernelGGL(k_f16t_detile, dim3((unsigned)(((size_t)nq * m + 255) / 256)), dim3(256), 0, ctx->stream, (const u16*)img, nq, m, image_out);
+    ISM_CHECK_LAUNCH(ctx, "k_f16t_detile");
+    ISM_HIP(ctx, hipMemcpyAsync(qn2_out, n2, (size_t)nq * sizeof(float), hipMemcpyDeviceToDevice, ctx->stream));
+    ISM_HIP(ctx, hipMemcpyAsync(qn2h_out, n2h, (size_t)nq * sizeof(float), hipMemcpyDeviceToDevice, ctx->stream));
+    ISM_HIP(ctx, hipStreamSynchronize(ctx->stream));
+    return m;
 }
 
 static int build_image(ismhip_ctx* ctx, ismhip_codebook* cb, PcaImage& P, const std::vector<float>& R, int m, double energy, double trace) {
@@ -185,6 +420,7 @@
     if (hipMalloc((void**)&P.f16t, f16t_halves(n_tiles, nk) * sizeof(u16)) != hipSuccess) return ism_set_err(ctx, ISMHIP_ERR_NOMEM, "codebook rotated f16 image");
     if (hipMalloc((void**)&P.cn_scaled, ((size_t)cb->n_words_pad + 256) * sizeof(float) + 16) != hipSuccess) return ism_set_err(ctx, ISMHIP_ERR_NOMEM, "codebook rotated norms");
     P.osc = P.cn_scaled + cb->n_words_pad + 256;
+    { const int rc = split_r16(ctx, P, R, m, dp, sig); if (rc != ISMHIP_OK) return rc; }
     P.m = m;
     int rc = launch_rotate(ctx, cb->words, cb->n_words_pad, dp, dp, P.R, m, P.sc, P.f16t);
     if (rc != ISMHIP_OK) { P.m = 0; return rc; }
@@ -278,6 +514,7 @@
 void ism_codebook_free_pca(ismhip_codebook* cb) {
     for (PcaImage* P : {&cb->pca, &cb->pca2}) {
         if (P->R) (void)hipFree(P->R);
+        if (P->R16) (void)hipFree(P->R16);
         if (P->f16t) (void)hipFree(P->f16t);
         if (P->cn_scaled) (void)hipFree(P->cn_scaled);
         *P = PcaImage();
```

Result: faster. 20600 objects/s, median of 6 (+1.9%).
